# js43o/HifiDiff

Measured on AMD Instinct MI355X. Metric: faces/sec (whole node), 16→128 1000-step reverse diffusion, batch 64, higher is better.
Workload: dtype bf16

## Files before the change

hifidiff_amd/csrc/hd_dispatch.hpp:

```cpp
#pragma once
#include <type_traits>
#include "hd_gemm.hpp"
#include "hd_wide.hpp"

namespace hd {

enum LdKind { LK_F32, LK_LN, LK_BF16, LK_BF16S, LK_CONV_F32, LK_CONV_F32G, LK_CONV_BF16 };
enum EpKind { EK_BIASF32, EK_RESID, EK_GATE, EK_PIXSHUF, EK_BIASBF16, EK_DWGATE, EK_SCA };

template <class LD, class EP, bool PAIR>
hipError_t launch_tile(const GemmP& p, int mode, hipStream_t s) {
    constexpr bool kWideLN = std::is_same<LD, LdF32LN_T<false>>::value && std::is_same<EP, EpGateBF16>::value && PAIR;
    constexpr bool kWidePlain = std::is_same<LD, LdBF16Plain>::value && std::is_same<EP, EpResidF32>::value && !PAIR;
    if constexpr (kWideLN || kWidePlain) {
        const int form = (mode & 32) ? wide_shape_ok<PAIR>(p) : 0;
        if ((form == 1 || (form == 3 && kWideLN)) && (!kWideLN || wide_stats_ok<PAIR>(p))) return launch_gemm_wide<kWideLN, EP, PAIR>(p, s);
    }
    if constexpr (ld_is_deep<LD>::value && ep_is_deep<EP>::value) {
        if ((mode & 16) && deep_shape_ok<PAIR>(p)) return launch_gemm_deep<LD, EP, PAIR>(p, s);
    }
    mode &= 15;
    if constexpr (PAIR) {
        switch (mode) {
            case 0: return launch_gemm<T128P, LD, EP>(p, s);
            case 1: return launch_gemm<T64P, LD, EP>(p, s);
            case 2: return launch_skinny_auto<1, 2, true, LD, EP>(p, s);
            case 4: return launch_gemm<T32WP, LD, EP>(p, s);
            case 5: return launch_skinny_auto<4, 1, true, LD, EP>(p, s);
            case 6: return launch_skinny_auto<8, 1, true, LD, EP>(p, s);
            default: return launch_skinny_auto<1, 1, true, LD, EP>(p, s);
        }
    } else {
        switch (mode) {
            case 0: return launch_gemm<T128, LD, EP>(p, s);
            case 1: return launch_gemm<T64, LD, EP>(p, s);
            case 2: return launch_skinny_auto<1, 2, false, LD, EP>(p, s);
            case 4: return launch_gemm<T32W, LD, EP>(p, s);
            case 5: return launch_skinny_auto<4, 1, false, LD, EP>(p, s);
            case 6: return launch_skinny_auto<8, 1, false, LD, EP>(p, s);
            default: return launch_skinny_auto<1, 1, false, LD, EP>(p, s);
        }
    }
}

template <class LN>
hipError_t dispatch_dwgate(const GemmP& p, hipStream_t s) {
    if constexpr (std::is_same<LN, LdF32LN_T<false>>::value) {
        static const bool no_wide = hd_env("HD_NO_WIDE") != nullptr;
        const int form = wide_shape_ok<true>(p);
        if (!no_wide && form && wide_stats_ok<true>(p) && p.hw >= 4 && wide_form_rows(form) % p.hw == 0 && p.side * p.side == p.hw)
            return launch_gemm_wide<true, EpDwGate, true>(p, s);
    }
    if constexpr (ld_is_deep<LN>::value) {
        static const bool no_deep_dw = hd_env("HD_NO_DEEP_DW") != nullptr;
        if (!no_deep_dw && deep_shape_ok<true>(p) && p.M % 128 == 0 && p.hw >= 4 && p.hw <= 128 && 128 % p.hw == 0 && p.side * p.side == p.hw)
            return launch_gemm_deep<LN, EpDwGate, true>(p, s);
    }
    if (p.hw <= 32 && 64 % p.hw == 0 && p.M % 64 == 0 && (p.M / 32) * (p.N / 64) >= (p.Kp >= 2048 ? 512 : 1024)) return launch_skinny_auto<1, 2, true, LN, EpDwGate>(p, s);
    if (p.hw <= 32) return launch_skinny_auto<1, 1, true, LN, EpDwGate>(p, s);
    static const bool big64 = hd_env("HD_NO_DW64_WM8") == nullptr;
    if (p.hw == 64 && big64 && p.M % 256 == 0 && (p.M / 64) * (p.N / 64) >= 1024) return launch_skinny_auto<8, 1, true, LN, EpDwGate>(p, s);
    if (p.hw == 64) return launch_skinny_auto<2, 1, true, LN, EpDwGate>(p, s);
    if (p.hw == 256) return launch_skinny_auto<8, 1, true, LN, EpDwGate>(p, s);
    return hipErrorInvalidValue;
}

template <class LN>
hipError_t dispatch_ln(const GemmP& p, EpKind ek, int mode, hipStream_t s) {
    if (ek == EK_DWGATE) {
        static const bool no_dw1 = hd_env("HD_NO_DW1") != nullptr;
        if (p.hw == 1 && !no_dw1) return launch_skinny_auto<1, 1, true, LN, EpDwGate1>(p, s);
        return dispatch_dwgate<LN>(p, s);
    }
    if (ek == EK_BIASF32) return launch_tile<LN, EpBiasF32, false>(p, mode, s);
    if (ek == EK_GATE) return launch_tile<LN, EpGateBF16, true>(p, mode, s);
    return hipErrorInvalidValue;
}

hipError_t dispatch_gemm_ln_shared(const GemmP& p, EpKind ek, int mode, hipStream_t s);
hipError_t dispatch_gemm_ln_face(const GemmP& p, EpKind ek, int mode, hipStream_t s);
hipError_t dispatch_gemm_bf16(const GemmP& p, LdKind lk, EpKind ek, int mode, hipStream_t s);
hipError_t dispatch_gemm_misc(const GemmP& p, LdKind lk, EpKind ek, int mode, hipStream_t s);

}
```

hifidiff_amd/csrc/hd_gemm.hpp:

```cpp
#pragma once
#include <hip/hip_runtime.h>
#include <stdint.h>

#include <stdlib.h>

#include <atomic>

#pragma clang fp contract(off)

namespace hd {

inline hipError_t grant_dynamic_lds(const void* fn, int bytes, std::atomic<unsigned long long>& mask) {
    int dev = 0;
    hipError_t e = hipGetDevice(&dev);
    if (e != hipSuccess) return e;
    const unsigned long long bit = 1ull << (dev & 63);
    if (mask.load(std::memory_order_acquire) & bit) return hipSuccess;
    e = hipFuncSetAttribute(fn, hipFuncAttributeMaxDynamicSharedMemorySize, bytes);
    if (e != hipSuccess) return e;
    mask.fetch_or(bit, std::memory_order_release);
    return hipSuccess;
}


inline const char* hd_env(const char* name) {
    return getenv("HD_EXPERIMENTS") != nullptr ? getenv(name) : nullptr;
}

typedef __attribute__((ext_vector_type(8))) __bf16 bf16x8_t;
typedef __attribute__((ext_vector_type(16))) float f32x16_t;

constexpr int BK = 64;
constexpr int LDS_ROW = BK * 2 + 16;

struct GemmP {
    int M, N, K, Kp;
    int nt_total;
    const uint4* W;
    const float2* stats_in;
    int stats_np, stats_cnt;
    float2* stats_out;
    const void* A;
    int lda;
    float a_scale;
    int hw;
    int face0;
    const float* film;
    int film_face_stride, film_step_stride, film_gain_off, film_bias_off;
    const int* step_ptr;
    float ln_eps;
    const float* rowscale;
    int Hin, Win, Cin, KH, KW, stride, pad, Hout, Wout, ntaps;
    const float* gate_c;
    const float* gate_s;
    const float* add_src;
    void* out;
    int ldo;
    unsigned short* out16;
    unsigned short* outg16;
    const float* bias;
    const float* rscale;
    const void* resid;
    int ldr;
    int act;
    int shuffle_r;
    int xcd_tile_affine;
    const float* dw_w;
    const float* dw_b;
    float* pooled;
    unsigned short* pooled16;
    int side;
    unsigned short* scale_G;
    int scale_hw;
    int w_nt;
    const uint4* pf_base;
    unsigned pf_tile_u4;
    int pf_ntiles;
#ifdef HD_STAMPS
    unsigned long long* stamps;
#endif
};

#ifdef HD_STAMPS
#define HD_STAMP(i)                                                                                     \
    do {                                                                                                \
        if (p.stamps && threadIdx.x == 0)                                                               \
            p.stamps[((size_t)blockIdx.y * gridDim.x + blockIdx.x) * 8 + (i)] = __builtin_amdgcn_s_memrealtime(); \
    } while (0)
#else
#define HD_STAMP(i) do { } while (0)
#endif

typedef float f32x2_t __attribute__((ext_vector_type(2)));
typedef __bf16 bf16x2_t __attribute__((ext_vector_type(2)));
__device__ __forceinline__ unsigned pack2(f32x2_t v) { return __builtin_bit_cast(unsigned, __builtin_convertvector(v, bf16x2_t)); }
__device__ __forceinline__ unsigned pack2(float lo, float hi) { return pack2((f32x2_t){lo, hi}); }
__device__ __forceinline__ uint4 pack8(const float* v) {
    return make_uint4(pack2(v[0], v[1]), pack2(v[2], v[3]), pack2(v[4], v[5]), pack2(v[6], v[7]));
}
__device__ __forceinline__ void unpack8(uint4 u, float* v) {
    v[0] = __uint_as_float(u.x << 16); v[1] = __uint_as_float(u.x & 0xffff0000u);
    v[2] = __uint_as_float(u.y << 16); v[3] = __uint_as_float(u.y & 0xffff0000u);
    v[4] = __uint_as_float(u.z << 16); v[5] = __uint_as_float(u.z & 0xffff0000u);
    v[6] = __uint_as_float(u.w << 16); v[7] = __uint_as_float(u.w & 0xffff0000u);
}
__device__ __forceinline__ float bf16_bits_to_f32(unsigned short v) { return __uint_as_float((unsigned)v << 16); }
__device__ __forceinline__ unsigned short f32_to_bf16_bits(float f) {
    return __builtin_bit_cast(unsigned short, (__bf16)f);
}
template <int CTRL>
__device__ __forceinline__ float dpp_mov(float v) {
    return __builtin_bit_cast(float, __builtin_amdgcn_update_dpp(0, __builtin_bit_cast(int, v), CTRL, 0xF, 0xF, true));
}
__device__ __forceinline__ float row16_sum(float v) {
    v += dpp_mov<0xB1>(v);
    v += dpp_mov<0x4E>(v);
    v += dpp_mov<0x141>(v);
    v += dpp_mov<0x140>(v);
    return v;
}
__device__ __forceinline__ float lane_value(float v, int lane) {
    return __builtin_bit_cast(float, __builtin_amdgcn_readlane(__builtin_bit_cast(int, v), lane));
}
__device__ __forceinline__ float halfwave_sum_hi(float v) {
    v = row16_sum(v);
    const int t = __builtin_amdgcn_update_dpp(0, __builtin_bit_cast(int, v), 0x142, 0xA, 0xF, false);
    return v + __builtin_bit_cast(float, t);
}
__device__ __forceinline__ float wave_sum(float v) {
    v = halfwave_sum_hi(v);
    return lane_value(v, 31) + lane_value(v, 63);
}

struct F8 { float4 a, b; };
__device__ __forceinline__ F8 ldg44(const float* p) {
    F8 r; r.a = *reinterpret_cast<const float4*>(p); r.b = *reinterpret_cast<const float4*>(p + 32); return r;
}
__device__ __forceinline__ F8 zero8() { F8 r; r.a = make_float4(0, 0, 0, 0); r.b = r.a; return r; }
__device__ __forceinline__ void f8_to_arr(const F8& x, float* v) {
    v[0] = x.a.x; v[1] = x.a.y; v[2] = x.a.z; v[3] = x.a.w; v[4] = x.b.x; v[5] = x.b.y; v[6] = x.b.z; v[7] = x.b.w;
}
template <bool SPLIT>
__device__ __forceinline__ void lds_write_unit(char* row_base, int kq, uint4 v) {
    if (SPLIT) {
        *reinterpret_cast<uint2*>(row_base + 8 * kq) = make_uint2(v.x, v.y);
        *reinterpret_cast<uint2*>(row_base + 64 + 8 * kq) = make_uint2(v.z, v.w);
    } else {
        *reinterpret_cast<uint4*>(row_base + 16 * kq) = v;
    }
}

struct LdF32Plain {
    static constexpr int kRawRegs = 8;
    static constexpr bool kGainBiasLds = false, kSplit = true, kStaticK = false;
    struct St { const float* rowp; bool valid; };
    struct Raw { F8 x; };
    struct Pre {};
    template <int BM, int THREADS> static __device__ __forceinline__ void block_issue(const GemmP&, int, float*, int, Pre&) {}
    template <int BM, int THREADS> static __device__ __forceinline__ void block_finish(const GemmP&, int, char*, float*, int, const Pre&) {}
    template <int BM, int THREADS> static __device__ void block_init(const GemmP&, int, char*, float*, int) {}
    template <class S> static __device__ __forceinline__ void unit_stats(S&, int, const char*) {}
    static __device__ __forceinline__ void unit_init(const GemmP& p, St& st, int row, int, const char*, const float*) {
        st.valid = row < p.M;
        st.rowp = reinterpret_cast<const float*>(p.A) + (size_t)(st.valid ? row : 0) * p.lda;
    }
    static __device__ __forceinline__ void fetch(const GemmP& p, const St& st, int kc, int kq, Raw& r) {
        if (st.valid && kc + 32 + 4 * kq < p.K) r.x = ldg44(st.rowp + kc + 4 * kq);
        else { r.x = zero8(); if (st.valid && kc + 4 * kq < p.K) r.x.a = *reinterpret_cast<const float4*>(st.rowp + kc + 4 * kq); }
    }
    static __device__ __forceinline__ uint4 finish(const GemmP& p, const St&, int, int, const Raw& r) {
        float v[8]; f8_to_arr(r.x, v);
#pragma unroll
        for (int i = 0; i < 8; ++i) v[i] *= p.a_scale;
        return pack8(v);
    }
};

template <bool PER_FACE>
struct LdF32LN_T {
    static constexpr int kRawRegs = 4;
    static constexpr bool kGainBiasLds = !PER_FACE, kSplit = false, kStaticK = true;
    static constexpr bool kDeep = !PER_FACE;
    struct St { const unsigned short* rowp; const float* gain; const float* bias; const float* gbl; float mu, rstd; bool valid; };
    struct Raw { uint4 x; };
    static constexpr int kPP = 4;
    struct Pre { float2 s[kPP]; float4 g[2], b[2]; };
    template <int BM, int THREADS> static constexpr int tpr() { return THREADS / BM >= 16 ? 16 : (THREADS / BM >= 1 ? THREADS / BM : 1); }
    template <int BM, int THREADS> static __device__ __forceinline__ bool fast(const GemmP& p) {
        return p.stats_np <= kPP * tpr<BM, THREADS>() && BM * tpr<BM, THREADS>() <= THREADS;
    }
    static __device__ __forceinline__ const float* film_row(const GemmP& p) {
        const int step = p.step_ptr ? *p.step_ptr : 0;
        return p.film + (size_t)step * p.film_step_stride;
    }
    template <int BM, int THREADS> static __device__ __forceinline__ void block_issue(const GemmP& p, int row0, float* gb, int tid, Pre& pre) {
        constexpr int TPR = tpr<BM, THREADS>();
        if (fast<BM, THREADS>(p)) {
            const int rl = tid / TPR, part = tid % TPR, row = row0 + rl;
            const bool rv = rl < BM && row < p.M;
            const float2* sp = p.stats_in + (size_t)(rv ? row : 0) * p.stats_np;
#pragma unroll
            for (int i = 0; i < kPP; ++i) {
                const int j = part + i * TPR;
                pre.s[i] = (rv && j < p.stats_np) ? sp[j] : make_float2(0.f, -1.f);
            }
        }
        if (gb && p.film_face_stride == 0) {
            const float* f = film_row(p);
#pragma unroll
            for (int i = 0; i < 2; ++i) {
                const int k = (tid + i * THREADS) * 4;
                if (k < p.K) {
                    pre.g[i] = *reinterpret_cast<const float4*>(f + p.film_gain_off + k);
                    pre.b[i] = *reinterpret_cast<const float4*>(f + p.film_bias_off + k);
                }
            }
        }
    }
    template <int BM, int THREADS> static __device__ __forceinline__ void block_finish(const GemmP& p, int row0, char* stats, float* gb, int tid, const Pre& pre) {
        constexpr int TPR = tpr<BM, THREADS>();
        float2* st = reinterpret_cast<float2*>(stats);
        if (gb && p.film_face_stride == 0) {
#pragma unroll
            for (int i = 0; i < 2; ++i) {
                const int k = (tid + i * THREADS) * 4;
                if (k < p.K) {
                    *reinterpret_cast<float4*>(gb + k) = pre.g[i];
                    *reinterpret_cast<float4*>(gb + p.Kp + k) = pre.b[i];
                }
            }
// ... 297 lines not shown
        for (int h = 0; h < 2; ++h) {
            float4 x = r.inb[h] ? r.x[h] : make_float4(0, 0, 0, 0);
            if (GATED && r.inb[h]) {
                const float4 a = r.add[h], g = r.gc[h];
                const float s = 1.0f + r.gs[h];
                x.x = (x.x + a.x) * (s + g.x); x.y = (x.y + a.y) * (s + g.y);
                x.z = (x.z + a.z) * (s + g.z); x.w = (x.w + a.w) * (s + g.w);
            }
            v[4 * h] = x.x; v[4 * h + 1] = x.y; v[4 * h + 2] = x.z; v[4 * h + 3] = x.w;
        }
        return pack8(v);
    }
};

__device__ __forceinline__ float activate(float v, int act) {
    if (act == 1) return fmaxf(v, 0.f);
    if (act == 2) return 1.0f / (1.0f + expf(-v));
    return v;
}
struct ColC { float bias, bias2, rscale, rscale2; };

struct EpBiasF32 {
    static constexpr bool kStats = true, kTile = false;
    static __device__ __forceinline__ size_t stat_index(const GemmP& p, int row, int tile_idx) { return (size_t)row * (p.N >> 5) + tile_idx; }
    static __device__ __forceinline__ ColC col_init(const GemmP& p, int col) { ColC c; c.bias = p.bias ? p.bias[col] : 0.f; c.bias2 = 0.f; c.rscale = 1.f; return c; }
    static __device__ __forceinline__ float pre(const GemmP&, int, int) { return 0.f; }
    static __device__ __forceinline__ float store(const GemmP& p, int row, int col, float v, float, const ColC& c) {
        v = activate(v + c.bias, p.act);
        reinterpret_cast<float*>(p.out)[(size_t)row * p.ldo + col] = v;
        if (p.out16) p.out16[(size_t)row * p.ldo + col] = f32_to_bf16_bits(v);
        return v;
    }
};
struct EpScaBF16 {
    static constexpr bool kStats = false, kTile = false, kScaTile = true;
    static __device__ __forceinline__ ColC col_init(const GemmP& p, int col) { ColC c; c.bias = p.bias[col]; c.bias2 = 0.f; c.rscale = 1.f; return c; }
    static __device__ __forceinline__ float pre(const GemmP&, int, int) { return 0.f; }
    static __device__ __forceinline__ float store(const GemmP& p, int row, int col, float v, float, const ColC& c) {
        v += c.bias;
        reinterpret_cast<float*>(p.out)[(size_t)row * p.ldo + col] = v;
        return v;
    }
};
struct EpResidF32 {
    static constexpr bool kStats = true, kTile = false;
    static constexpr bool kDeep = true;
    static __device__ __forceinline__ size_t stat_index(const GemmP& p, int row, int tile_idx) { return (size_t)row * (p.N >> 5) + tile_idx; }
    static __device__ __forceinline__ ColC col_init(const GemmP& p, int col) { ColC c; c.bias = p.bias[col]; c.bias2 = 0.f; c.rscale = p.rscale[col]; return c; }
    static __device__ __forceinline__ float pre(const GemmP& p, int row, int col) {
        return reinterpret_cast<const float*>(p.resid)[(size_t)row * p.ldr + col];
    }
    static __device__ __forceinline__ float store(const GemmP& p, int row, int col, float v, float r, const ColC& c) {
        v = fmaf(v + c.bias, c.rscale, r);
        reinterpret_cast<float*>(p.out)[(size_t)row * p.ldo + col] = v;
        if (p.out16) p.out16[(size_t)row * p.ldo + col] = f32_to_bf16_bits(v);
        if (p.outg16) {
            const float a = p.add_src ? p.add_src[(size_t)row * p.ldo + col] : 0.f;
            const float g = 1.0f + p.gate_c[(size_t)(row / p.hw) * p.N + col] + p.gate_s[row];
            p.outg16[(size_t)row * p.ldo + col] = f32_to_bf16_bits((v + a) * g);
        }
        return v;
    }
};
struct EpGateBF16 {
    static constexpr bool kStats = false, kTile = false;
    static constexpr bool kDeep = true;
    static __device__ __forceinline__ ColC col_init(const GemmP& p, int col) { ColC c; c.bias = p.bias[col]; c.bias2 = p.bias[col + (p.N >> 1)]; c.rscale = 1.f; return c; }
    static __device__ __forceinline__ float pre(const GemmP&, int, int) { return 0.f; }
    static __device__ __forceinline__ void store2(const GemmP& p, int row, int col, float v1, float v2, const ColC& c) {
        reinterpret_cast<unsigned short*>(p.out)[(size_t)row * p.ldo + col] = f32_to_bf16_bits((v1 + c.bias) * (v2 + c.bias2));
    }
};
struct EpDwGate1 {
    static constexpr bool kStats = false, kTile = false;
    static __device__ __forceinline__ ColC col_init(const GemmP& p, int col) {
        const int C2 = p.N >> 1;
        const float wa = p.dw_w[(size_t)4 * p.N + col], wb = p.dw_w[(size_t)4 * p.N + col + C2];
        ColC c; c.bias = p.dw_b[col] + wa * p.bias[col]; c.bias2 = p.dw_b[col + C2] + wb * p.bias[col + C2];
        c.rscale = wa; c.rscale2 = wb;
        return c;
    }
    static __device__ __forceinline__ float pre(const GemmP&, int, int) { return 0.f; }
    static __device__ __forceinline__ void store2(const GemmP& p, int row, int col, float v1, float v2, const ColC& c) {
        const float g = fmaf(c.rscale, v1, c.bias) * fmaf(c.rscale2, v2, c.bias2);
        const size_t o = (size_t)row * p.ldo + col;
        reinterpret_cast<unsigned short*>(p.out)[o] = f32_to_bf16_bits(g);
        p.pooled[o] = g;
        if (p.pooled16) p.pooled16[o] = f32_to_bf16_bits(g);
    }
};
struct EpSca1BF16 {
    static constexpr bool kStats = false, kTile = false;
    static __device__ __forceinline__ ColC col_init(const GemmP& p, int col) { ColC c; c.bias = p.bias[col]; c.bias2 = 0.f; c.rscale = 1.f; c.rscale2 = 0.f; return c; }
    static __device__ __forceinline__ float pre(const GemmP& p, int row, int col) { return bf16_bits_to_f32(p.scale_G[(size_t)row * p.ldo + col]); }
    static __device__ __forceinline__ float store(const GemmP& p, int row, int col, float v, float g, const ColC& c) {
        v += c.bias;
        reinterpret_cast<float*>(p.out)[(size_t)row * p.ldo + col] = v;
        p.scale_G[(size_t)row * p.ldo + col] = f32_to_bf16_bits(g * v);
        return v;
    }
};
struct EpPixShufF32 {
    static constexpr bool kStats = true, kTile = false;
    static __device__ __forceinline__ ColC col_init(const GemmP&, int) { ColC c; c.bias = 0.f; c.bias2 = 0.f; c.rscale = 1.f; return c; }
    static __device__ __forceinline__ size_t out_row(const GemmP& p, int row, int sub) {
        const int lw = 31 - __builtin_clz(p.Win);
        const int b = row >> (2 * lw), rem = row & ((1 << (2 * lw)) - 1);
        const int h = rem >> lw, w = rem & (p.Win - 1);
        return (((size_t)b << (lw + 1)) + (2 * h + (sub >> 1))) * (2 * p.Win) + (2 * w + (sub & 1));
    }
    static __device__ __forceinline__ size_t index(const GemmP& p, int row, int col) {
        if (p.shuffle_r == 2) {
            const int lc = 31 - __builtin_clz(p.ldo);
            return out_row(p, row, col >> lc) * p.ldo + (col & (p.ldo - 1));
        }
        return (size_t)row * p.ldo + col;
    }
    static __device__ __forceinline__ size_t stat_index(const GemmP& p, int row, int tile_idx) {
        if (p.shuffle_r == 2) {
            const int lt = 31 - __builtin_clz(p.ldo >> 5);
            return out_row(p, row, tile_idx >> lt) * (p.ldo >> 5) + (tile_idx & ((p.ldo >> 5) - 1));
        }
        return (size_t)row * (p.N >> 5) + tile_idx;
    }
    static __device__ __forceinline__ float pre(const GemmP& p, int row, int col) {
        return p.resid ? reinterpret_cast<const float*>(p.resid)[index(p, row, col)] : 0.f;
    }
    static __device__ __forceinline__ float store(const GemmP& p, int row, int col, float v, float r, const ColC&) {
        v += r;
        const size_t o = index(p, row, col);
        reinterpret_cast<float*>(p.out)[o] = v;
        if (p.out16) p.out16[o] = f32_to_bf16_bits(v);
        return v;
    }
};
struct EpBiasBF16 {
    static constexpr bool kStats = false, kTile = false;
    static __device__ __forceinline__ ColC col_init(const GemmP& p, int col) { ColC c; c.bias = p.bias[col]; c.bias2 = 0.f; c.rscale = 1.f; return c; }
    static __device__ __forceinline__ float pre(const GemmP& p, int row, int col) {
        return p.resid ? bf16_bits_to_f32(reinterpret_cast<const unsigned short*>(p.resid)[(size_t)row * p.ldr + col]) : 0.f;
    }
    static __device__ __forceinline__ float store(const GemmP& p, int row, int col, float v, float r, const ColC& c) {
        v = activate(v + c.bias + r, p.act);
        reinterpret_cast<unsigned short*>(p.out)[(size_t)row * p.ldo + col] = f32_to_bf16_bits(v);
        return v;
    }
};
struct EpDwGate {
    static constexpr bool kStats = false, kTile = true;
    static __device__ __forceinline__ ColC col_init(const GemmP&, int) { ColC c; c.bias = 0.f; c.bias2 = 0.f; c.rscale = 1.f; return c; }
    static __device__ __forceinline__ float pre(const GemmP&, int, int) { return 0.f; }
    static __device__ __forceinline__ void store2(const GemmP&, int, int, float, float, const ColC&) {}
};

constexpr int kStatLane = 16;
__device__ __forceinline__ float2 halfwave_mean_m2(float v) {
    const float s1 = halfwave_sum_hi(v), s2 = halfwave_sum_hi(v * v);
    const float mean = s1 * (1.0f / 32.0f);
    return make_float2(mean, fmaxf(fmaf(-s1, mean, s2), 0.f));
}

template <bool FULL, bool PAIR, class EP>
__device__ __forceinline__ void tile_epilogue_mfma(const GemmP& p, const f32x16_t& a1, const f32x16_t& a2, int rbase, int col,
                                                   int ncols, int tile_idx, int lane) {
    const bool cv = FULL || col < ncols;
    const ColC cc = EP::col_init(p, cv ? col : 0);
    float pre[16], v[16];
#pragma unroll
    for (int i = 0; i < 16; ++i) {
        const int row = rbase + (i & 3) + 8 * (i >> 2);
        pre[i] = (FULL || (cv && row < p.M)) ? EP::pre(p, row, col) : 0.f;
    }
#pragma unroll
    for (int i = 0; i < 16; ++i) {
        const int row = rbase + (i & 3) + 8 * (i >> 2);
        v[i] = 0.f;
        if (FULL || (cv && row < p.M)) {
            if constexpr (PAIR) EP::store2(p, row, col, a1[i], a2[i], cc);
            else v[i] = EP::store(p, row, col, a1[i], pre[i], cc);
        }
    }
    if constexpr (EP::kStats) {
        if (p.stats_out) {
            float2 ms[16];
#pragma unroll
            for (int i = 0; i < 16; ++i) ms[i] = halfwave_mean_m2(v[i]);
            if ((lane & 31) == kStatLane) {
#pragma unroll
                for (int i = 0; i < 16; ++i) {
                    const int row = rbase + (i & 3) + 8 * (i >> 2);
                    if (FULL || row < p.M) p.stats_out[EP::stat_index(p, row, tile_idx)] = ms[i];
                }
            }
        }
    }
}

template <int WM_, int WN_, int MT_, int TN_, bool PAIR_>
struct Cfg {
    static constexpr int WM = WM_, WN = WN_, MT = MT_, TN = TN_;
    static constexpr bool PAIR = PAIR_;
    static constexpr int WAVES = WM * WN;
    static constexpr int THREADS = 64 * WAVES;
    static constexpr int BM = WM * MT * 32;
    static constexpr int TNT = PAIR ? 2 * TN : TN;
    static constexpr int NCOLS = WN * TN * 32;
    static constexpr int UNITS = BM * 8 / THREADS;
    static constexpr int A_BUF = BM * LDS_ROW;
    static constexpr int STATS_OFF = 2 * A_BUF;
    static constexpr int GB_OFF = STATS_OFF + BM * 8;
    static constexpr int SMEM = GB_OFF;
    static_assert(UNITS >= 1 && UNITS * THREADS == BM * 8, "tile/threads mismatch");
};

template <class C, class LD, class EP>
__global__ __launch_bounds__(C::THREADS) void gemm_kernel(const GemmP p) {
    extern __shared__ __attribute__((aligned(16))) char smem[];
    const int tid = threadIdx.x, lane = tid & 63, wave = tid >> 6;
    const int w_m = wave / C::WN, w_n = wave - w_m * C::WN;
    const int row0 = blockIdx.x * C::BM;
    const int ksteps_total = p.Kp >> 4;
    const int c_end = p.Kp >> 6;

    int tile[C::TNT];
#pragma unroll
    for (int tn = 0; tn < C::TN; ++tn) {
        const int t = (blockIdx.y * C::WN + w_n) * C::TN + tn;
        tile[tn] = t;
        if (C::PAIR) tile[C::TN + tn] = t + (p.N >> 6);
    }
    const int tiles_half = C::PAIR ? (p.N >> 6) : p.nt_total;

    HD_STAMP(0);
    float* gb = LD::kGainBiasLds ? reinterpret_cast<float*>(smem + C::GB_OFF) : nullptr;
    typename LD::St st[C::UNITS];
    int u_ldsoff[C::UNITS];
    const int kq = tid & 7;
#pragma unroll
    for (int u = 0; u < C::UNITS; ++u) {
        const int rl = (tid >> 3) + u * (C::THREADS / 8);
        u_ldsoff[u] = rl * LDS_ROW;
        LD::unit_init(p, st[u], row0 + rl, rl, smem + C::STATS_OFF, gb);
    }

    f32x16_t acc[C::MT][C::TNT];
#pragma unroll
    for (int mt = 0; mt < C::MT; ++mt)
#pragma unroll
        for (int tn = 0; tn < C::TNT; ++tn)
#pragma unroll
            for (int i = 0; i < 16; ++i) acc[mt][tn][i] = 0.f;

    typename LD::Raw raw[C::UNITS];
    uint4 bcur[C::TNT][4], bnxt[C::TNT][4];
    const uint4* Wl = p.W + lane;

#define HD_LOAD_B(dst, chunk)                                                                         \
    _Pragma("unroll") for (int tn = 0; tn < C::TNT; ++tn) {                                           \
        const bool tv = (tn < C::TN ? tile[tn] : tile[tn] - (p.N >> 6)) < tiles_half &&               \
                        tile[tn] < p.nt_total;                                                        \
        _Pragma("unroll") for (int s = 0; s < 4; ++s)                                                 \
            dst[tn][s] = tv ? Wl[((size_t)tile[tn] * ksteps_total + (chunk) * 4 + s) * 64]            \
                            : make_uint4(0, 0, 0, 0);                                                 \
    }
#define HD_FETCH_A(chunk)                                                                             \
    _Pragma("unroll") for (int u = 0; u < C::UNITS; ++u) LD::fetch(p, st[u], (chunk) * BK, kq, raw[u]);
#define HD_WRITE_A(chunk, buf)                                                                        \
    _Pragma("unroll") for (int u = 0; u < C::UNITS; ++u)                                              \
        lds_write_unit<LD::kSplit>(smem + (buf) * C::A_BUF + u_ldsoff[u], kq, LD::finish(p, st[u], (chunk) * BK, kq, raw[u]));

    HD_FETCH_A(0);
    HD_LOAD_B(bcur, 0);
    LD::template block_init<C::BM, C::THREADS>(p, row0, smem + C::STATS_OFF, gb, tid);
#pragma unroll
    for (int u = 0; u < C::UNITS; ++u) LD::unit_stats(st[u], (tid >> 3) + u * (C::THREADS / 8), smem + C::STATS_OFF);
    HD_STAMP(1);
    HD_WRITE_A(0, 0);
    __syncthreads();
    HD_STAMP(2);

    const int a_lane_off = (lane & 31) * LDS_ROW + (lane >> 5) * 16;
    for (int c = 0; c < c_end; ++c) {
        const int buf = c & 1;
        const bool has_next = (c + 1) < c_end;
        if (has_next) {
            HD_FETCH_A(c + 1);
            HD_LOAD_B(bnxt, c + 1);
        }
        const char* sA = smem + buf * C::A_BUF + a_lane_off;
#pragma unroll
        for (int s = 0; s < 4; ++s) {
            bf16x8_t a[C::MT];
#pragma unroll
            for (int mt = 0; mt < C::MT; ++mt)
                a[mt] = *reinterpret_cast<const bf16x8_t*>(sA + ((w_m * C::MT + mt) * 32) * LDS_ROW + s * 32);
#pragma unroll
            for (int tn = 0; tn < C::TNT; ++tn)
#pragma unroll
                for (int mt = 0; mt < C::MT; ++mt)
                    acc[mt][tn] = __builtin_amdgcn_mfma_f32_32x32x16_bf16(
                        a[mt], __builtin_bit_cast(bf16x8_t, bcur[tn][s]), acc[mt][tn], 0, 0, 0);
        }
        if (has_next) {
            HD_WRITE_A(c + 1, buf ^ 1);
        }
        __syncthreads();
// ... 289 lines not shown
            const bool up = y > 0, dn = y < S - 1;
            const int row = row0 + p0;
            unsigned short* gout = reinterpret_cast<unsigned short*>(p.out) + (size_t)row * p.ldo + col;
            const int left = p.M - row;
            float rsum;
            switch (S) {
                case 16: rsum = dw_gate_row<16>(t1a, t1b, p0, up, dn, wa, wb, ba, bb, gout, p.ldo, true, left); break;
                case 8: rsum = dw_gate_row<8>(t1a, t1b, p0, up, dn, wa, wb, ba, bb, gout, p.ldo, true, left); break;
                case 4: rsum = dw_gate_row<4>(t1a, t1b, p0, up, dn, wa, wb, ba, bb, gout, p.ldo, true, left); break;
                default: rsum = dw_gate_row<2>(t1a, t1b, p0, up, dn, wa, wb, ba, bb, gout, p.ldo, true, left); break;
            }
            rs[rr * 32 + j] = rsum;
        }
        asm volatile("s_waitcnt lgkmcnt(0)\n\ts_barrier" ::: "memory");
        const int faces = 128 / HW;
        for (int idx = tid; idx < faces * 32; idx += THREADS) {
            const int f = idx >> 5;
            float sacc = 0.f;
            for (int r = 0; r < S; ++r) sacc += rs[(f * S + r) * 32 + j];
            const int face = row0 / HW + f;
            if (face * HW < p.M) {
                const float pm = sacc / (float)HW;
                p.pooled[(size_t)face * C2 + col] = pm;
                if (p.pooled16) p.pooled16[(size_t)face * C2 + col] = f32_to_bf16_bits(pm);
            }
        }
        (void)ncols;
        return;
    }
    float* xch = reinterpret_cast<float*>(smem);
    if (half) {
#pragma unroll
        for (int i = 0; i < 16; ++i) xch[(w_m * 16 + i) * 64 + lane] = acc[i];
    }
    asm volatile("s_waitcnt lgkmcnt(0)\n\ts_barrier" ::: "memory");
    if (!half) {
        f32x16_t acc2;
#pragma unroll
        for (int i = 0; i < 16; ++i) acc2[i] = xch[(w_m * 16 + i) * 64 + lane];
        const int ncols = p.N >> 1;
        const int rtile = row0 + w_m * 32;
        const int rbase = rtile + 4 * (lane >> 5);
        const int col = tile0 * 32 + (lane & 31);
        if (rtile + 32 <= p.M) tile_epilogue_mfma<true, true, EP>(p, acc, acc2, rbase, col, ncols, tile0, lane);
        else tile_epilogue_mfma<false, true, EP>(p, acc, acc2, rbase, col, ncols, tile0, lane);
    }
    HD_STAMP(5);
}

template <class EP, class = void> struct ep_is_sca_tile { static constexpr bool value = false; };
template <class EP> struct ep_is_sca_tile<EP, decltype((void)EP::kScaTile)> { static constexpr bool value = EP::kScaTile; };

typedef unsigned u32x4_t __attribute__((ext_vector_type(4)));
__device__ __forceinline__ void prefetch_issue(const GemmP& p, int lin, int nwg, int tid, int nthreads, u32x4_t& sink) {
    if (!p.pf_base) return;
    const int x = lin & 7, r = lin >> 3, per_x = nwg >> 3;
    const int tiles_x = (p.pf_ntiles - x + 7) >> 3;
    if (tiles_x <= 0 || r >= per_x) return;
    const unsigned total = (unsigned)tiles_x * p.pf_tile_u4;
    const unsigned share = (total + per_x - 1) / per_x;
    const unsigned lo = share * r, hi = (lo + share < total) ? lo + share : total;
    for (unsigned i = lo + tid; i < hi; i += nthreads) {
        const unsigned t = i / p.pf_tile_u4, o = i - t * p.pf_tile_u4;
        const uint4* q = p.pf_base + ((size_t)(x + 8 * t) * p.pf_tile_u4 + o);
        asm volatile("global_load_dwordx4 %0, %1, off" : "+v"(sink) : "v"(q) : "memory");
    }
}
__device__ __forceinline__ void prefetch_drain(u32x4_t& sink) {
    asm volatile("s_waitcnt vmcnt(0)" : "+v"(sink) : : "memory");
}

typedef unsigned nt_u32x4 __attribute__((ext_vector_type(4)));
__device__ __forceinline__ uint4 nt_load_u4(const uint4* q) {
    const nt_u32x4 v = __builtin_nontemporal_load(reinterpret_cast<const nt_u32x4*>(q));
    return make_uint4(v.x, v.y, v.z, v.w);
}
template <int WM_, int WK_, int MT_, bool PAIR_, int D_, bool HALF_ = false>
struct SkinnyCfg {
    static constexpr int WM = WM_, WK = WK_, MT = MT_, D = D_;
    static constexpr bool HALF = HALF_;
    static_assert(!HALF_ || (WM_ == 1 && MT_ == 1), "HALF tiles are single-row-tile workgroups");
    static constexpr int WROWS = HALF_ ? 16 : MT_ * 32;
    static constexpr int WAVES = WM * WK, THREADS = 64 * WAVES, BM = WM * WROWS, TNT = PAIR_ ? 2 : 1;
    static constexpr int UN = WROWS / 8;
    static constexpr int A_WAVE = MT * 32 * LDS_ROW;
    static constexpr int RED = WK * BM * 32 * TNT * 4;
    static constexpr int STAGE = (WAVES * A_WAVE > RED) ? WAVES * A_WAVE : RED;
    static constexpr int GT_OFF = STAGE;
    static constexpr int STATS_OFF = GT_OFF + BM * 32 * 4;
    static constexpr int GB_OFF = STATS_OFF + BM * 8;
};

template <int S>
__device__ __forceinline__ float dw_gate_row(const float* t1a, const float* t1b, int p0, bool up, bool dn, const float* wa,
                                             const float* wb, float ba, float bb, unsigned short* gout, int ldo, bool store_ok,
                                             int rows_left) {
    float va[3][S + 2], vb[3][S + 2];
#pragma unroll
    for (int r = 0; r < 3; ++r) { va[r][0] = 0.f; va[r][S + 1] = 0.f; vb[r][0] = 0.f; vb[r][S + 1] = 0.f; }
#pragma unroll
    for (int x = 0; x < S; ++x) {
        va[0][x + 1] = up ? t1a[(p0 + x - S) * 32] : 0.f; vb[0][x + 1] = up ? t1b[(p0 + x - S) * 32] : 0.f;
        va[1][x + 1] = t1a[(p0 + x) * 32];                vb[1][x + 1] = t1b[(p0 + x) * 32];
        va[2][x + 1] = dn ? t1a[(p0 + x + S) * 32] : 0.f; vb[2][x + 1] = dn ? t1b[(p0 + x + S) * 32] : 0.f;
    }
    float rsum = 0.f;
#pragma unroll
    for (int x = 0; x < S; ++x) {
        float u1 = ba, u2 = bb;
#pragma unroll
        for (int r = 0; r < 3; ++r) {
            u1 = fmaf(wa[r * 3], va[r][x], u1); u1 = fmaf(wa[r * 3 + 1], va[r][x + 1], u1); u1 = fmaf(wa[r * 3 + 2], va[r][x + 2], u1);
            u2 = fmaf(wb[r * 3], vb[r][x], u2); u2 = fmaf(wb[r * 3 + 1], vb[r][x + 1], u2); u2 = fmaf(wb[r * 3 + 2], vb[r][x + 2], u2);
        }
        const float g = u1 * u2;
        rsum += g;
        if (store_ok && x < rows_left) gout[(size_t)x * ldo] = f32_to_bf16_bits(g);
    }
    return rsum;
}

template <class C> struct SkinnyPre { static constexpr int NIT = (C::BM * 32 + C::THREADS - 1) / C::THREADS; ColC cc; float pre[NIT]; };
template <bool FULL, class C, class EP>
__device__ __forceinline__ void skinny_rows_pre(const GemmP& p, int row0, int col, int ncols, int tid, SkinnyPre<C>& sp) {
    constexpr int NIT = SkinnyPre<C>::NIT;
    constexpr bool EVEN = (C::BM * 32) % C::THREADS == 0;
    const bool cv = FULL || col < ncols;
    sp.cc = EP::col_init(p, cv ? col : 0);
#pragma unroll
    for (int it = 0; it < NIT; ++it) {
        const int e = it * C::THREADS + tid;
        const int row = row0 + (e >> 5);
        const bool ok = (EVEN || e < C::BM * 32) && (FULL || (row < p.M && cv));
        sp.pre[it] = ok ? EP::pre(p, row, col) : 0.f;
    }
}
template <bool FULL, class C, class EP>
__device__ __forceinline__ void skinny_rows_epilogue(const GemmP& p, const float* red, int row0, int col, int ncols, int tile_idx, int tid,
                                                     const SkinnyPre<C>& sp) {
    constexpr int NIT = (C::BM * 32 + C::THREADS - 1) / C::THREADS, TNT = C::TNT, WK = C::WK;
    constexpr int TILE_F = C::BM * 32 * TNT;
    constexpr bool EVEN = (C::BM * 32) % C::THREADS == 0;
    const bool cv = FULL || col < ncols;
    const ColC cc = sp.cc;
    const float (&pre)[NIT] = sp.pre;
    float v[NIT];
#pragma unroll
    for (int it = 0; it < NIT; ++it) {
        const int e = it * C::THREADS + tid;
        const int row = row0 + (e >> 5);
        const bool ev = EVEN || e < C::BM * 32;
        float v1 = 0.f, v2 = 0.f;
        if (ev) {
#pragma unroll
            for (int w = 0; w < WK; ++w) {
                v1 += red[w * TILE_F + e];
                if (TNT == 2) v2 += red[w * TILE_F + C::BM * 32 + e];
            }
        }
        v[it] = 0.f;
        if (ev && (FULL || (row < p.M && cv))) {
            if constexpr (TNT == 2) EP::store2(p, row, col, v1, v2, cc);
            else v[it] = EP::store(p, row, col, v1, pre[it], cc);
        }
    }
    if constexpr (EP::kStats) {
        if (p.stats_out) {
            float2 ms[NIT];
#pragma unroll
            for (int it = 0; it < NIT; ++it) ms[it] = halfwave_mean_m2(v[it]);
            if ((tid & 31) == kStatLane) {
#pragma unroll
                for (int it = 0; it < NIT; ++it) {
                    const int e = it * C::THREADS + tid;
                    const int row = row0 + (e >> 5);
                    if ((EVEN || e < C::BM * 32) && (FULL || row < p.M)) p.stats_out[EP::stat_index(p, row, tile_idx)] = ms[it];
                }
            }
        }
    }
}

template <class C, class LD, class EP, bool W_NT = false, int CPW = 0>
__global__ __launch_bounds__(C::THREADS) void gemm_skinny_kernel(const GemmP p) {
    extern __shared__ __attribute__((aligned(16))) char smem[];
    constexpr int MT = C::MT, TNT = C::TNT, WK = C::WK, D = C::D, UN = C::UN;
    const int tid = threadIdx.x, lane = tid & 63, wave = tid >> 6;
    const int wm = wave / WK, wk = wave - wm * WK;
    int bx = blockIdx.x, by = blockIdx.y;
    if (p.xcd_tile_affine && (gridDim.y & 7) == 0 && gridDim.x > 1) {
        const int lin = blockIdx.y * gridDim.x + blockIdx.x;
        const int j = lin >> 3;
        bx = j % (int)gridDim.x;
        by = (j / (int)gridDim.x) * 8 + (lin & 7);
    }
    const int row0 = bx * C::BM;
    const int ksteps_total = p.Kp >> 4;
    const int cpw = CPW > 0 ? CPW : (p.Kp >> 6) / WK;
    const int c0 = wk * cpw, c_end = c0 + cpw;
    int tile[TNT];
    tile[0] = by;
    if (TNT == 2) tile[1] = by + (p.N >> 6);
    const uint4* Wl = p.W + lane;
    constexpr bool w_nt = W_NT;
    HD_STAMP(0);

    f32x16_t acc[MT][TNT];
#pragma unroll
    for (int mt = 0; mt < MT; ++mt)
#pragma unroll
        for (int tn = 0; tn < TNT; ++tn)
#pragma unroll
            for (int i = 0; i < 16; ++i) acc[mt][tn][i] = 0.f;
    uint4 bq[D][4][TNT];
    typename LD::Raw aq[D][UN];
#define HD_SK_LOAD_B(slot, chunk)                                                                      \
    _Pragma("unroll") for (int ss = 0; ss < 4; ++ss) _Pragma("unroll") for (int tn = 0; tn < TNT; ++tn) \
        bq[slot][ss][tn] = ((chunk) < c_end) ? (w_nt ? nt_load_u4(&Wl[((size_t)tile[tn] * ksteps_total + (chunk) * 4 + ss) * 64]) : Wl[((size_t)tile[tn] * ksteps_total + (chunk) * 4 + ss) * 64]) : make_uint4(0, 0, 0, 0);
    float* gb = LD::kGainBiasLds ? reinterpret_cast<float*>(smem + C::GB_OFF) : nullptr;
    typename LD::Pre pre;
    LD::template block_issue<C::BM, C::THREADS>(p, row0, gb, tid, pre);
#define HD_SK_LOAD_B_NC(slot, chunk)                                                                   \
    _Pragma("unroll") for (int ss = 0; ss < 4; ++ss) _Pragma("unroll") for (int tn = 0; tn < TNT; ++tn) \
        bq[slot][ss][tn] = w_nt ? nt_load_u4(&Wl[((size_t)tile[tn] * ksteps_total + (chunk) * 4 + ss) * 64]) : Wl[((size_t)tile[tn] * ksteps_total + (chunk) * 4 + ss) * 64];
    if constexpr (CPW == 0) {
#pragma unroll
        for (int d = 0; d < D; ++d) { HD_SK_LOAD_B(d, c0 + d); }
    }

    typename LD::St st[UN];
    int u_off[UN];
    const int kq = lane & 7;
#pragma unroll
    for (int u = 0; u < UN; ++u) {
        const int rw = (lane >> 3) + 8 * u;
        const int rl = wm * C::WROWS + rw;
        u_off[u] = rw * LDS_ROW;
        LD::unit_init(p, st[u], row0 + rl, rl, smem + C::STATS_OFF, gb);
    }
#define HD_SK_FETCH_A(slot, chunk)                                                                     \
    _Pragma("unroll") for (int u = 0; u < UN; ++u)                                                     \
        LD::fetch(p, st[u], ((chunk) < c_end) ? (chunk) * BK : p.Kp, kq, aq[slot][u]);
#define HD_SK_FETCH_A_NC(slot, chunk) \
    _Pragma("unroll") for (int u = 0; u < UN; ++u) LD::fetch_nc(p, st[u], (chunk) * BK, kq, aq[slot][u]);
    if constexpr (CPW > 0) {
#pragma unroll
        for (int d = 0; d < (D < CPW ? D : CPW); ++d) { HD_SK_LOAD_B_NC(d, c0 + d); HD_SK_FETCH_A_NC(d, c0 + d); }
    } else {
#pragma unroll
        for (int d = 0; d < D; ++d) { HD_SK_FETCH_A(d, c0 + d); }
    }
    constexpr bool kEarlyDw = EP::kTile && C::THREADS >= 512;
    float dw_wa[9], dw_wb[9], dw_ba = 0.f, dw_bb = 0.f, dw_b1a = 0.f, dw_b1b = 0.f;
    auto load_dw = [&]() {
        const int ncols_e = p.N >> 1, col_e = tile[0] * 32 + (tid & 31);
        const bool cok = col_e < ncols_e;
#pragma unroll
        for (int t = 0; t < 9; ++t) { dw_wa[t] = cok ? p.dw_w[(size_t)t * p.N + col_e] : 0.f; dw_wb[t] = cok ? p.dw_w[(size_t)t * p.N + col_e + ncols_e] : 0.f; }
        if (cok) { dw_ba = p.dw_b[col_e]; dw_bb = p.dw_b[col_e + ncols_e]; dw_b1a = p.bias[col_e]; dw_b1b = p.bias[col_e + ncols_e]; }
    };
    if constexpr (kEarlyDw) load_dw();
    uint4 sca_g[2] = {make_uint4(0, 0, 0, 0), make_uint4(0, 0, 0, 0)};
    if constexpr (ep_is_sca_tile<EP>::value) {
        const int hw = p.scale_hw, units = C::BM * hw * 4;
        if (hw > 0 && tile[0] * 32 + 32 <= p.N) {
#pragma unroll
            for (int j = 0; j < 2; ++j) {
                const int u = tid + j * C::THREADS;
                const int f = u / (hw * 4), rem = u - f * hw * 4, r = rem >> 2, q = rem & 3;
                if (u < units && row0 + f < p.M)
                    sca_g[j] = *reinterpret_cast<const uint4*>(p.scale_G + ((size_t)(row0 + f) * hw + r) * p.ldo + tile[0] * 32 + q * 8);
            }
        }
    }
    constexpr bool kEarlyPre = !EP::kTile && !ep_is_sca_tile<EP>::value && C::THREADS >= 512;
    SkinnyPre<C> spre;
    if constexpr (kEarlyPre) {
        const int ncols_e = (TNT == 2) ? (p.N >> 1) : p.N, col_e = tile[0] * 32 + (tid & 31);
        const bool full_e = (row0 + C::BM <= p.M) && (tile[0] * 32 + 32 <= ncols_e);
        if (full_e) skinny_rows_pre<true, C, EP>(p, row0, col_e, ncols_e, tid, spre);
        else skinny_rows_pre<false, C, EP>(p, row0, col_e, ncols_e, tid, spre);
    }
    u32x4_t pf_sink = {0u, 0u, 0u, 0u};
    prefetch_issue(p, (int)(blockIdx.y * gridDim.x + blockIdx.x), (int)(gridDim.x * gridDim.y), tid, C::THREADS, pf_sink);
    HD_STAMP(6);
    LD::template block_finish<C::BM, C::THREADS>(p, row0, smem + C::STATS_OFF, gb, tid, pre);
#pragma unroll
    for (int u = 0; u < UN; ++u) LD::unit_stats(st[u], wm * C::WROWS + (lane >> 3) + 8 * u, smem + C::STATS_OFF);
    HD_STAMP(1);

    char* sA = smem + wave * C::A_WAVE;
    const int a_lane_off = (lane & 31) * LDS_ROW + (lane >> 5) * 16;
    if constexpr (C::HALF) {
        for (int i = lane; i < 16 * LDS_ROW / 16; i += 64) reinterpret_cast<uint4*>(sA + 16 * LDS_ROW)[i] = make_uint4(0, 0, 0, 0);
        __builtin_amdgcn_wave_barrier();
    }
    auto chunk_mma = [&](int d, int cc) {
        if constexpr (CPW > 0) {
            typename LD::ChunkC chunk_c;
            LD::chunk_consts(p, st[0], cc * BK, kq, chunk_c);
#pragma unroll
            for (int u = 0; u < UN; ++u) lds_write_unit<LD::kSplit>(sA + u_off[u], kq, LD::finish_nc(p, st[u], cc * BK, kq, aq[d][u], chunk_c));
        } else {
#pragma unroll
            for (int u = 0; u < UN; ++u) lds_write_unit<LD::kSplit>(sA + u_off[u], kq, LD::finish(p, st[u], cc * BK, kq, aq[d][u]));
        }
        __builtin_amdgcn_wave_barrier();
#pragma unroll
        for (int ss = 0; ss < 4; ++ss) {
            bf16x8_t a[MT];
#pragma unroll
            for (int mt = 0; mt < MT; ++mt)
                a[mt] = *reinterpret_cast<const bf16x8_t*>(sA + a_lane_off + (mt * 32) * LDS_ROW + ss * 32);
#pragma unroll
            for (int tn = 0; tn < TNT; ++tn)
#pragma unroll
                for (int mt = 0; mt < MT; ++mt)
                    acc[mt][tn] = __builtin_amdgcn_mfma_f32_32x32x16_bf16(
                        a[mt], __builtin_bit_cast(bf16x8_t, bq[d][ss][tn]), acc[mt][tn], 0, 0, 0);
        }
        __builtin_amdgcn_wave_barrier();
    };
    if constexpr (CPW > 0) {
#pragma unroll
        for (int i = 0; i < CPW; ++i) {
            const int d = i % D, cc = c0 + i;
            chunk_mma(d, cc);
            if (i + D < CPW) { HD_SK_LOAD_B_NC(d, cc + D); HD_SK_FETCH_A_NC(d, cc + D); }
            if (i == 0) HD_STAMP(2);
        }
    } else {
        for (int cb = c0; cb < c_end; cb += D) {
#pragma unroll
            for (int d = 0; d < D; ++d) {
                const int cc = cb + d;
                if (cc < c_end) {
                    chunk_mma(d, cc);
                    HD_SK_LOAD_B(d, cc + D);
                    HD_SK_FETCH_A(d, cc + D);
                    if (cc == c0) HD_STAMP(2);
                }
            }
        }
    }
#undef HD_SK_LOAD_B
#undef HD_SK_FETCH_A
#undef HD_SK_LOAD_B_NC
#undef HD_SK_FETCH_A_NC
    HD_STAMP(3);

    __syncthreads();
    HD_STAMP(4);
    float* red = reinterpret_cast<float*>(smem);
    constexpr int TILE_F = C::BM * 32 * TNT;
#pragma unroll
    for (int mt = 0; mt < MT; ++mt)
#pragma unroll
        for (int tn = 0; tn < TNT; ++tn)
#pragma unroll
            for (int i = 0; i < (C::HALF ? 8 : 16); ++i) {
                const int r = (wm * MT + mt) * 32 + (i & 3) + 8 * (i >> 2) + 4 * (lane >> 5);
                red[wk * TILE_F + (tn * C::BM + r) * 32 + (lane & 31)] = acc[mt][tn][i];
            }
    __syncthreads();
    const int ncols = (TNT == 2) ? (p.N >> 1) : p.N;
    const int col = tile[0] * 32 + (tid & 31);

    if constexpr (EP::kTile) {
        static_assert(TNT == 2, "EpDwGate needs a PAIR tile");
        const int C2 = p.N >> 1;
        if constexpr (!kEarlyDw) load_dw();
        {
            const float bias_a = dw_b1a, bias_b = dw_b1b;
            for (int e = tid; e < C::BM * 32; e += C::THREADS) {
                float va = bias_a, vb = bias_b;
#pragma unroll
                for (int w = 0; w < WK; ++w) { va += red[w * TILE_F + e]; vb += red[w * TILE_F + C::BM * 32 + e]; }
                red[e] = va; red[C::BM * 32 + e] = vb;
            }
        }
        __syncthreads();
        float* rs = reinterpret_cast<float*>(smem + C::GT_OFF);
        const int j = tid & 31;
        const int S = p.side, ls = 31 - __builtin_clz(S), HW = p.hw;
        const float (&wa)[9] = dw_wa; const float (&wb)[9] = dw_wb;
        const float ba = dw_ba, bb = dw_bb;
        const float* t1a = red + j;
        const float* t1b = red + C::BM * 32 + j;
        const int nrows_img = C::BM >> ls;
        for (int rr = tid >> 5; rr < nrows_img; rr += C::THREADS / 32) {
            const int p0 = rr << ls;
            const int y = (p0 & (HW - 1)) >> ls;
            const bool up = y > 0, dn = y < S - 1;
            const int row = row0 + p0;
            unsigned short* gout = reinterpret_cast<unsigned short*>(p.out) + (size_t)row * p.ldo + col;
            const bool ok = col < ncols;
            const int left = p.M - row;
            float rsum;
            switch (S) {
                case 16: rsum = dw_gate_row<16>(t1a, t1b, p0, up, dn, wa, wb, ba, bb, gout, p.ldo, ok, left); break;
                case 8: rsum = dw_gate_row<8>(t1a, t1b, p0, up, dn, wa, wb, ba, bb, gout, p.ldo, ok, left); break;
                case 4: rsum = dw_gate_row<4>(t1a, t1b, p0, up, dn, wa, wb, ba, bb, gout, p.ldo, ok, left); break;
                case 2: rsum = dw_gate_row<2>(t1a, t1b, p0, up, dn, wa, wb, ba, bb, gout, p.ldo, ok, left); break;
                default: rsum = dw_gate_row<1>(t1a, t1b, p0, up, dn, wa, wb, ba, bb, gout, p.ldo, ok, left); break;
            }
            rs[rr * 32 + j] = rsum;
        }
        __syncthreads();
        const int faces = C::BM / HW;
        for (int idx = tid; idx < faces * 32; idx += C::THREADS) {
            const int f = idx >> 5;
            float sacc = 0.f;
            for (int r = 0; r < S; ++r) sacc += rs[(f * S + r) * 32 + j];
            const int face = row0 / HW + f;
            if (face * HW < p.M && col < ncols) {
                const float pm = sacc / (float)HW;
                p.pooled[(size_t)face * C2 + col] = pm;
                if (p.pooled16) p.pooled16[(size_t)face * C2 + col] = f32_to_bf16_bits(pm);
            }
        }
    } else if constexpr (ep_is_sca_tile<EP>::value) {
        {
            const float bias = col < ncols ? p.bias[col] : 0.f;
            for (int e = tid; e < C::BM * 32; e += C::THREADS) {
                float v = bias;
#pragma unroll
                for (int w = 0; w < WK; ++w) v += red[w * TILE_F + e];
                const int face = row0 + (e >> 5);
                if (face < p.M && col < ncols) reinterpret_cast<float*>(p.out)[(size_t)face * p.ldo + col] = v;
                red[e] = v;
            }
        }
        __syncthreads();
        const int hw = p.scale_hw;
        if (hw > 0 && tile[0] * 32 + 32 <= ncols) {
            const int units = C::BM * hw * 4;
            for (int u0 = tid; u0 < units; u0 += C::THREADS * 2) {
                uint4 g[2]; unsigned short* gp[2]; const float* sp[2]; bool ok[2];
#pragma unroll
                for (int j = 0; j < 2; ++j) {
                    const int u = u0 + j * C::THREADS;
                    const int f = u / (hw * 4), rem = u - f * hw * 4, r = rem >> 2, q = rem & 3;
                    const int face = row0 + f;
                    ok[j] = u < units && face < p.M;
                    gp[j] = p.scale_G + ((size_t)(ok[j] ? face : 0) * hw + r) * p.ldo + tile[0] * 32 + q * 8;
                    sp[j] = red + f * 32 + q * 8;
                    g[j] = (u0 == tid) ? sca_g[j]
                                       : (ok[j] ? *reinterpret_cast<const uint4*>(gp[j]) : make_uint4(0, 0, 0, 0));
                }
#pragma unroll
                for (int j = 0; j < 2; ++j) {
                    if (ok[j]) {
                        float v[8];
                        unpack8(g[j], v);
#pragma unroll
                        for (int i = 0; i < 8; ++i) v[i] *= sp[j][i];
                        *reinterpret_cast<uint4*>(gp[j]) = pack8(v);
                    }
                }
            }
        }
    } else {
        const bool full = (row0 + C::BM <= p.M) && (tile[0] * 32 + 32 <= ncols);
        if constexpr (!kEarlyPre) {
            if (full) skinny_rows_pre<true, C, EP>(p, row0, col, ncols, tid, spre);
            else skinny_rows_pre<false, C, EP>(p, row0, col, ncols, tid, spre);
        }
        if (full) skinny_rows_epilogue<true, C, EP>(p, red, row0, col, ncols, tile[0], tid, spre);
        else skinny_rows_epilogue<false, C, EP>(p, red, row0, col, ncols, tile[0], tid, spre);
    }
    if (p.pf_base) prefetch_drain(pf_sink);
    HD_STAMP(5);
}

typedef Cfg<4, 1, 1, 2, false> T128;
typedef Cfg<4, 1, 1, 1, true> T128P;
typedef Cfg<2, 2, 1, 1, false> T64;
typedef Cfg<2, 2, 1, 1, true> T64P;
typedef Cfg<1, 4, 1, 2, false> T32W;
typedef Cfg<1, 4, 1, 1, true> T32WP;

template <class C, class LD, class EP>
inline hipError_t launch_gemm(const GemmP& p, hipStream_t s) {
    const int ncols = C::PAIR ? p.N / 2 : p.N;
    const int smem = C::SMEM + (LD::kGainBiasLds ? 2 * p.Kp * 4 : 0);
    if (smem > 65536) {
        static std::atomic<unsigned long long> granted{0};
        { const hipError_t e = grant_dynamic_lds(reinterpret_cast<const void*>(&gemm_kernel<C, LD, EP>), 160 * 1024, granted); if (e != hipSuccess) return e; }
    }
    dim3 grid((p.M + C::BM - 1) / C::BM, (ncols + C::NCOLS - 1) / C::NCOLS, 1);
    hipLaunchKernelGGL((gemm_kernel<C, LD, EP>), grid, dim3(C::THREADS), smem, s, p);
    return hipGetLastError();
}

template <bool PAIR>
inline bool deep_shape_ok(const GemmP& p) {
    const int ncols = PAIR ? p.N / 2 : p.N;
    return p.K == p.Kp && (p.Kp == 512 || p.Kp == 1024) && p.M >= (PAIR ? 1024 : 2048) && ncols % 32 == 0 && p.film_face_stride == 0 &&
           ((p.M + 127) / 128) * (ncols / 32) >= 256;
}
#ifndef HD_DEEP_P
#define HD_DEEP_P 4
#endif
template <class LD, class EP, bool PAIR>
inline hipError_t launch_gemm_deep(const GemmP& p, hipStream_t s) {
    typedef Cfg<4, 1, 1, 1, PAIR> C;
    constexpr int P = HD_DEEP_P;
    const int ncols = PAIR ? p.N / 2 : p.N;
    const int smem = C::SMEM + (LD::kGainBiasLds ? 2 * p.Kp * 4 : 0) + 2 * (PAIR ? 8 : 4) * 1024;
    dim3 grid((p.M + C::BM - 1) / C::BM, ncols / 32, 1);
    if constexpr (PAIR) {
        if (p.Kp == 1024) hipLaunchKernelGGL((gemm_deep_pair8_kernel<LD, EP, 16, P>), grid, dim3(512), smem, s, p);
        else hipLaunchKernelGGL((gemm_deep_pair8_kernel<LD, EP, 8, P>), grid, dim3(512), smem, s, p);
        return hipGetLastError();
    }
    if (p.Kp == 1024) hipLaunchKernelGGL((gemm_deep_kernel<C, LD, EP, 16, P>), grid, dim3(C::THREADS), smem, s, p);
    else hipLaunchKernelGGL((gemm_deep_kernel<C, LD, EP, 8, P>), grid, dim3(C::THREADS), smem, s, p);
    return hipGetLastError();
}

template <class C, class LD, class EP, bool NT, int CPW>
inline hipError_t launch_skinny_inst(const GemmP& p, hipStream_t s, int smem) {
    if (smem > 65536) {
        static std::atomic<unsigned long long> granted{0};
        { const hipError_t e = grant_dynamic_lds(reinterpret_cast<const void*>(&gemm_skinny_kernel<C, LD, EP, NT, CPW>), 160 * 1024, granted); if (e != hipSuccess) return e; }
    }
    const int ncols = (C::TNT == 2) ? p.N / 2 : p.N;
    dim3 grid((p.M + C::BM - 1) / C::BM, (ncols + 31) / 32, 1);
    hipLaunchKernelGGL((gemm_skinny_kernel<C, LD, EP, NT, CPW>), grid, dim3(C::THREADS), smem, s, p);
    return hipGetLastError();
}

template <class C, class LD, class EP>
inline hipError_t launch_skinny(const GemmP& p, hipStream_t s) {
    const int smem = C::GB_OFF + (LD::kGainBiasLds ? 2 * p.Kp * 4 : 0);
    if (smem > 160 * 1024 || (p.Kp / 64) % C::WK != 0) return hipErrorInvalidValue;
    const bool nt = p.w_nt != 0;
    if constexpr (LD::kStaticK) {
        static const bool no_static = hd_env("HD_NO_STATIC_K") != nullptr;
        const int cpw = (p.Kp / 64) / C::WK;
        const int ncols = (C::TNT == 2) ? p.N / 2 : p.N;
        const bool ok = !no_static && p.K == p.Kp && ncols % 32 == 0 && LD::static_ok(p);
        if (ok && (cpw == 2 || cpw == 4)) {
            if (cpw == 4) return nt ? launch_skinny_inst<C, LD, EP, true, 4>(p, s, smem) : launch_skinny_inst<C, LD, EP, false, 4>(p, s, smem);
            return nt ? launch_skinny_inst<C, LD, EP, true, 2>(p, s, smem) : launch_skinny_inst<C, LD, EP, false, 2>(p, s, smem);
        }
        if constexpr (LD::kStatic8 && C::WK == 8 && C::MT == 1) {
            if (ok && cpw == 8) return nt ? launch_skinny_inst<C, LD, EP, true, 8>(p, s, smem) : launch_skinny_inst<C, LD, EP, false, 8>(p, s, smem);
        }
    }
    return nt ? launch_skinny_inst<C, LD, EP, true, 0>(p, s, smem) : launch_skinny_inst<C, LD, EP, false, 0>(p, s, smem);
}

template <int MT, bool PAIR, class LD>
struct ChunkDepth {
    static constexpr int TNT = PAIR ? 2 : 1;
    static constexpr int fixed = MT * TNT * 16 + 48 + MT * 4 * 6;
    static constexpr int per_d = TNT * 16 + MT * 4 * LD::kRawRegs;
    static constexpr int D = (fixed + 3 * per_d <= 236) ? 3 : ((fixed + 2 * per_d <= 236) ? 2 : 1);
};

template <int WM, int MT, bool PAIR, class LD, class EP>
inline hipError_t launch_skinny_auto(const GemmP& p, hipStream_t s) {
    constexpr int D = ChunkDepth<MT, PAIR, LD>::D;
    const int chunks = p.Kp / 64;
    if constexpr (WM == 1 && MT == 1) {
        static const bool no_half = hd_env("HD_NO_HALF") != nullptr;
        const int tiles = (PAIR ? p.N / 2 : p.N) / 32;
        static const int half_m = hd_env("HD_HALF_M") ? atoi(hd_env("HD_HALF_M")) : 64;
        static const int half_wg = hd_env("HD_HALF_WG") ? atoi(hd_env("HD_HALF_WG")) : 256;
        if (!no_half && p.M <= half_m && p.M % 16 == 0 && ((p.M + 31) / 32) * tiles < half_wg) {
            if (chunks >= 16 && chunks % 8 == 0) return launch_skinny<SkinnyCfg<1, 8, 1, PAIR, D, true>, LD, EP>(p, s);
            if (chunks >= 8 && chunks % 4 == 0) return launch_skinny<SkinnyCfg<1, 4, 1, PAIR, D, true>, LD, EP>(p, s);
        }
    }
    if constexpr (WM <= 1) if (chunks >= 16 && chunks % 8 == 0) return launch_skinny<SkinnyCfg<WM, 8, MT, PAIR, D>, LD, EP>(p, s);
    if constexpr (WM <= 2) if (chunks >= 8 && chunks % 4 == 0) return launch_skinny<SkinnyCfg<WM, 4, MT, PAIR, D>, LD, EP>(p, s);
    if constexpr (WM <= 4) if (chunks >= 4 && chunks % 2 == 0) return launch_skinny<SkinnyCfg<WM, 2, MT, PAIR, D>, LD, EP>(p, s);
    return launch_skinny<SkinnyCfg<WM, 1, MT, PAIR, D>, LD, EP>(p, s);
}

}

#pragma clang fp contract(fast)
```

hifidiff_amd/csrc/hd_internal.hpp:

```cpp
#pragma once
#include <hip/hip_runtime.h>

#include <cmath>
#include <cstdio>
#include <cstring>
#include <functional>
#include <map>
#include <memory>
#include <string>
#include <unordered_map>
#include <vector>

#include "../../include/hifidiff_hip.h"
#include "hd_chain.hpp"
#include "hd_conv.hpp"
#include "hd_cr.hpp"
#include "hd_dispatch.hpp"
#include "hd_gemm.hpp"
#include "hd_kernels.hpp"
#include "hd_end.hpp"
#include "hd_faceset.hpp"
#include "hd_vae.hpp"
#include "hd_stage_api.hpp"

using namespace hd;

namespace hdi {

constexpr int WIDTH = 128;
constexpr int FILM_IN = 256;
constexpr size_t HOST_MIRROR_MAX = 1 << 16;

struct RawTensor {
    std::vector<int64_t> shape;
    size_t numel = 0;
    float* dev = nullptr;
    std::vector<float> host;
};

struct PackedW {
    uint4* w = nullptr;
    int N = 0, K = 0, Kp = 0, nt_total = 0;
    const float* bias = nullptr;
};

struct BlockW {
    std::string name;
    int C = 0, film_off = -1;
    PackedW conv1, conv3, sca, conv4, conv5;
    const float *dw_w = nullptr, *dw_b = nullptr, *beta = nullptr, *gamma = nullptr;
    const float* dw_wT = nullptr;
};

struct HcaW {
    int C = 0;
    PackedW mlp0, mlp2, sp0, fused;
    const float* sp3_w = nullptr;
    float sp3_b = 0.f;
    bool centre_only = false;
};

struct ResConv { PackedW w; int cin, cout, k, stride, pad; };
struct ResBlock { ResConv c1, c2, c3, ds; bool has_ds = false; };


struct Op {
    std::string name;
    std::function<hipError_t(hipStream_t)> run;
    std::shared_ptr<GemmP> gemm;
    bool skinny_affine = false;
    const void* out = nullptr;
    size_t out_elems = 0;
    int out_bf16 = 0;
    int lk = -1, ek = -1, mode = -1;
};

struct Level { int C, H, M; float *X, *Y, *T1, *pooled, *S; unsigned short *G, *Xb, *Yb, *Xg, *pooled16; float2 *sx, *sy; };

struct SampleCall {
    const char* fn = "";
    int n = 0, ncoef = 7;
    const float *timesteps = nullptr, *coef = nullptr;
    const float* noise = nullptr;
    uint64_t seed = 0;
    const int32_t* start_rows = nullptr;
    int n_iters = 0;
    const int32_t *begin_rows = nullptr, *end_rows = nullptr;
    const uint64_t* face_seeds = nullptr;
    const int32_t* first = nullptr;
    int resume = 0;
};
constexpr size_t kFaceArgBytes = sizeof(uint64_t) + 4 * sizeof(int32_t);
struct FaceArgs { unsigned long long* seeds; int *rows, *first, *begins, *ends; };
inline FaceArgs face_args(void* base, int B) {
    unsigned long long* seeds = static_cast<unsigned long long*>(base);
    int* rows = reinterpret_cast<int*>(seeds + B);
    return FaceArgs{seeds, rows, rows + B, rows + 2 * B, rows + 3 * B};
}
struct StageCursor {
    size_t at = 0;
    size_t take(size_t bytes) { const size_t o = at; at += (bytes + 7) / 8 * 8; return o; }
};

}
using namespace hdi;

struct Chain {
    int B = 0, face0 = 0, index = 0;
    Level lv[5];
    float *lat = nullptr, *eps = nullptr, *x0_hist = nullptr, *prior[5] = {}, *gate_c[5] = {}, *gate_s[5] = {}, *idc_term = nullptr;
    float *id_emb = nullptr, *pool_tmp = nullptr, *mlp_tmp = nullptr, *sp_tmp = nullptr;
    unsigned short* res_buf[4] = {};
    uint4* face8 = nullptr;
    std::vector<Op> program;
    std::vector<Op> prep_program;
    StepState* step_state = nullptr;
    float* film_cur = nullptr;
    hipStream_t stream = nullptr;
    hipEvent_t done = nullptr;
    hipGraphExec_t graph_exec = nullptr;
    hipGraphExec_t graph_multi = nullptr;
    hipGraphExec_t graph_rows_exec = nullptr, graph_rows_multi = nullptr;
    unsigned rows_gen = 0;
    const float* rows_film = nullptr;
    bool fold_intro = false, fold_down0 = false, fold_up = false, fuse_end = false;
};

constexpr int kGraphSteps = 10;

struct VaeWs { float *X = nullptr, *T = nullptr, *S = nullptr, *mom = nullptr, *Q = nullptr, *K = nullptr, *V = nullptr, *resz = nullptr, *out3 = nullptr;
               unsigned short *H = nullptr, *H2 = nullptr, *Xb = nullptr, *U = nullptr; uint4* in8 = nullptr; double* part = nullptr; int B = 0, R = 0; };

struct Workspace {
    Workspace() = default;
    Workspace(const Workspace&) = delete;
    Workspace& operator=(const Workspace&) = delete;
    int key = 0;
    int B = 0;
    uint64_t stamp = 0;
    std::vector<Chain> chains;
    float *lat = nullptr, *eps = nullptr;
    float* x0_hist = nullptr;
    Chain slot_stage;
    bool slot_stage_ok = false;
    int* slots_dev = nullptr;
    std::vector<void*> allocs;
    std::map<std::string, std::pair<void*, std::pair<size_t, int>>> dbg;
    unsigned graph_gen = 0;
    const float* graph_film = nullptr;
    int graph_B = 0;
    std::vector<Op> cr_program;
    const float* cr_in = nullptr; float* cr_out = nullptr;
    float* cr_skip[5] = {};
    float *cr_loc1 = nullptr, *cr_loc2 = nullptr, *cr_theta = nullptr;
    VaeWs vws;
    std::vector<Op> vae_enc_prog, vae_dec_prog;
    const void *vae_enc_key[4] = {}, *vae_dec_key[2] = {};
    int vae_enc_flags = -1;
    uint64_t vae_seed = 0;
};

enum class EvalMode { EpsShared, EpsFaces, LoopShared, LoopRows };
constexpr bool mode_is_loop(EvalMode m) { return m == EvalMode::LoopShared || m == EvalMode::LoopRows; }
constexpr bool mode_is_rows(EvalMode m) { return m == EvalMode::LoopRows; }
constexpr bool mode_shared_row(EvalMode m) { return m == EvalMode::EpsShared || m == EvalMode::LoopShared; }
constexpr bool mode_allows_stages(EvalMode m) { return m != EvalMode::EpsFaces; }
static_assert(!mode_is_loop(EvalMode::EpsShared) && !mode_is_loop(EvalMode::EpsFaces) && mode_is_loop(EvalMode::LoopShared) && mode_is_loop(EvalMode::LoopRows), "EvalMode table");
static_assert(!mode_is_rows(EvalMode::EpsShared) && !mode_is_rows(EvalMode::EpsFaces) && !mode_is_rows(EvalMode::LoopShared) && mode_is_rows(EvalMode::LoopRows), "EvalMode table");
static_assert(mode_shared_row(EvalMode::EpsShared) && !mode_shared_row(EvalMode::EpsFaces) && mode_shared_row(EvalMode::LoopShared) && !mode_shared_row(EvalMode::LoopRows), "EvalMode table");
static_assert(mode_allows_stages(EvalMode::EpsShared) && !mode_allows_stages(EvalMode::EpsFaces) && mode_allows_stages(EvalMode::LoopShared) && mode_allows_stages(EvalMode::LoopRows), "EvalMode table");

struct hd_ctx;
struct MaskState {
    float *dmask = nullptr, *dknown = nullptr, *dnoise = nullptr;
    int *on = nullptr, *slots = nullptr;
    int cap = 0;
    FaceSet faces;
    bool active(const hd_ctx* c) const;
    void fill(const hd_ctx* c, StepState& st, size_t f0) const;
    int clear_all(hd_ctx* c, hipStream_t s);
    int clear_slots(hd_ctx* c, int n, const int32_t* slots, const int* slots_dev, hipStream_t s);
};
struct GuideState {
    bool on = false;
    float *lp = nullptr, *w = nullptr;
    int *n = nullptr, *rows = nullptr, *args = nullptr;
    int cap = 0;
    FaceSet faces;
    bool active(const hd_ctx* c) const;
    void fill(const hd_ctx* c, StepState& st, size_t f0) const;
    int clear_all(hd_ctx* c, hipStream_t s);
    int clear_slots(hd_ctx* c, int n, const int32_t* slots, const int* slots_dev, hipStream_t s);
};
struct PreviewState {
    bool on = false;
    int every = 1, snaps = 0, B = 0, planes = 0;
    float *x0 = nullptr, *snap = nullptr;
    int *row = nullptr, *slots = nullptr;
    bool active(const hd_ctx* c) const;
    void fill(const hd_ctx* c, StepState& st, size_t f0) const;
    int clear_all(hd_ctx* c, hipStream_t s);
    int clear_slots(hd_ctx* c, int n, const int32_t* slots, const int* slots_dev, hipStream_t s);
    void free_planes(hd_ctx* c);
};
struct HistState {
    bool valid = false;
    FaceSet faces;
    bool active(const hd_ctx*) const { return false; }
    void fill(const hd_ctx*, StepState&, size_t) const {}
    int clear_all(hd_ctx* c, hipStream_t s);
    int clear_slots(hd_ctx* c, int n, const int32_t* slots, const int* slots_dev, hipStream_t s);
};

struct hd_ctx {
    int L = 16, device = 0, S = 1;
    bool conditional = true;
    bool cr = false;
    struct CrStage { std::string name; int C, H, nblk, samp, level; };
    std::vector<CrStage> cr_stages;
    std::vector<BlockW> cr_blocks;
    PackedW cr_samp[9];
    float* cr_ln_pack = nullptr;
    std::string err;
    std::unordered_map<std::string, RawTensor> raw;
    std::vector<void*> allocs;
    std::unique_ptr<Workspace> ws = std::make_unique<Workspace>();
    std::map<int, std::unique_ptr<Workspace>> ws_cache;
    uint64_t ws_clock = 0;
    bool finalized = false;

    std::vector<BlockW> den_blocks, fpg_blocks;
    std::map<std::string, int> den_block_index;
    PackedW den_down[4], den_up[4], fpg_down[4], fpg_convs[5], idc_conv;
    float *intro_wT = nullptr, *fpg_intro_wT = nullptr, *ending_wT = nullptr;
    HcaW hca[5];
    ResConv res_conv1;
    std::vector<ResBlock> res_blocks;
    int film_total = 0;
    float *film_W = nullptr, *film_b = nullptr, *ln_pack = nullptr, *fpg_ln_pack = nullptr;
    FilmBlock* film_blocks_dev = nullptr;
    float* freq_dev = nullptr;
    int64_t weight_bytes_per_step = 0;
    double flops_per_face_step = 0.0;

    Chain* ch = nullptr;
    bool prepared = false;

    float *t_dev = nullptr, *temb_a = nullptr, *temb_b = nullptr, *temb_c = nullptr, *film_table = nullptr;
    int film_rows_cap = 0;
    EvalMode mode = EvalMode::EpsShared;
    float* coef_dev = nullptr;
    int coef_cap = 0;
    float* c7_dev = nullptr;
    int c7_cap = 0;
    float* film_pf = nullptr;
    size_t film_pf_cap = 0;
    unsigned long long* faces_dev = nullptr;
    int faces_cap = 0;
    unsigned rows_gen = 1, graphs_gen = 1;
    MaskState mask;
    GuideState guide;
    PreviewState preview;
    HistState hist;
    int graph_captures = 0;
    int stage_count = 0, face_stage_count = 0;
    int sample_stages = -1, sample_face_stages = -1, rows_stages = -1;
    hipEvent_t fork_ev = nullptr;
    struct Stage { float* host = nullptr; size_t cap = 0; hipEvent_t ev = nullptr; bool pending = false; } stage[2];
    int stage_idx = 0;
    std::vector<float> film_sched;
    bool film_valid = false;
    hipEvent_t film_ev = nullptr;

    bool vae = false;
    struct VaeRes { std::string name; int cin = 0, cout = 0; PackedW c1, c2, sc; bool has_sc = false; const float *n1w = nullptr, *n1b = nullptr, *n2w = nullptr, *n2b = nullptr; };
    struct VaeAttn { std::string name; const float *gw = nullptr, *gb = nullptr; PackedW q, k, v, o; };
    struct VaeW {
        PackedW enc_in, enc_out, dec_in, dec_out, enc_down[3], dec_up[3];
        VaeRes enc_res[4][2], enc_mid[2], dec_mid[2], dec_res[4][3];
        VaeAttn enc_attn, dec_attn;
        const float *enc_nw = nullptr, *enc_nb = nullptr, *dec_nw = nullptr, *dec_nb = nullptr;
        const float *quant_w = nullptr, *quant_b = nullptr, *pq_w = nullptr, *pq_b = nullptr, *ones = nullptr;
    } vw;

    struct XStage {
        XBlockW* blocks_dev = nullptr; unsigned* sync = nullptr; int nblocks = 0;
        XBlockW* blocks2_dev = nullptr; unsigned* sync2 = nullptr;
        uint4 *hX = nullptr, *hG = nullptr, *hY = nullptr; float2 *hsx = nullptr, *hsy = nullptr;
    };
    std::map<int, XStage> xstages;
    bool xcd_ok = false;
    bool xcd_on = true;
    int xcd2_mask = 0;
    bool xcd2_on = true;
    int xcd_phase_limit = 0, xcd_force_global = 0;
    struct FStage { unsigned* sync = nullptr; float* pool_part = nullptr; };
    std::map<int, FStage> fstages;
    bool face_ok = false;
    bool face_on = true;
    int face_block_limit = 0;
    bool end_fold = true;
    bool end_fused = true;
    bool up_fold = true;
    bool down_fold = true;
    bool intro_fold = true;
    int face_l1_rows = 16;
    int stage_limit_first = -1;
    unsigned* xcd_tmo_host = nullptr;
    unsigned* xcd_tmo_dev = nullptr;
    unsigned* abort_dev = nullptr;
    int stage_test_abort = 0;

    int op_limit = -1, prep_limit = -1;

    bool profiling = false;
    hipEvent_t ev0 = nullptr, ev1 = nullptr;
    double last_loop_ms = 0.0;
    int last_steps = 0;
    std::map<std::string, std::pair<void*, std::pair<size_t, int>>> dbg;

    int pool_cap = 0;
    float* pool_dev = nullptr;
    float* pool_buf[kSlotBufs] = {};
    int pool_sz[kSlotBufs] = {};
    std::vector<char> pool_ok;
};

struct FilmRows { const float* base; int face_stride; };
inline FilmRows film_rows(const hd_ctx* c, const Chain* chp) {
    return {mode_is_rows(c->mode) ? c->film_pf : mode_is_loop(c->mode) ? chp->film_cur : c->film_table, mode_shared_row(c->mode) ? 0 : c->film_total};
}
template <class P> inline void set_film(P& p, const hd_ctx* c, const Chain* chp) { const FilmRows f = film_rows(c, chp); p.film = f.base; p.film_face_stride = f.face_stride; }

#define HD_FAIL(ctx, code, ...)                                   \
    do {                                                          \
        char _b[512];                                             \
        snprintf(_b, sizeof(_b), __VA_ARGS__);                    \
        (ctx)->err = _b;                                          \
        return (code);                                            \
    } while (0)
#define HIPCHECK(ctx, expr)                                                                         \
    do {                                                                                            \
        hipError_t _e = (expr);                                                                     \
        if (_e != hipSuccess) HD_FAIL(ctx, HD_ERR_HIP, "%s failed: %s (%s:%d)", #expr, hipGetErrorString(_e), __FILE__, __LINE__); \
    } while (0)

namespace {

template <class T>
int alloc_into(hd_ctx* c, std::vector<void*>& owner, T** out, size_t count) {
    void* p = nullptr;
    HIPCHECK(c, hipMalloc(&p, count * sizeof(T) + 256));
    owner.push_back(p);
    *out = reinterpret_cast<T*>(p);
    return HD_OK;
}
template <class T> int dev_alloc(hd_ctx* c, T** out, size_t count) { return alloc_into(c, c->allocs, out, count); }
template <class T> int ws_alloc(hd_ctx* c, T** out, size_t count) { return alloc_into(c, c->ws->allocs, out, count); }
void dev_free(hd_ctx* c, void* p) {
    if (!p) return;
    for (auto& a : c->allocs)
        if (a == p) { a = nullptr; break; }
    (void)hipFree(p);
}

struct BufSpec { char** p; size_t bytes; bool zero; };
template <class T> BufSpec buf_spec(T** p, size_t count, bool zero) { return {reinterpret_cast<char**>(p), count * sizeof(T), zero}; }
int realloc_buffers(hd_ctx* c, std::initializer_list<BufSpec> bufs, hipStream_t s) {
    auto drop = [&] { for (const BufSpec& b : bufs) { dev_free(c, *b.p); *b.p = nullptr; } };
    auto make = [&]() -> int {
        for (const BufSpec& b : bufs) { const int rc = dev_alloc(c, b.p, b.bytes); if (rc) return rc; }
        for (const BufSpec& b : bufs) if (b.zero) HIPCHECK(c, hipMemsetAsync(*b.p, 0, b.bytes, s));
        return HD_OK;
    };
    drop();
    const int rc = make();
    if (rc) drop();
    return rc;
}
template <class F>
int each_extra(hd_ctx* c, F f) {
    int rc = f(c->mask);
    if (!rc) rc = f(c->guide);
    if (!rc) rc = f(c->preview);
    if (!rc) rc = f(c->hist);
    return rc;
}

struct ChainCursor {
    hd_ctx* c; Chain* prev;
    ChainCursor(hd_ctx* c_, Chain* ch) : c(c_), prev(c_->ch) { c->ch = ch; }
    ~ChainCursor() { c->ch = prev; }
    ChainCursor(const ChainCursor&) = delete;
    ChainCursor& operator=(const ChainCursor&) = delete;
};

int alloc_level(hd_ctx* c, Level& v, int B, size_t xg, bool names, int l) {
    const size_t mc = (size_t)v.M * v.C;
    int rc = 0;
    rc |= ws_alloc(c, &v.X, mc); rc |= ws_alloc(c, &v.Y, mc); rc |= ws_alloc(c, &v.T1, 2 * mc + (size_t)B * ((v.H + 7) / 8) * v.C);
    rc |= ws_alloc(c, &v.G, mc); rc |= ws_alloc(c, &v.pooled, (size_t)B * v.C); rc |= ws_alloc(c, &v.S, (size_t)B * v.C);
    rc |= ws_alloc(c, &v.sx, (size_t)v.M * (v.C / 32)); rc |= ws_alloc(c, &v.sy, (size_t)v.M * (v.C / 32));
    rc |= ws_alloc(c, &v.Xb, mc); rc |= ws_alloc(c, &v.Yb, mc); rc |= ws_alloc(c, &v.Xg, xg);
    rc |= ws_alloc(c, &v.pooled16, (size_t)B * v.C);
    if (rc || !names) return rc;
    auto& dbg = c->ws->dbg;
    const std::string s = std::to_string(l);
    dbg["X" + s] = {v.X, {mc, 0}}; dbg["Y" + s] = {v.Y, {mc, 0}}; dbg["T1_" + s] = {v.T1, {2 * mc, 0}};
    dbg["G" + s] = {v.G, {mc, 1}}; dbg["pooled" + s] = {v.pooled, {(size_t)B * v.C, 0}}; dbg["S" + s] = {v.S, {(size_t)B * v.C, 0}};
    dbg["Xb" + s] = {v.Xb, {mc, 1}}; dbg["Yb" + s] = {v.Yb, {mc, 1}};
    dbg["pooled16_" + s] = {v.pooled16, {(size_t)B * v.C, 1}};
    dbg["sx" + s] = {v.sx, {(size_t)v.M * (v.C / 32) * 2, 0}}; dbg["sy" + s] = {v.sy, {(size_t)v.M * (v.C / 32) * 2, 0}};
    return HD_OK;
}

constexpr size_t kWsCached = 3;
void destroy_chain_queue(Chain& ch) {
    if (ch.stream) (void)hipStreamDestroy(ch.stream);
    if (ch.done) (void)hipEventDestroy(ch.done);
    ch.stream = nullptr; ch.done = nullptr;
}
void destroy(Workspace& w) {
    if (w.slot_stage_ok) destroy_chain_queue(w.slot_stage);
    for (auto& ch : w.chains) {
        for (hipGraphExec_t g : {ch.graph_exec, ch.graph_multi, ch.graph_rows_exec, ch.graph_rows_multi}) if (g) (void)hipGraphExecDestroy(g);
        destroy_chain_queue(ch);
    }
    for (void* p : w.allocs) if (p) (void)hipFree(p);
    w.chains.clear(); w.allocs.clear();
}
template <class Make>
int switch_workspace(hd_ctx* c, int key, Make make) {
    if (key == c->ws->key) return HD_OK;
    c->prepared = false; c->ch = nullptr;
    if (c->ws->B != 0) {
        c->ws->stamp = ++c->ws_clock;
        const int old_key = c->ws->key;
        c->ws_cache[old_key] = std::move(c->ws);
        while (c->ws_cache.size() > kWsCached) {
            auto old = c->ws_cache.begin();
            for (auto it = c->ws_cache.begin(); it != c->ws_cache.end(); ++it) if (it->second->stamp < old->second->stamp) old = it;
            (void)hipDeviceSynchronize();
            destroy(*old->second);
            c->ws_cache.erase(old);
        }
    }
    auto it = c->ws_cache.find(key);
    if (it != c->ws_cache.end()) {
        c->ws = std::move(it->second);
        c->ws_cache.erase(it);
    } else {
        c->ws = std::make_unique<Workspace>();
        c->ws->key = key;
        if (const int rc = make(*c->ws)) { destroy(*c->ws); c->ws = std::make_unique<Workspace>(); return rc; }
    }
    c->ch = c->ws->chains.empty() ? nullptr : &c->ws->chains[0];
    return HD_OK;
}
void invalidate_step_graphs(hd_ctx* c) { ++c->graphs_gen; ++c->rows_gen; }

const RawTensor* find_raw(hd_ctx* c, const std::string& n) {
    auto it = c->raw.find(n);
    return it == c->raw.end() ? nullptr : &it->second;
}

using Shape = std::vector<int64_t>;
void m_conv(std::vector<std::pair<std::string, Shape>>& m, const std::string& n, int co, int ci, int kh, int kw, bool bias = true) {
    m.push_back({n + ".weight", {co, ci, kh, kw}});
    if (bias) m.push_back({n + ".bias", {co}});
}
void m_lin(std::vector<std::pair<std::string, Shape>>& m, const std::string& n, int co, int ci) {
    m.push_back({n + ".weight", {co, ci}});
    m.push_back({n + ".bias", {co}});
}
void m_bn(std::vector<std::pair<std::string, Shape>>& m, const std::string& n, int c) {
    m.push_back({n + ".weight", {c}}); m.push_back({n + ".bias", {c}});
    m.push_back({n + ".running_mean", {c}}); m.push_back({n + ".running_var", {c}});
    m.push_back({n + ".num_batches_tracked", {}});
}
void m_naf(std::vector<std::pair<std::string, Shape>>& m, const std::string& p, int c, bool film) {
    m.push_back({p + ".beta", {1, c, 1, 1}}); m.push_back({p + ".gamma", {1, c, 1, 1}});
    if (film) m_lin(m, p + ".mlp.1", 4 * c, FILM_IN);
    m_conv(m, p + ".conv1", 2 * c, c, 1, 1);
    m_conv(m, p + ".conv2", 2 * c, 1, 3, 3);
    m_conv(m, p + ".conv3", c, c, 1, 1);
    m_conv(m, p + ".sca.1", c, c, 1, 1);
    m_conv(m, p + ".conv4", 2 * c, c, 1, 1);
    m_conv(m, p + ".conv5", c, c, 1, 1);
    for (const char* n : {".norm1", ".norm2"}) { m.push_back({p + n + ".weight", {c}}); m.push_back({p + n + ".bias", {c}}); }
}
std::vector<std::pair<std::string, Shape>> build_manifest(int L, bool conditional = true) {
    std::vector<std::pair<std::string, Shape>> m;
    const int enc[4] = {2, 2, 4, 8}, res_layers[4] = {3, 4, 6, 3}, planes[4] = {64, 128, 256, 512};
    if (conditional) { m_conv(m, "idc.conv1", 64, 3, 7, 7, false); m_bn(m, "idc.batch_norm1", 64); }
    int cin = 64;
    for (int li = 0; li < 4 && conditional; ++li)
        for (int b = 0; b < res_layers[li]; ++b) {
            std::string q = "idc.layer" + std::to_string(li + 1) + "." + std::to_string(b);
            m_conv(m, q + ".conv1", planes[li], cin, 1, 1); m_bn(m, q + ".batch_norm1", planes[li]);
            m_conv(m, q + ".conv2", planes[li], planes[li], 3, 3); m_bn(m, q + ".batch_norm2", planes[li]);
            m_conv(m, q + ".conv3", planes[li] * 4, planes[li], 1, 1); m_bn(m, q + ".batch_norm3", planes[li] * 4);
            if (b == 0) { m_conv(m, q + ".i_downsample.0", planes[li] * 4, cin, 1, 1); m_bn(m, q + ".i_downsample.1", planes[li] * 4); }
            cin = planes[li] * 4;
        }
    const std::string d = "denoiser";
    m_lin(m, d + ".time_mlp.1", 1024, 128); m_lin(m, d + ".time_mlp.3", 512, 512);
    m_conv(m, d + ".intro", 128, 4, 3, 3); m_conv(m, d + ".ending", 4, 128, 3, 3);
    int c = WIDTH;
    for (int i = 0; i < 4; ++i) { for (int j = 0; j < enc[i]; ++j) m_naf(m, d + ".encoders." + std::to_string(i) + "." + std::to_string(j), c, true); c *= 2; }
    c = WIDTH * 16;
    for (int i = 0; i < 4; ++i) { c /= 2; for (int j = 0; j < 2; ++j) m_naf(m, d + ".decoders." + std::to_string(i) + "." + std::to_string(j), c, true); }
    c = WIDTH * 16;
    for (int j = 0; j < 8; ++j) m_naf(m, d + ".middle_blks." + std::to_string(j), c, true);
    for (int i = 0; i < 4; ++i) { m_conv(m, d + ".ups." + std::to_string(i) + ".0", c * 2, c, 1, 1, false); c /= 2; }
    c = WIDTH;
    for (int i = 0; i < 4; ++i) { m_conv(m, d + ".downs." + std::to_string(i), 2 * c, c, 2, 2); c *= 2; }
    if (!conditional) return m;
    c = WIDTH * 16;
    for (int i = 0; i < 5; ++i) {
        std::string p = d + ".hcas." + std::to_string(i);
        m_lin(m, p + ".channel_mlp.0", c, c); m_lin(m, p + ".channel_mlp.2", c, c);
        m_conv(m, p + ".spatial_mlp.0", c / 2, c, 1, 1); m_bn(m, p + ".spatial_mlp.1", c / 2);
        m_conv(m, p + ".spatial_mlp.3", 1, c / 2, 1, 1); m_bn(m, p + ".spatial_mlp.4", 1);
        m_conv(m, p + ".fused_mlp.0", c, c, 3, 3); m_bn(m, p + ".fused_mlp.1", c);
        c /= 2;
    }
    const int s = L / 16;
    m_conv(m, d + ".idc_conv", 2048 * s * s, 2048, 1, 1);
    const std::string f = "fpg";
    m_conv(m, f + ".intro", 128, 4, 3, 3);
    c = WIDTH;
    for (int i = 0; i < 4; ++i) { for (int j = 0; j < enc[i]; ++j) m_naf(m, f + ".encoders." + std::to_string(i) + "." + std::to_string(j), c, false); c *= 2; }
    c = WIDTH;
    for (int i = 0; i < 4; ++i) { m_conv(m, f + ".downs." + std::to_string(i), 2 * c, c, 2, 2); c *= 2; }
    m_conv(m, f + ".convs.0.0", c, c, 1, 1, false);
    for (int i = 1; i < 5; ++i) { m_conv(m, f + ".convs." + std::to_string(i) + ".0", c * 2, c, 1, 1, false); c /= 2; }
    return m;
}

static void cr_stage_list(std::vector<hd_ctx::CrStage>& st) {
    st.clear();
    const int enc[4] = {2, 2, 4, 8};
    int C = 32, H = 128;
    for (int i = 0; i < 4; ++i) { st.push_back({"encoders." + std::to_string(i), C, H, enc[i], 1, i}); C *= 2; H /= 2; }
    st.push_back({"middle_blocks", C, H, 8, 0, 4});
    for (int i = 0; i < 4; ++i) { st.push_back({"decoders." + std::to_string(i), C, H, 2, 2, 4 - i}); C /= 2; H *= 2; }
}
static void stn_shape(int res, int* k0, int* k1, int* fc) {
    if (res <= 8) { *k0 = 3; *k1 = 1; } else if (res <= 16) { *k0 = 5; *k1 = 3; } else if (res <= 32) { *k0 = 7; *k1 = 5; } else { *k0 = 9; *k1 = 7; }
    const int fr = (res - *k0 - 2 * *k1 + 3) / 4;
    *fc = 10 * fr * fr;
}
std::vector<std::pair<std::string, Shape>> build_cr_manifest() {
    std::vector<std::pair<std::string, Shape>> m;
    m_conv(m, "intro", 32, 3, 3, 3); m_conv(m, "outro", 3, 32, 3, 3);
    std::vector<hd_ctx::CrStage> st;
    cr_stage_list(st);
    for (const auto& g : st) {
        for (int j = 0; j < g.nblk; ++j) m_naf(m, g.name + ".nfbs." + std::to_string(j), g.C, false);
        int k0, k1, fc;
        stn_shape(g.H, &k0, &k1, &fc);
        const int n1 = (int)std::sqrt((double)fc);
        m_conv(m, g.name + ".stn.localization.0", 8, g.C, k0, k0); m_conv(m, g.name + ".stn.localization.3", 10, 8, k1, k1);
        m_lin(m, g.name + ".stn.fc_loc.0", n1, fc); m_lin(m, g.name + ".stn.fc_loc.2", 6, n1);
        if (g.samp == 1) m_conv(m, g.name + ".sampling", 2 * g.C, g.C, 2, 2);
        else if (g.samp == 2) m_conv(m, g.name + ".sampling.0", 2 * g.C, g.C, 1, 1, false);
    }
    return m;
}

int upload_vec(hd_ctx* c, const std::vector<float>& v, const float** out) {
    float* d = nullptr;
    int rc = dev_alloc(c, &d, v.size());
    if (rc) return rc;
    HIPCHECK(c, hipMemcpy(d, v.data(), v.size() * sizeof(float), hipMemcpyHostToDevice));
    *out = d;
    return HD_OK;
}

int bn_affine(hd_ctx* c, const std::string& bn, std::vector<float>& s, std::vector<float>& o) {
    const RawTensor *w = find_raw(c, bn + ".weight"), *b = find_raw(c, bn + ".bias"), *m = find_raw(c, bn + ".running_mean"),
                    *v = find_raw(c, bn + ".running_var");
    if (!w || !b || !m || !v) HD_FAIL(c, HD_ERR_WEIGHTS, "missing BatchNorm tensors for %s", bn.c_str());
    const size_t n = w->numel;
    s.resize(n); o.resize(n);
    for (size_t i = 0; i < n; ++i) {
        s[i] = w->host[i] / std::sqrt(v->host[i] + 1e-5f);
        o[i] = b->host[i] - m->host[i] * s[i];
    }
    return HD_OK;
}

struct PackOpts { int cin_pad = 0; bool centre_only = false; int S2 = 1; std::string bn; };

int pack_weight(hd_ctx* c, const std::string& name, PackedW* out, const PackOpts& o = PackOpts()) {
    const RawTensor* w = find_raw(c, name + ".weight");
    if (!w) HD_FAIL(c, HD_ERR_WEIGHTS, "missing %s.weight", name.c_str());
    const int N = (int)w->shape[0], Cin = (int)w->shape[1];
    const int KH = w->shape.size() == 4 ? (int)w->shape[2] : 1, KW = w->shape.size() == 4 ? (int)w->shape[3] : 1;
    const int cin_pad = o.cin_pad ? o.cin_pad : Cin;
    const int ntaps = o.centre_only ? 1 : KH * KW;
    PackP p{};
    p.src = w->dev; p.N = N; p.Cin = Cin; p.Cin_pad = cin_pad; p.KH = KH; p.KW = KW; p.ntaps = ntaps;
    p.centre_only = o.centre_only ? 1 : 0; p.S2 = o.S2;
    const int K = ntaps * cin_pad;
    p.Kp = (K + 63) / 64 * 64;
    p.nt_total = (N + 31) / 32;
    std::vector<float> s, off;
    const float* nscale = nullptr;
    if (!o.bn.empty()) {
        int rc = bn_affine(c, o.bn, s, off);
        if (rc) return rc;
        rc = upload_vec(c, s, &nscale);
        if (rc) return rc;
    }
    p.nscale = nscale;
    const size_t n16 = (size_t)p.nt_total * (p.Kp / 16) * 64;
    int rc = dev_alloc(c, &p.dst, n16);
    if (rc) return rc;
    const int blocks = (int)std::min<size_t>((n16 + 255) / 256, 65535);
    hipLaunchKernelGGL(pack_weight_kernel, dim3(blocks), dim3(256), 0, 0, p);
    HIPCHECK(c, hipGetLastError());
    out->w = p.dst; out->N = N; out->K = K; out->Kp = p.Kp; out->nt_total = p.nt_total;
    const RawTensor* b = find_raw(c, name + ".bias");
    out->bias = b ? b->dev : nullptr;
    if (!o.bn.empty() || (o.S2 > 1 && b)) {
        std::vector<float> bf(N, 0.f);
        for (int n = 0; n < N; ++n) {
            float v = b ? b->host[n] : 0.f;
            if (!o.bn.empty()) v = v * s[n] + off[n];
            bf[n] = v;
        }
        if (o.S2 > 1) {
            std::vector<float> bp(N);
            const int cg = N / o.S2;
            for (int np = 0; np < N; ++np) bp[np] = bf[(np % cg) * o.S2 + np / cg];
            bf.swap(bp);
        }
        rc = upload_vec(c, bf, &out->bias);
        if (rc) return rc;
    }
    return HD_OK;
}

bool dwgate_ok(int hw) { return hw == 1 || hw == 4 || hw == 16 || hw == 64 || hw == 256; }

hipError_t dispatch_gemm(const GemmP& p, LdKind lk, EpKind ek, int mode, hipStream_t s) {
    if (lk == LK_LN) return p.film_face_stride != 0 ? dispatch_gemm_ln_face(p, ek, mode, s) : dispatch_gemm_ln_shared(p, ek, mode, s);
    if (lk == LK_BF16 || lk == LK_BF16S) return dispatch_gemm_bf16(p, lk, ek, mode, s);
    return dispatch_gemm_misc(p, lk, ek, mode, s);
}

int choose_mode(const GemmP& p, bool pair) {
    const int ncols = pair ? p.N / 2 : p.N;
    const int nb64 = (ncols + 63) / 64, nb32 = (ncols + 31) / 32;
    static const int force = hd_env("HD_GEMM_MODE") ? atoi(hd_env("HD_GEMM_MODE")) : -1;
    if (force >= 0) return force;
    const int nb256 = (ncols + (pair ? 127 : 255)) / (pair ? 128 : 256);
    if (p.Kp <= 256 && nb256 <= 2 && ((p.M + 31) / 32) * nb256 >= 512) return 4;
    const bool wm_ok = p.Kp >= 1024 || (p.Kp >= 512 && ((p.M + 63) / 64) * nb32 >= 1024);
    if (wm_ok && p.M >= 2048) {
        if (((p.M + 255) / 256) * nb32 >= 256) return 6;
        if (((p.M + 127) / 128) * nb32 >= 192) return 5;
    }
    static const int tall_maxk = hd_env("HD_TALL_MAXK") ? atoi(hd_env("HD_TALL_MAXK")) : 128;
    if (p.Kp <= tall_maxk) {
        if (((p.M + 127) / 128) * nb64 >= 256) return 0;
        if (((p.M + 63) / 64) * nb64 >= 256) return 1;
    }
    const int wg64 = ((p.M + 63) / 64) * nb32;
    static const int short_k_wg = hd_env("HD_SHORTK_WG") ? atoi(hd_env("HD_SHORTK_WG")) : 2048;
    if (wg64 >= 192 && (p.Kp > 512 || wg64 >= short_k_wg)) return 2;
    return 3;
}

GemmP base_gemm(const PackedW& w, int M) {
    GemmP p{};
    p.M = M; p.N = w.N; p.K = w.K; p.Kp = w.Kp; p.nt_total = w.nt_total; p.W = w.w; p.bias = w.bias;
    p.a_scale = 1.f; p.hw = 1; p.ln_eps = 1e-6f; p.shuffle_r = 1; p.stats_np = 1; p.stats_cnt = 1;
    return p;
}

void add_gemm(hd_ctx* c, std::vector<Op>& prog, const std::string& name, GemmP p, LdKind lk, EpKind ek, int mode_hint = -1) {
    int t128 = choose_mode(p, ek == EK_GATE || ek == EK_DWGATE);
    if (mode_hint >= 0 && hd_env("HD_GEMM_MODE") == nullptr) t128 = mode_hint;
    {
        static const bool no_deep = hd_env("HD_NO_DEEP") != nullptr;
        const bool kinds = (lk == LK_LN && ek == EK_GATE) || (lk == LK_BF16 && ek == EK_RESID);
        if (kinds && !no_deep && mode_hint < 0 && (ek == EK_GATE ? deep_shape_ok<true>(p) : deep_shape_ok<false>(p))) t128 |= 16;
    }
    {
        static const bool no_wide = hd_env("HD_NO_WIDE") != nullptr;
        const bool pair = (lk == LK_LN && ek == EK_GATE), plain = (lk == LK_BF16 && ek == EK_RESID);
        if (!no_wide && ((pair && (wide_shape_ok<true>(p) == 1 || wide_shape_ok<true>(p) == 3)) || (plain && wide_shape_ok<false>(p) == 1))) t128 |= 32;
    }
    {
        static const std::string over = hd_env("HD_OP_MODE") ? hd_env("HD_OP_MODE") : "";
        for (size_t at = 0; at < over.size();) {
            const size_t end = over.find(',', at) == std::string::npos ? over.size() : over.find(',', at);
            const size_t eq = over.find('=', at);
            if (eq != std::string::npos && eq < end && name.find(over.substr(at, eq - at)) != std::string::npos) { t128 = atoi(over.c_str() + eq + 1); break; }
            at = end + 1;
        }
    }
    {
        const size_t a_bytes = (size_t)p.M * p.Kp * ((lk == LK_BF16 || lk == LK_BF16S || lk == LK_CONV_BF16 || lk == LK_LN) ? 2 : 4);
        p.xcd_tile_affine = ((size_t)p.N * p.Kp * 2 > a_bytes) ? 1 : 0;
        static const bool no_nt = hd_env("HD_NO_NT") != nullptr;
        static const int nt_maxm = hd_env("HD_NT_MAXM") ? atoi(hd_env("HD_NT_MAXM")) : 256;
        p.w_nt = (!no_nt && p.xcd_tile_affine && p.M <= nt_maxm) ? 1 : 0;
    }
    const bool film = (lk == LK_LN);
    size_t out_rows = (size_t)p.M * (ek == EK_PIXSHUF ? p.shuffle_r * p.shuffle_r : 1);
    Op op;
    op.name = name; op.out = p.out; op.out_elems = out_rows * p.ldo; op.out_bf16 = (ek == EK_GATE || ek == EK_BIASBF16 || ek == EK_DWGATE) ? 1 : 0;
    Chain* chp = c->ch;
    auto gp = std::make_shared<GemmP>(p);
    op.gemm = gp;
    op.lk = (int)lk; op.ek = (int)ek; op.mode = t128;
    op.skinny_affine = p.xcd_tile_affine && (t128 & 48) == 0 && t128 != 0 && t128 != 1 && t128 != 4;
    op.run = [c, chp, gp, lk, ek, t128, film](hipStream_t s) mutable -> hipError_t {
                        if (film && gp->film == nullptr) {
                            GemmP q = *gp;
                            set_film(q, c, chp);
                            return dispatch_gemm(q, lk, ek, t128, s);
                        }
                        return dispatch_gemm(*gp, lk, ek, t128, s);
                    };
    prog.push_back(op);
}

struct GateOut { const float* gate_c = nullptr; const float* gate_s = nullptr; const float* add = nullptr; };
void add_naf_block(hd_ctx* c, std::vector<Op>& prog, const BlockW& bw, const Level& lv, const float* static_film, int* x_np,
                   int* x_cnt, const GateOut* gate = nullptr) {
    const int C = bw.C, M = lv.M, HW = lv.H * lv.H;
    auto film_fields = [&](GemmP& p, int half) {
        p.hw = HW; p.face0 = c->ch->face0;
        p.film = static_film;
        p.film_bias_off = bw.film_off + (2 * half) * C;
        p.film_gain_off = bw.film_off + (2 * half + 1) * C;
    };
    bool strip_pool = false;
    static const bool no_fuse = hd_env("HD_NO_DWFUSE") != nullptr, no_chain = hd_env("HD_NO_CHAIN") != nullptr;
    static const bool no_strip = hd_env("HD_NO_STRIP") != nullptr || no_fuse || no_chain;
    const bool by_strips = ((C == 128 && lv.H == 32) || (C == 256 && lv.H == 16)) && (*x_np) * (*x_cnt) == C && *x_np <= 16 && !no_strip;
    if (dwgate_ok(HW) && !no_fuse && !by_strips) {
        GemmP p = base_gemm(bw.conv1, M);
        p.A = lv.Xb; p.lda = C; film_fields(p, 0);
        p.stats_in = lv.sx; p.stats_np = *x_np; p.stats_cnt = *x_cnt;
        p.out = lv.G; p.ldo = C; p.dw_w = bw.dw_wT; p.dw_b = bw.dw_b; p.pooled = lv.pooled; p.pooled16 = lv.pooled16; p.side = lv.H;
        add_gemm(c, prog, bw.name + ".conv2_gate_pool", p, LK_LN, EK_DWGATE);
    } else if (by_strips) {
        StripP q{};
        q.faces = M / HW; q.side = lv.H; q.C = C;
        q.Xb = lv.Xb; q.stats_in = lv.sx; q.stats_np = *x_np; q.stats_cnt = *x_cnt;
        q.W1 = bw.conv1.w; q.b1 = bw.conv1.bias; q.dw_wT = bw.dw_wT; q.dw_b = bw.dw_b;
        q.film = static_film; q.film_gain_off = bw.film_off + C; q.film_bias_off = bw.film_off; q.film_face_stride = 0; q.face0 = c->ch->face0; q.ln_eps = 1e-6f;
        q.G = lv.G; q.pool_part = lv.T1;
        Chain* chp = c->ch;
        Op op;
        op.name = bw.name + ".conv2_gate_pool"; op.out = lv.G; op.out_elems = (size_t)M * C; op.out_bf16 = 1;
        op.run = [c, chp, q](hipStream_t s) mutable -> hipError_t {
            StripP r = q;
            if (r.film == nullptr) set_film(r, c, chp);
            return run_strip_dwgate(r, s);
        };
        prog.push_back(op);
        strip_pool = true;
    } else {
        {
            GemmP p = base_gemm(bw.conv1, M);
            p.A = lv.Xb; p.lda = C; film_fields(p, 0);
            p.stats_in = lv.sx; p.stats_np = *x_np; p.stats_cnt = *x_cnt;
            p.out = lv.T1; p.ldo = 2 * C;
            add_gemm(c, prog, bw.name + ".conv1", p, LK_LN, EK_BIASF32);
        }
        {
            const float *T1 = lv.T1, *w = bw.dw_w, *b = bw.dw_b;
            unsigned short* G = lv.G; float* pooled = lv.pooled;
            const int H = lv.H, faces = M / HW;
            float* part = lv.T1 + (size_t)2 * M * C;
            const int nbands = (H + 7) / 8;
            prog.push_back({bw.name + ".conv2_gate_pool", [=](hipStream_t s) -> hipError_t {
                                hipLaunchKernelGGL(dwconv_gate_pool_kernel, dim3(C / 32, faces, nbands), dim3(256), 0, s, T1, w, b, G, part, H, H, C);
                                return hipGetLastError();
                            }});
            prog.back().out = G; prog.back().out_elems = (size_t)M * C; prog.back().out_bf16 = 1;
            prog.push_back({bw.name + ".pool_finish", [=](hipStream_t s) -> hipError_t {
                                hipLaunchKernelGGL(dwconv_pool_finish_kernel, dim3((faces * C + 255) / 256), dim3(256), 0, s, part, pooled, faces, nbands, C,
                                                   1.0f / (float)(H * H));
                                return hipGetLastError();
                            }});
            prog.back().out = pooled; prog.back().out_elems = (size_t)faces * C;
        }
    }
    if ((C == 128 || C == 256) && HW % 32 == 0 && !no_fuse && !no_chain) {
        ChainP q{};
        q.M = M; q.hw = HW; q.face0 = c->ch->face0;
        q.G = lv.G; q.pooled = lv.pooled; q.X = lv.X;
        if (strip_pool) { q.pool_part = lv.T1; q.pool_nparts = lv.H / 4 ; q.pool_scale = 1.0f / (float)HW; q.pooled_out = lv.pooled; }
        q.Wsca = bw.sca.w; q.W3 = bw.conv3.w; q.W4 = bw.conv4.w; q.W5 = bw.conv5.w;
        q.bsca = bw.sca.bias; q.b3 = bw.conv3.bias; q.b4 = bw.conv4.bias; q.b5 = bw.conv5.bias; q.beta = bw.beta; q.gamma = bw.gamma;
        q.film = static_film; q.film_bias_off = bw.film_off + 2 * C; q.film_gain_off = bw.film_off + 3 * C; q.ln_eps = 1e-6f;
        q.Xout = lv.X; q.Xout16 = lv.Xb; q.stats_out = lv.sx;
        if (gate) { q.outg16 = lv.Xg; q.gate_c = gate->gate_c; q.gate_s = gate->gate_s; q.add_src = gate->add; q.stats_out = nullptr; q.Xout16 = nullptr; }
        Chain* chp = c->ch;
        const bool big = (C == 256);
        static const int mt128 = hd_env("HD_CHAIN_MT") ? atoi(hd_env("HD_CHAIN_MT")) : 1;
        const bool two = !big && mt128 == 2 && HW % 64 == 0 && M % 64 == 0;
        Op op;
        op.name = bw.name + ".conv5"; op.out = lv.X; op.out_elems = (size_t)M * C; op.out_bf16 = 0;
        op.run = [c, chp, q, big, two](hipStream_t s) mutable -> hipError_t {
            ChainP r = q;
            if (r.film == nullptr) set_film(r, c, chp);
            return big ? launch_chain<256, 1>(r, s) : two ? launch_chain<128, 2>(r, s) : launch_chain<128, 1>(r, s);
        };
        prog.push_back(op);
        *x_np = C / 32; *x_cnt = 32;
        return;
    }
    const int hint35 = (M == 1024 && C == 1024) ? 3 : -1, hint3 = (M == 4096 && C == 512) ? 1 : hint35, hint4 = (M == 4096 && C == 512) ? 1 : -1;
    const bool prescale = dwgate_ok(HW) && !no_fuse && HW <= 16;
    if (prescale) {
        {
            GemmP p = base_gemm(bw.sca, M / HW);
            p.A = lv.pooled16; p.lda = C; p.out = lv.S; p.ldo = C; p.scale_G = lv.G; p.scale_hw = HW;
            add_gemm(c, prog, bw.name + ".sca", p, LK_BF16, EK_SCA);
        }
        {
            GemmP p = base_gemm(bw.conv3, M);
            p.A = lv.G; p.lda = C;
            p.out = lv.Y; p.ldo = C; p.resid = lv.X; p.ldr = C; p.rscale = bw.beta;
            p.stats_out = lv.sy; p.out16 = lv.Yb;
            add_gemm(c, prog, bw.name + ".conv3", p, LK_BF16, EK_RESID, hint3);
        }
    } else {
        {
            GemmP p = base_gemm(bw.sca, M / HW);
            p.out = lv.S; p.ldo = C;
            if (dwgate_ok(HW) && !no_fuse) {
                p.A = lv.pooled16; p.lda = C; p.scale_G = lv.G; p.scale_hw = 0;
                add_gemm(c, prog, bw.name + ".sca", p, LK_BF16, EK_SCA);
            } else {
                p.A = lv.pooled; p.lda = C;
                add_gemm(c, prog, bw.name + ".sca", p, LK_F32, EK_BIASF32);
            }
        }
        {
            GemmP p = base_gemm(bw.conv3, M);
            p.A = lv.G; p.lda = C; p.hw = HW; p.rowscale = lv.S;
            p.out = lv.Y; p.ldo = C; p.resid = lv.X; p.ldr = C; p.rscale = bw.beta;
            p.stats_out = lv.sy; p.out16 = lv.Yb;
            add_gemm(c, prog, bw.name + ".conv3", p, LK_BF16S, EK_RESID, hint3);
        }
    }
    {
        GemmP p = base_gemm(bw.conv4, M);
        p.A = lv.Yb; p.lda = C; film_fields(p, 1);
        p.stats_in = lv.sy; p.stats_np = C / 32; p.stats_cnt = 32;
        p.out = lv.G; p.ldo = C;
        add_gemm(c, prog, bw.name + ".conv4", p, LK_LN, EK_GATE, hint4);
    }
    {
        GemmP p = base_gemm(bw.conv5, M);
        p.A = lv.G; p.lda = C;
        p.out = lv.X; p.ldo = C; p.resid = lv.Y; p.ldr = C; p.rscale = bw.gamma;
        p.stats_out = lv.sx; p.out16 = lv.Xb;
        if (gate) {
            p.outg16 = lv.Xg; p.gate_c = gate->gate_c; p.gate_s = gate->gate_s; p.add_src = gate->add; p.hw = HW;
            p.stats_out = nullptr; p.out16 = nullptr;
        }
        add_gemm(c, prog, bw.name + ".conv5", p, LK_BF16, EK_RESID, hint35);
    }
    *x_np = C / 32; *x_cnt = 32;
}

void add_down(hd_ctx* c, std::vector<Op>& prog, const std::string& name, const PackedW& w, const Level& src, const Level& dst) {
    GemmP p = base_gemm(w, dst.M);
    p.A = src.Xb; p.lda = src.C; p.Hin = src.H; p.Win = src.H; p.Cin = src.C; p.KH = 2; p.KW = 2; p.stride = 2; p.pad = 0;
    p.Hout = dst.H; p.Wout = dst.H; p.ntaps = 4;
    p.out = dst.X; p.ldo = dst.C; p.stats_out = dst.sx; p.out16 = dst.Xb;
    add_gemm(c, prog, name, p, LK_CONV_BF16, EK_BIASF32, dst.M >= 4096 ? 3 : -1);
}

void add_up(hd_ctx* c, std::vector<Op>& prog, const std::string& name, const PackedW& w, const void* in, bool in_bf16, int M_in,
            int H_in, int C_in, float* out, const float* skip, int r, unsigned short* out16 = nullptr, float2* stats = nullptr) {
    GemmP p = base_gemm(w, M_in);
    p.A = in; p.lda = C_in; p.Hin = H_in; p.Win = H_in; p.shuffle_r = r;
    p.out = out; p.ldo = w.N / (r * r); p.resid = skip; p.bias = nullptr;
    p.out16 = out16; p.stats_out = stats;
    const int hint = M_in >= 4096 ? 3 : (M_in >= 1024 && M_in < 2048 && w.Kp >= 1024) ? 1 : -1;
    add_gemm(c, prog, name, p, in_bf16 ? LK_BF16 : LK_F32, EK_PIXSHUF, hint);
}

void add_hca(hd_ctx* c, std::vector<Op>& prog, const std::string& name, const HcaW& hw, const unsigned short* in, float* out,
             unsigned short* out16, int M, int H) {
    static const bool no_lds = hd_env("HD_NO_CONVLDS") != nullptr;
    if (!hw.centre_only && !no_lds) {
        ConvP q{};
        q.M = M; q.X = in; q.W = hw.fused.w; q.bias = hw.fused.bias; q.out = out; q.out16 = out16;
        const int C = hw.C;
        int which = -1;
        if (C == 128 && H == 16) which = 0; else if (C == 256 && H == 8) which = 1; else if (C == 512 && H == 4) which = 2;
        else if (C == 1024 && H == 2) which = 3; else if (C == 256 && H == 16) which = 4; else if (C == 512 && H == 8) which = 5;
        else if (C == 1024 && H == 4) which = 6; else if (C == 2048 && H == 2) which = 7; else if (C == 128 && H == 32) which = 8;
        if (which >= 0) {
            Op op;
            op.name = name; op.out = out; op.out_elems = (size_t)M * C;
            op.run = [q, which](hipStream_t s) -> hipError_t {
                switch (which) {
                    case 0: return launch_hca_conv<ConvL0>(q, s);
                    case 1: return launch_hca_conv<ConvL1>(q, s);
                    case 2: return launch_hca_conv<ConvL2>(q, s);
                    case 3: return launch_hca_conv<ConvL3>(q, s);
                    case 4: return launch_hca_conv<ConvL1x32>(q, s);
                    case 5: return launch_hca_conv<ConvL2x32>(q, s);
                    case 6: return launch_hca_conv<ConvL3x32>(q, s);
                    case 8: return launch_hca_conv<ConvL0x32>(q, s);
                    default: return launch_hca_conv<ConvL4x32>(q, s);
                }
            };
            prog.push_back(op);
            return;
        }
    }
    GemmP p = base_gemm(hw.fused, M);
    p.A = in; p.lda = hw.C; p.Hin = H; p.Win = H; p.Cin = hw.C; p.Hout = H; p.Wout = H; p.stride = 1;
    if (hw.centre_only) { p.KH = 1; p.KW = 1; p.pad = 0; p.ntaps = 1; }
    else { p.KH = 3; p.KW = 3; p.pad = 1; p.ntaps = 9; }
    p.out = out; p.ldo = hw.C; p.act = 1; p.out16 = out16;
    add_gemm(c, prog, name, p, LK_CONV_BF16, EK_BIASF32);
}

void link_prefetch(std::vector<Op>& prog, bool wrap) {
    static const bool off = hd_env("HD_PREFETCH") == nullptr;
    static const std::string only = hd_env("HD_PREFETCH") ? hd_env("HD_PREFETCH") : "";
    static const size_t min_bytes = hd_env("HD_PF_MIN") ? (size_t)atol(hd_env("HD_PF_MIN")) : (size_t)1 << 20;
    const int n = (int)prog.size();
    for (int i = 0; i < n; ++i) {
        if (!prog[i].gemm) continue;
        prog[i].gemm->pf_base = nullptr;
        if (off) continue;
        if (only != "1" && (prog[i].name.size() < only.size() || prog[i].name.compare(prog[i].name.size() - only.size(), only.size(), only) != 0)) continue;
        const int j = (i + 1 < n) ? i + 1 : (wrap ? 0 : -1);
        if (j < 0 || !prog[j].gemm || !prog[j].skinny_affine) continue;
        const GemmP& nx = *prog[j].gemm;
        const size_t tile_bytes = (size_t)nx.Kp * 32 * 2;
        if ((size_t)nx.nt_total * tile_bytes < min_bytes) continue;
        prog[i].gemm->pf_base = nx.W; prog[i].gemm->pf_tile_u4 = (unsigned)(tile_bytes / 16); prog[i].gemm->pf_ntiles = nx.nt_total;
// ... 31 lines not shown
```

hifidiff_amd/csrc/hd_kernels.hpp:

```cpp
#pragma once
#include <hip/hip_runtime.h>
#include <stdint.h>

#include "hd_gemm.hpp"

namespace hd {

struct StepState {
    int step;
    int n_steps;
    const float* noise;
    unsigned long long seed;
    float* x0_hist;
    const float* c7;
    const int* start_rows;
    int hist_first;
    const unsigned long long* face_seeds;
    const int* face_first;
    const float* mask;
    const float* mask_known;
    const float* mask_noise;
    const int* mask_on;
    const int* begin_rows;
    const int* end_rows;
    float* pv_x0;
    int* pv_row;
    float* pv_snap;
    int pv_every, pv_snaps, pv_batch;
    const float* gd_lp;
    const float* gd_w;
    const int* gd_n;
    const int* gd_j0;
    const int* gd_j1;
};

struct PackP {
    const float* src; uint4* dst;
    int N, Cin, Cin_pad, KH, KW, ntaps, centre_only, S2, Kp, nt_total;
    const float* nscale;
};
static __global__ void pack_weight_kernel(const PackP p) {
    const int ksteps = p.Kp >> 4;
    const size_t total = (size_t)p.nt_total * ksteps * 64;
    for (size_t e = (size_t)blockIdx.x * blockDim.x + threadIdx.x; e < total; e += (size_t)gridDim.x * blockDim.x) {
        const int lane = (int)(e & 63);
        const size_t tk = e >> 6;
        const int ks = (int)(tk % ksteps), nt = (int)(tk / ksteps);
        const int np = nt * 32 + (lane & 31);
        float v[8];
#pragma unroll
        for (int j = 0; j < 8; ++j) {
            const int k = ks * 16 + 8 * (lane >> 5) + j;
            const int tap = k / p.Cin_pad, c = k - tap * p.Cin_pad;
            float x = 0.f;
            if (np < p.N && tap < p.ntaps && c < p.Cin) {
                int n = np;
                if (p.S2 > 1) { const int cg = p.N / p.S2; n = (np % cg) * p.S2 + np / cg; }
                int ky, kx;
                if (p.centre_only) { ky = p.KH >> 1; kx = p.KW >> 1; }
                else { ky = tap / p.KW; kx = tap - ky * p.KW; }
                x = p.src[(((size_t)n * p.Cin + c) * p.KH + ky) * p.KW + kx];
                if (p.nscale) x *= p.nscale[n];
            }
            v[j] = x;
        }
        p.dst[e] = pack8(v);
    }
}

static __global__ void pack_weight16_kernel(const float* __restrict__ src, uint4* __restrict__ dst, int N, int K) {
    const int ksteps = K >> 5;
    const size_t total = (size_t)(N >> 4) * ksteps * 64;
    for (size_t e = (size_t)blockIdx.x * blockDim.x + threadIdx.x; e < total; e += (size_t)gridDim.x * blockDim.x) {
        const int lane = (int)(e & 63);
        const size_t tk = e >> 6;
        const int ks = (int)(tk % ksteps), mb = (int)(tk / ksteps);
        const float* q = src + (size_t)(mb * 16 + (lane & 15)) * K + ks * 32 + 8 * (lane >> 4);
        float v[8];
#pragma unroll
        for (int j = 0; j < 8; ++j) v[j] = q[j];
        dst[e] = pack8(v);
    }
}

static __global__ void dw_weight_layout_kernel(const float* __restrict__ w, float* __restrict__ wT, int n2c) {
    const int i = blockIdx.x * blockDim.x + threadIdx.x;
    if (i >= n2c * 9) return;
    const int ch = i / 9, t = i - ch * 9;
    wT[(size_t)t * n2c + ch] = w[i];
}

static __global__ void intro_weight_layout_kernel(const float* __restrict__ w, float* __restrict__ wT) {
    const int i = blockIdx.x * blockDim.x + threadIdx.x;
    if (i >= 128 * 36) return;
    const int co = i / 36;
    wT[(i - co * 36) * 128 + co] = w[i];
}
constexpr int kIntroPx = 8, kEndingPx = 8, kLongRunRows = 32768;
template <int PXS>
__global__ __launch_bounds__(256) void intro_conv_kernel(const float* __restrict__ lat, const float* __restrict__ wT,
                                                          const float* __restrict__ b, float* __restrict__ out,
                                                          unsigned short* __restrict__ out16, float2* __restrict__ stats, int B, int L,
                                                          StepState* st, int advance) {
    __shared__ float patch[4][4][3][PXS + 4];
    if (advance && blockIdx.x == 0 && threadIdx.x == 0) st->step += 1;
    const int lane = threadIdx.x & 63, wave = threadIdx.x >> 6;
    const int nseg = B * L * (L / PXS);
    const int seg = blockIdx.x * 4 + wave;
    if (seg >= nseg) return;
    const int spr = L / PXS;
    const int bb = seg / (L * spr), rem = seg - bb * L * spr, y = rem / spr, x0 = (rem - y * spr) * PXS;
    for (int i = lane; i < 4 * 3 * (PXS + 2); i += 64) {
        const int ci = i / (3 * (PXS + 2)), r = (i - ci * 3 * (PXS + 2)) / (PXS + 2), xx = i - ci * 3 * (PXS + 2) - r * (PXS + 2);
        const int yy = y + r - 1, x = x0 + xx - 1;
        patch[wave][ci][r][xx] = (yy >= 0 && yy < L && x >= 0 && x < L) ? lat[((size_t)(bb * 4 + ci) * L + yy) * L + x] : 0.f;
    }
    float wl[36][2];
#pragma unroll
    for (int r = 0; r < 36; ++r) { wl[r][0] = wT[r * 128 + lane]; wl[r][1] = wT[r * 128 + lane + 64]; }
    const float b0 = b[lane], b1 = b[lane + 64];
    __builtin_amdgcn_wave_barrier();
    const size_t row0 = ((size_t)bb * L + y) * L + x0;
#pragma unroll
    for (int px = 0; px < PXS; ++px) {
        float a0 = b0, a1 = b1;
#pragma unroll
        for (int ci = 0; ci < 4; ++ci)
#pragma unroll
            for (int r = 0; r < 3; ++r)
#pragma unroll
                for (int k = 0; k < 3; ++k) {
                    const float v = patch[wave][ci][r][px + k];
                    a0 += v * wl[ci * 9 + r * 3 + k][0];
                    a1 += v * wl[ci * 9 + r * 3 + k][1];
                }
        const size_t o = (row0 + px) * 128;
        out[o + lane] = a0; out[o + lane + 64] = a1;
        out16[o + lane] = f32_to_bf16_bits(a0); out16[o + lane + 64] = f32_to_bf16_bits(a1);
        const float s1 = wave_sum(a0 + a1), s2 = wave_sum(a0 * a0 + a1 * a1);
        const float mean = s1 * (1.0f / 128.0f);
        if (lane == 0) stats[row0 + px] = make_float2(mean, fmaxf(s2 - s1 * mean, 0.f));
    }
}

struct SchedArgs {
    float* lat;
    const float* coef;
    const StepState* st;
    int elem0, n_total;
    const float* film_table; float* film_cur; int film_total;
};
__device__ __forceinline__ float philox_normal(unsigned long long seed, unsigned step, unsigned idx);
__device__ __forceinline__ int st_row(const StepState* st, int f) { return ((const __attribute__((address_space(1))) int*)st->start_rows)[f]; }
__device__ __forceinline__ int st_begin(const StepState* st, int f) { return st->begin_rows ? ((const __attribute__((address_space(1))) int*)st->begin_rows)[f] : 0; }
__device__ __forceinline__ int st_end(const StepState* st, int f) { return st->end_rows ? ((const __attribute__((address_space(1))) int*)st->end_rows)[f] : st->n_steps; }
__device__ __forceinline__ bool st_first(const StepState* st, int f, int k, int r) {
    return k == r && (st->face_first ? ((const __attribute__((address_space(1))) int*)st->face_first)[f] != 0 : st->hist_first != 0);
}
__device__ __forceinline__ bool st_guided(const StepState* st, int f, int j) {
    if (!st->gd_w) return false;
    if (((const __attribute__((address_space(1))) float*)st->gd_w)[f] == 0.f) return false;
    return j >= ((const __attribute__((address_space(1))) int*)st->gd_j0)[f] && j < ((const __attribute__((address_space(1))) int*)st->gd_j1)[f];
}
__device__ __forceinline__ float sched_x0(float xv, float e, const float* c) {
    float x0 = (xv - c[0] * e) / c[1];
    x0 = fminf(fmaxf(x0, -c[2]), c[2]);
    return x0;
}
template <bool PF = false>
__device__ __forceinline__ float sched_from_x0(float x0, float xv, float e, const float* c, const StepState* st, int step, size_t gi, int n_total,
                                              size_t li, bool first, int f, unsigned ef, int ll) {
    float c3 = c[3];
    if (PF && first && st->x0_hist) c3 += ((const __attribute__((address_space(1))) float*)st->c7)[step];
    float r = c3 * x0 + c[4] * xv + c[5] * e;
    if (c[6] != 0.f) {
        float z;
        if (st->noise) z = ((const __attribute__((address_space(1))) float*)st->noise)[(size_t)step * n_total + gi];
        else if (PF && st->face_seeds) z = philox_normal(((const __attribute__((address_space(1))) unsigned long long*)st->face_seeds)[f], (unsigned)(step - st_begin(st, f)), ef);
        else z = philox_normal(st->seed, (unsigned)(PF ? step - st_begin(st, f) : step), (unsigned)gi);
        r += c[6] * z;
    }
    if (st->x0_hist) {
        __attribute__((address_space(1))) float* h = (__attribute__((address_space(1))) float*)st->x0_hist;
        float c7 = ((const __attribute__((address_space(1))) float*)st->c7)[step];
        if (PF && first) c7 = 0.f;
        if (c7 != 0.f) r += c7 * h[li];
        h[li] = x0;
    }
    if (st->mask && ((const __attribute__((address_space(1))) int*)st->mask_on)[f] != 0) {
        const bool last = step + 1 >= (PF ? st_end(st, f) : st->n_steps);
        const float b0 = last ? 1.f : c[7 + 1], b1 = last ? 0.f : c[7 + 0];
        const float m = ((const __attribute__((address_space(1))) float*)st->mask)[(size_t)f * ll + (ef & (unsigned)(ll - 1))];
        const float kn = b0 * ((const __attribute__((address_space(1))) float*)st->mask_known)[li] +
                         b1 * ((const __attribute__((address_space(1))) float*)st->mask_noise)[li];
        r = m * r + (1.f - m) * kn;
    }
    if (st->pv_x0) {
        float p = x0;
        if (st->mask && ((const __attribute__((address_space(1))) int*)st->mask_on)[f] != 0) {
            const float m = ((const __attribute__((address_space(1))) float*)st->mask)[(size_t)f * ll + (ef & (unsigned)(ll - 1))];
            p = m * x0 + (1.f - m) * ((const __attribute__((address_space(1))) float*)st->mask_known)[li];
        }
        ((__attribute__((address_space(1))) float*)st->pv_x0)[li] = p;
        const int j1 = step - (PF ? st_begin(st, f) : 0) + 1, s = j1 / st->pv_every - 1;
        const bool snap = j1 % st->pv_every == 0 && s < st->pv_snaps;
        if (snap) ((__attribute__((address_space(1))) float*)st->pv_snap)[(size_t)s * st->pv_batch * 4 * ll + li] = p;
        if (ef == 0) {
            __attribute__((address_space(1))) int* rows = (__attribute__((address_space(1))) int*)st->pv_row;
            rows[f] = step;
            if (snap) rows[(size_t)(1 + s) * st->pv_batch + f] = step;
// ... 540 lines not shown
```

hifidiff_amd/csrc/hd_lib.hip:

```cpp
#include "hd_internal.hpp"

static std::string g_create_error;
void set_contextless_error(const std::string& msg) { g_create_error = msg; }

namespace {

int alloc_chain(hd_ctx* c, Chain& ch) {
    const int L = c->L, B = ch.B;
    const bool names = (ch.index == 0);
    auto& dbg = c->ws->dbg;
    int rc = 0;
    for (int l = 0; l < 5; ++l) {
        Level& v = ch.lv[l];
        v.C = WIDTH << l; v.H = L >> l; v.M = B * v.H * v.H;
        const size_t mc = (size_t)v.M * v.C;
        rc |= alloc_level(c, v, B, mc, names, l);
        const int pi = 4 - l;
        rc |= ws_alloc(c, &ch.prior[pi], mc); rc |= ws_alloc(c, &ch.gate_c[pi], (size_t)B * v.C);
        rc |= ws_alloc(c, &ch.gate_s[pi], (size_t)v.M);
        if (rc) return rc;
        if (names) {
            const std::string ps = std::to_string(pi);
            dbg["Xg" + std::to_string(l)] = {v.Xg, {mc, 1}};
            dbg["prior" + ps] = {ch.prior[pi], {mc, 0}}; dbg["wc" + ps] = {ch.gate_c[pi], {(size_t)B * v.C, 0}};
// ... 321 lines not shown

void add_fpg(hd_ctx* c, std::vector<Op>& prog, const float* cr_latent_dev) {
    const int B = c->ch->B, L = c->L;
    const RawTensor *iw = find_raw(c, "fpg.intro.weight"), *ib = find_raw(c, "fpg.intro.bias");
    {
        const float *w = c->fpg_intro_wT, *b = ib->dev; float* out = c->ch->lv[0].X; const int M = c->ch->lv[0].M; float2* sx = c->ch->lv[0].sx;
        unsigned short* xb = c->ch->lv[0].Xb;
        Chain* chp = c->ch;
        prog.push_back({"fpg.intro", [=](hipStream_t s) -> hipError_t {
                            if (M >= kLongRunRows) hipLaunchKernelGGL(intro_conv_kernel<16>, dim3((M / 16 + 3) / 4), dim3(256), 0, s, cr_latent_dev, w, b, out, xb, sx, B, L, chp->step_state, 0);
                            else hipLaunchKernelGGL(intro_conv_kernel<kIntroPx>, dim3((M / kIntroPx + 3) / 4), dim3(256), 0, s, cr_latent_dev, w, b, out, xb, sx, B, L, chp->step_state, 0);
                            return hipGetLastError();
                        }});
        prog.back().out = out; prog.back().out_elems = (size_t)M * 128;
    }
    const int enc[4] = {2, 2, 4, 8};
    int bi = 0;
    int np = 1, cnt = WIDTH;
    for (int l = 0; l < 4; ++l) {
        for (int j = 0; j < enc[l]; ++j) add_naf_block(c, prog, c->fpg_blocks[bi++], c->ch->lv[l], c->fpg_ln_pack, &np, &cnt);
        add_down(c, prog, "fpg.downs." + std::to_string(l), c->fpg_down[l], c->ch->lv[l], c->ch->lv[l + 1]);
        np = c->ch->lv[l + 1].C / 32; cnt = 32;
    }
    add_up(c, prog, "fpg.convs.0", c->fpg_convs[0], c->ch->lv[4].X, false, c->ch->lv[4].M, c->ch->lv[4].H, c->ch->lv[4].C, c->ch->prior[0], nullptr, 1);
    for (int i = 1; i < 5; ++i) {
        const Level &hi = c->ch->lv[5 - i], &lo = c->ch->lv[4 - i];
        GemmP p = base_gemm(c->fpg_convs[i], hi.M);
        p.A = c->ch->prior[i - 1]; p.lda = hi.C; p.Hin = hi.H; p.Win = hi.H; p.shuffle_r = 2;
        p.out = c->ch->prior[i]; p.ldo = lo.C; p.resid = lo.X; p.bias = nullptr;
        add_gemm(c, prog, "fpg.convs." + std::to_string(i), p, LK_F32, EK_PIXSHUF);
    }
}

void add_resconv(hd_ctx* c, std::vector<Op>& prog, const std::string& name, const ResConv& rc, const unsigned short* in, int Hin,
                 unsigned short* out, const unsigned short* resid, bool relu) {
    const int Hout = (Hin + 2 * rc.pad - rc.k) / rc.stride + 1;
    GemmP p = base_gemm(rc.w, c->ch->B * Hout * Hout);
    p.A = in; p.out = out; p.ldo = rc.cout; p.resid = resid; p.ldr = rc.cout; p.act = relu ? 1 : 0;
    if (rc.k == 1 && rc.stride == 1) {
        p.lda = rc.cin;
        add_gemm(c, prog, name, p, LK_BF16, EK_BIASBF16);
    } else {
        const int cin = rc.w.K / (rc.k * rc.k);
        p.lda = cin; p.Hin = Hin; p.Win = Hin; p.Cin = cin; p.KH = rc.k; p.KW = rc.k; p.stride = rc.stride; p.pad = rc.pad;
        p.Hout = Hout; p.Wout = Hout; p.ntaps = rc.k * rc.k;
        add_gemm(c, prog, name, p, LK_CONV_BF16, EK_BIASBF16);
    }
}

void add_resnet(hd_ctx* c, std::vector<Op>& prog, const float* cr_face_dev) {
    const int B = c->ch->B;
    {
        uint4* f8 = c->ch->face8; const size_t npix = (size_t)B * 128 * 128;
        prog.push_back({"idc.input", [=](hipStream_t s) -> hipError_t {
                            hipLaunchKernelGGL(nchw3_to_nhwc8_bf16_kernel, dim3((unsigned)((npix + 255) / 256)), dim3(256), 0, s, cr_face_dev, f8, 128 * 128, npix);
                            return hipGetLastError();
                        }});
        prog.back().out = f8; prog.back().out_elems = npix * 8; prog.back().out_bf16 = 1;
    }
    unsigned short *b0 = c->ch->res_buf[0], *b1 = c->ch->res_buf[1], *b2 = c->ch->res_buf[2], *b3 = c->ch->res_buf[3];
    add_resconv(c, prog, "idc.conv1", c->res_conv1, reinterpret_cast<const unsigned short*>(c->ch->face8), 128, b0, nullptr, true);
    {
        const size_t total = (size_t)B * 32 * 32 * 64;
        prog.push_back({"idc.max_pool", [=](hipStream_t s) -> hipError_t {
                            hipLaunchKernelGGL(maxpool3x3s2_bf16_kernel, dim3((unsigned)((total + 255) / 256)), dim3(256), 0, s, b0, b1, B, 64, 64, 64);
                            return hipGetLastError();
                        }});
        prog.back().out = b1; prog.back().out_elems = total; prog.back().out_bf16 = 1;
    }
    unsigned short *x = b1, *y1 = b0, *y2 = b2, *idn = b3;
    int H = 32, bi = 0;
    const int res_layers[4] = {3, 4, 6, 3};
    for (int li = 0; li < 4; ++li)
        for (int b = 0; b < res_layers[li]; ++b) {
            const ResBlock& rb = c->res_blocks[bi++];
            const std::string q = "idc.layer" + std::to_string(li + 1) + "." + std::to_string(b);
            const int Hout = H / rb.c2.stride;
            add_resconv(c, prog, q + ".conv1", rb.c1, x, H, y1, nullptr, true);
            add_resconv(c, prog, q + ".conv2", rb.c2, y1, H, y2, nullptr, true);
            const unsigned short* identity = x;
            if (rb.has_ds) { add_resconv(c, prog, q + ".i_downsample", rb.ds, x, H, idn, nullptr, false); identity = idn; }
            add_resconv(c, prog, q + ".conv3", rb.c3, y2, Hout, y1, identity, true);
            std::swap(x, y1);
            H = Hout;
        }
    {
        float* emb = c->ch->id_emb; const unsigned short* xin = x; const int HW = H * H;
        prog.push_back({"idc.avgpool", [=](hipStream_t s) -> hipError_t {
                            hipLaunchKernelGGL(avgpool_bf16_kernel, dim3(2048 / 256, B), dim3(256), 0, s, xin, emb, HW, 2048);
                            return hipGetLastError();
                        }});
        prog.back().out = emb; prog.back().out_elems = (size_t)B * 2048;
    }
}

int ensure_film_rows(hd_ctx* c, int rows) {
    if (rows <= c->film_rows_cap) return HD_OK;
    dev_free(c, c->t_dev); dev_free(c, c->temb_a); dev_free(c, c->temb_b); dev_free(c, c->temb_c); dev_free(c, c->film_table);
    int rc = 0;
    rc |= dev_alloc(c, &c->t_dev, rows); rc |= dev_alloc(c, &c->temb_a, (size_t)rows * 128);
    rc |= dev_alloc(c, &c->temb_b, (size_t)rows * 1024); rc |= dev_alloc(c, &c->temb_c, (size_t)rows * 512);
    rc |= dev_alloc(c, &c->film_table, (size_t)rows * c->film_total);
    if (rc) return rc;
    c->film_rows_cap = rows;
    c->film_valid = false;
    c->dbg["film"] = {c->film_table, {(size_t)rows * c->film_total, 0}};
    c->dbg["temb"] = {c->temb_c, {(size_t)rows * 512, 0}};
    return HD_OK;
}

int compute_film(hd_ctx* c, const float* t_dev, int n, hipStream_t s) {
    const RawTensor *w1 = find_raw(c, "denoiser.time_mlp.1.weight"), *b1 = find_raw(c, "denoiser.time_mlp.1.bias");
    const RawTensor *w3 = find_raw(c, "denoiser.time_mlp.3.weight"), *b3 = find_raw(c, "denoiser.time_mlp.3.bias");
    hipLaunchKernelGGL(time_embed_kernel, dim3((n * 64 + 255) / 256), dim3(256), 0, s, t_dev, c->freq_dev, c->temb_a, n);
    hipLaunchKernelGGL((linear_f32_kernel<false>), dim3(1024 / 64, (n + 63) / 64), dim3(256), 0, s, c->temb_a, 128, w1->dev, b1->dev, c->temb_b, 1024, n, 1024, 128);
    hipLaunchKernelGGL((linear_f32_kernel<true>), dim3(512 / 64, (n + 63) / 64), dim3(256), 0, s, c->temb_b, 1024, w3->dev, b3->dev, c->temb_c, 512, n, 512, 512);
    hipLaunchKernelGGL((linear_f32_kernel<true>), dim3((c->film_total + 63) / 64, (n + 63) / 64), dim3(256), 0, s, c->temb_c, 512, c->film_W, c->film_b,
                       c->film_table, c->film_total, n, c->film_total, FILM_IN);
    hipLaunchKernelGGL(film_fold_kernel, dim3(2048 / 256, (unsigned)c->den_blocks.size(), n), dim3(256), 0, s, c->film_table, c->ln_pack, c->film_blocks_dev, c->film_total);
    HIPCHECK(c, hipGetLastError());
    return HD_OK;
}



int setup_xcd(hd_ctx* c) {
    c->xcd_ok = false; c->face_ok = false;
    c->end_fold = getenv("HD_NO_END_FOLD") == nullptr;
    if (c->S != 1 || getenv("HD_NO_XCD")) return HD_OK;
    hipDeviceProp_t prop;
    if (hipGetDeviceProperties(&prop, c->device) != hipSuccess || prop.multiProcessorCount != XS_GROUPS * XS_GROUP_WG) return HD_OK;
    HIPCHECK(c, hipHostMalloc(reinterpret_cast<void**>(&c->xcd_tmo_host), 64, hipHostMallocMapped));
    c->xcd_tmo_host[0] = 0;
    HIPCHECK(c, hipHostGetDevicePointer(reinterpret_cast<void**>(&c->xcd_tmo_dev), c->xcd_tmo_host, 0));
    if (int rc = dev_alloc(c, &c->abort_dev, 64)) return rc;
    HIPCHECK(c, hipMemset(c->abort_dev, 0, 64 * sizeof(unsigned)));
    c->xcd_ok = true;
    c->xcd2_mask = getenv("HD_XCD2") ? (atoi(getenv("HD_XCD2")) & 3) : 1;
    c->face_ok = getenv("HD_NO_FACE") == nullptr;
    c->intro_fold = getenv("HD_NO_INTRO_FOLD") == nullptr;
    c->down_fold = getenv("HD_NO_DOWN_FOLD") == nullptr;
    c->up_fold = getenv("HD_NO_UP_FOLD") == nullptr;
    if (const char* e = getenv("HD_FACE_L1_ROWS")) c->face_l1_rows = atoi(e) == 32 ? 32 : 16;
    return HD_OK;
}
int get_xstage(hd_ctx* c, int first_block, int nblocks, hd_ctx::XStage** out) {
    auto it = c->xstages.find(first_block);
    if (it != c->xstages.end() && it->second.nblocks == nblocks) { *out = &it->second; return HD_OK; }
    hd_ctx::XStage st;
    st.nblocks = nblocks;
    std::vector<XBlockW> host((size_t)nblocks);
    for (int j = 0; j < nblocks; ++j) {
        const BlockW& bw = c->den_blocks[first_block + j];
        XBlockW& x = host[j];
        x.w1 = bw.conv1.w; x.wsca = bw.sca.w; x.w3 = bw.conv3.w; x.w4 = bw.conv4.w; x.w5 = bw.conv5.w;
        x.b1 = bw.conv1.bias; x.bsca = bw.sca.bias; x.b3 = bw.conv3.bias; x.b4 = bw.conv4.bias; x.b5 = bw.conv5.bias;
        x.beta = bw.beta; x.gamma = bw.gamma; x.dw_w = bw.dw_wT; x.dw_b = bw.dw_b; x.film_off = bw.film_off; x.pad_ = 0;
    }
    int rc = dev_alloc(c, &st.blocks_dev, (size_t)nblocks);
    rc |= dev_alloc(c, &st.sync, (size_t)3 * 256);
    if (rc) return rc;
    HIPCHECK(c, hipMemcpy(st.blocks_dev, host.data(), host.size() * sizeof(XBlockW), hipMemcpyHostToDevice));
    HIPCHECK(c, hipMemset(st.sync, 0, (size_t)3 * 256 * sizeof(unsigned)));
    const int C = c->den_blocks[first_block].C, HW = (C == 1024) ? 4 : 16;
    if (c->xcd2_mask & (C == 1024 ? 2 : 1)) {
        for (int j = 0; j < nblocks; ++j) {
            const BlockW& bw = c->den_blocks[first_block + j];
            const char* conv[5] = {".conv1", ".sca.1", ".conv3", ".conv4", ".conv5"};
            const uint4** dst[5] = {&host[j].w1, &host[j].wsca, &host[j].w3, &host[j].w4, &host[j].w5};
            for (int k = 0; k < 5; ++k) {
                const RawTensor* w = find_raw(c, bw.name + conv[k] + ".weight");
                if (!w || (int)w->shape[1] != C) HD_FAIL(c, HD_ERR_WEIGHTS, "missing %s%s.weight", bw.name.c_str(), conv[k]);
                const int N = (int)w->shape[0];
                uint4* d = nullptr;
                if (int r2 = dev_alloc(c, &d, (size_t)N * C / 8)) return r2;
                hipLaunchKernelGGL(pack_weight16_kernel, dim3(1024), dim3(256), 0, 0, w->dev, d, N, C);
                *dst[k] = d;
            }
        }
        int r2 = dev_alloc(c, &st.blocks2_dev, (size_t)nblocks);
        r2 |= dev_alloc(c, &st.sync2, (size_t)2048);
        const size_t hn = (size_t)64 * HW * C / 8;
        r2 |= dev_alloc(c, &st.hX, hn); r2 |= dev_alloc(c, &st.hG, hn); r2 |= dev_alloc(c, &st.hY, hn);
        r2 |= dev_alloc(c, &st.hsx, (size_t)64 * HW * (C / 16)); r2 |= dev_alloc(c, &st.hsy, (size_t)64 * HW * (C / 16));
        if (r2) return r2;
        HIPCHECK(c, hipGetLastError());
        HIPCHECK(c, hipMemcpy(st.blocks2_dev, host.data(), host.size() * sizeof(XBlockW), hipMemcpyHostToDevice));
        HIPCHECK(c, hipMemset(st.sync2, 0, (size_t)2048 * sizeof(unsigned)));
        HIPCHECK(c, hipMemset(st.hX, 0, hn * 16)); HIPCHECK(c, hipMemset(st.hG, 0, hn * 16)); HIPCHECK(c, hipMemset(st.hY, 0, hn * 16));
        HIPCHECK(c, hipMemset(st.hsx, 0, (size_t)64 * HW * (C / 16) * 8)); HIPCHECK(c, hipMemset(st.hsy, 0, (size_t)64 * HW * (C / 16) * 8));
    }
    c->xstages[first_block] = st;
    *out = &c->xstages[first_block];
    return HD_OK;
}
static int check_xcd(hd_ctx* c) {
    if (c->xcd_tmo_host && c->xcd_tmo_host[0]) {
        const unsigned code = c->xcd_tmo_host[0];
        (void)hipDeviceSynchronize();
        c->xcd_tmo_host[0] = 0;
        if (c->abort_dev) (void)hipMemset(c->abort_dev, 0, 64 * sizeof(unsigned));
        c->xcd_on = false;
        invalidate_step_graphs(c);
        for (auto& kv : c->xstages) {
            (void)hipMemset(kv.second.sync, 0, (size_t)3 * 256 * sizeof(unsigned));
            if (kv.second.sync2) (void)hipMemset(kv.second.sync2, 0, (size_t)2048 * sizeof(unsigned));
        }
        for (auto& kv : c->fstages) (void)hipMemset(kv.second.sync, 0, (size_t)2 * 64 * 16 * sizeof(unsigned));
        c->face_on = false;
        HD_FAIL(c, HD_ERR_HIP, "persistent stage: a hand-off wait gave up (code 0x%x%s); the results of that call are invalid (NaN), "
                               "the context now runs one launch per GEMM", code, c->stage_test_abort ? ", injected by stage_test_abort" : "");
    }
    return HD_OK;
}
static int poison_on_abort(hd_ctx* c, float* buf, size_t n, hipStream_t s) {
    if (!c->abort_dev || !c->xcd_ok) return HD_OK;
    hipLaunchKernelGGL(poison_if_abort_kernel, dim3((unsigned)((n + 255) / 256)), dim3(256), 0, s, c->abort_dev, buf, n);
    HIPCHECK(c, hipGetLastError());
    return HD_OK;
}

}

extern "C" {

const char* hd_last_error(const hd_ctx* ctx) { return ctx ? ctx->err.c_str() : g_create_error.c_str(); }

int hd_create_unconditional(hd_ctx** out, int latent_res, int device) {
    int rc = hd_create(out, latent_res, device);
    if (rc == HD_OK) (*out)->conditional = false;
    return rc;
}

int hd_create(hd_ctx** out, int latent_res, int device) {
    if (!out) return HD_ERR_INVALID;
    *out = nullptr;
    if (latent_res != 16 && latent_res != 32 && latent_res != 64) {
        g_create_error = "latent_res must be 16, 32 or 64 (level sides must be powers of two), got " + std::to_string(latent_res);
        return HD_ERR_INVALID;
    }
    int ndev = 0;
    if (hipGetDeviceCount(&ndev) != hipSuccess || ndev <= 0) { g_create_error = "no HIP device available"; return HD_ERR_HIP; }
    if (device < 0 || device >= ndev) { g_create_error = "device index out of range"; return HD_ERR_INVALID; }
    if (hipSetDevice(device) != hipSuccess) { g_create_error = "hipSetDevice failed"; return HD_ERR_HIP; }
    hipDeviceProp_t prop;
    if (hipGetDeviceProperties(&prop, device) != hipSuccess) { g_create_error = "hipGetDeviceProperties failed"; return HD_ERR_HIP; }
    if (std::string(prop.gcnArchName).find("gfx950") == std::string::npos) {
        g_create_error = std::string("this library is built for gfx950 (MI355X) only; device is ") + prop.gcnArchName;
        return HD_ERR_INVALID;
    }
    hd_ctx* c = new hd_ctx();
    c->L = latent_res; c->device = device; c->S = latent_res / 16;
    int rc = dev_alloc(c, &c->freq_dev, 64);
    if (rc) { g_create_error = c->err; hd_destroy(c); return rc; }
    float freq[64];
    const float e = (float)(-(std::log(10000.0) / 63.0));
    for (int k = 0; k < 64; ++k) freq[k] = expf((float)k * e);
    (void)hipMemcpy(c->freq_dev, freq, sizeof(freq), hipMemcpyHostToDevice);
    (void)hipEventCreate(&c->ev0); (void)hipEventCreate(&c->ev1);
    (void)hipEventCreateWithFlags(&c->fork_ev, hipEventDisableTiming);
    *out = c;
    return HD_OK;
}

void hd_destroy(hd_ctx* c) {
    if (!c) return;
    (void)hipSetDevice(c->device);
    (void)hipDeviceSynchronize();
    destroy(*c->ws);
    for (auto& kv : c->ws_cache) destroy(*kv.second);
    if (c->fork_ev) (void)hipEventDestroy(c->fork_ev);
    if (c->film_ev) (void)hipEventDestroy(c->film_ev);
    for (auto& sg : c->stage) { if (sg.ev) (void)hipEventDestroy(sg.ev); if (sg.host) (void)hipHostFree(sg.host); }
    if (c->xcd_tmo_host) (void)hipHostFree(c->xcd_tmo_host);
    if (c->ev0) (void)hipEventDestroy(c->ev0);
    if (c->ev1) (void)hipEventDestroy(c->ev1);
    for (auto& kv : c->raw) if (kv.second.dev) (void)hipFree(kv.second.dev);
    for (void* p : c->allocs) if (p) (void)hipFree(p);
    delete c;
}

int hd_load_weights(hd_ctx* c, const hd_tensor_desc* t, int n) {
    if (!c || (!t && n > 0)) return HD_ERR_INVALID;
    if (c->finalized) HD_FAIL(c, HD_ERR_INVALID, "weights already finalized");
    HIPCHECK(c, hipSetDevice(c->device));
    for (int i = 0; i < n; ++i) {
        if (!t[i].name || t[i].ndim < 0 || t[i].ndim > 4) HD_FAIL(c, HD_ERR_INVALID, "bad tensor descriptor %d", i);
        const std::string name = t[i].name;
        RawTensor r;
        r.numel = 1;
        for (int d = 0; d < t[i].ndim; ++d) { r.shape.push_back(t[i].shape[d]); r.numel *= (size_t)t[i].shape[d]; }
        const bool counter = name.size() > 19 && name.compare(name.size() - 19, 19, "num_batches_tracked") == 0;
        if (!counter) {
            if (!t[i].data) HD_FAIL(c, HD_ERR_INVALID, "tensor %s has no data", name.c_str());
            HIPCHECK(c, hipMalloc(reinterpret_cast<void**>(&r.dev), r.numel * sizeof(float) + 256));
            HIPCHECK(c, hipMemcpy(r.dev, t[i].data, r.numel * sizeof(float), t[i].is_device ? hipMemcpyDeviceToDevice : hipMemcpyHostToDevice));
            if (r.numel <= HOST_MIRROR_MAX) {
                r.host.resize(r.numel);
                HIPCHECK(c, hipMemcpy(r.host.data(), t[i].data, r.numel * sizeof(float), t[i].is_device ? hipMemcpyDeviceToHost : hipMemcpyHostToHost));
            }
        }
        auto it = c->raw.find(name);
        if (it != c->raw.end() && it->second.dev) (void)hipFree(it->second.dev);
        c->raw[name] = std::move(r);
    }
    return HD_OK;
}

int hd_finalize_weights(hd_ctx* c) {
    if (!c) return HD_ERR_INVALID;
    if (c->finalized) return HD_OK;
    HIPCHECK(c, hipSetDevice(c->device));
    if (c->cr) return finalize_cr(c);
    if (c->vae) return finalize_vae(c);
    const auto man = build_manifest(c->L, c->conditional);
    for (const auto& e : man) {
        const RawTensor* r = find_raw(c, e.first);
        if (!r) HD_FAIL(c, HD_ERR_WEIGHTS, "Missing key in state_dict: %s", e.first.c_str());
        if (r->shape != e.second) HD_FAIL(c, HD_ERR_WEIGHTS, "size mismatch for %s", e.first.c_str());
    }
    if (c->raw.size() != man.size()) {
        std::unordered_map<std::string, int> known;
        for (const auto& e : man) known[e.first] = 1;
        for (const auto& kv : c->raw)
            if (!known.count(kv.first)) HD_FAIL(c, HD_ERR_WEIGHTS, "Unexpected key in state_dict: %s", kv.first.c_str());
    }
    int rc = 0;
    auto load_block = [&](const std::string& p, int C, BlockW& bw) -> int {
        bw.name = p; bw.C = C;
        int r = 0;
        r |= pack_weight(c, p + ".conv1", &bw.conv1); r |= pack_weight(c, p + ".conv3", &bw.conv3);
        r |= pack_weight(c, p + ".sca.1", &bw.sca); r |= pack_weight(c, p + ".conv4", &bw.conv4);
        r |= pack_weight(c, p + ".conv5", &bw.conv5);
        if (r) return r;
        bw.dw_w = find_raw(c, p + ".conv2.weight")->dev; bw.dw_b = find_raw(c, p + ".conv2.bias")->dev;
        bw.beta = find_raw(c, p + ".beta")->dev; bw.gamma = find_raw(c, p + ".gamma")->dev;
        return make_dw_layout(c, bw);
    };
    const int enc[4] = {2, 2, 4, 8};
    std::vector<std::pair<std::string, int>> order;
    for (int l = 0; l < 4; ++l) for (int j = 0; j < enc[l]; ++j) order.push_back({"denoiser.encoders." + std::to_string(l) + "." + std::to_string(j), WIDTH << l});
    for (int j = 0; j < 8; ++j) order.push_back({"denoiser.middle_blks." + std::to_string(j), WIDTH << 4});
    for (int i = 0; i < 4; ++i) for (int j = 0; j < 2; ++j) order.push_back({"denoiser.decoders." + std::to_string(i) + "." + std::to_string(j), WIDTH << (3 - i)});
    int off = 0;
    for (auto& e : order) {
        BlockW bw;
        rc = load_block(e.first, e.second, bw);
        if (rc) return rc;
        bw.film_off = off;
        off += 4 * e.second;
        c->den_block_index[e.first] = (int)c->den_blocks.size();
        c->den_blocks.push_back(bw);
    }
    c->film_total = off;
    rc = setup_xcd(c);
    if (rc) return rc;
    off = 0;
    for (int l = 0; l < 4 && c->conditional; ++l)
        for (int j = 0; j < enc[l]; ++j) {
            BlockW bw;
            rc = load_block("fpg.encoders." + std::to_string(l) + "." + std::to_string(j), WIDTH << l, bw);
            if (rc) return rc;
            bw.film_off = off;
            off += 4 * (WIDTH << l);
            c->fpg_blocks.push_back(bw);
        }
    const int fpg_film_total = off;
    rc |= dev_alloc(c, &c->film_W, (size_t)c->film_total * FILM_IN); rc |= dev_alloc(c, &c->film_b, c->film_total);
    rc |= dev_alloc(c, &c->ln_pack, c->film_total); rc |= dev_alloc(c, &c->fpg_ln_pack, fpg_film_total + 4);
    rc |= dev_alloc(c, &c->film_blocks_dev, c->den_blocks.size());
    if (rc) return rc;
    std::vector<FilmBlock> fbs;
    auto copy_ln = [&](const BlockW& bw, float* dst) -> int {
        const char* names[4] = {".norm1.bias", ".norm1.weight", ".norm2.bias", ".norm2.weight"};
        for (int q = 0; q < 4; ++q)
            HIPCHECK(c, hipMemcpy(dst + bw.film_off + q * bw.C, find_raw(c, bw.name + names[q])->dev, bw.C * sizeof(float), hipMemcpyDeviceToDevice));
        return HD_OK;
    };
    for (const BlockW& bw : c->den_blocks) {
        HIPCHECK(c, hipMemcpy(c->film_W + (size_t)bw.film_off * FILM_IN, find_raw(c, bw.name + ".mlp.1.weight")->dev, (size_t)4 * bw.C * FILM_IN * sizeof(float), hipMemcpyDeviceToDevice));
        HIPCHECK(c, hipMemcpy(c->film_b + bw.film_off, find_raw(c, bw.name + ".mlp.1.bias")->dev, (size_t)4 * bw.C * sizeof(float), hipMemcpyDeviceToDevice));
        rc = copy_ln(bw, c->ln_pack);
        if (rc) return rc;
        fbs.push_back({bw.film_off, bw.C});
    }
    for (const BlockW& bw : c->fpg_blocks) { rc = copy_ln(bw, c->fpg_ln_pack); if (rc) return rc; }
    HIPCHECK(c, hipMemcpy(c->film_blocks_dev, fbs.data(), fbs.size() * sizeof(FilmBlock), hipMemcpyHostToDevice));
    {
        const RawTensor *iw = find_raw(c, "denoiser.intro.weight"), *ew = find_raw(c, "denoiser.ending.weight");
        const RawTensor* fw = c->conditional ? find_raw(c, "fpg.intro.weight") : iw;
        if (!iw || !fw || !ew) HD_FAIL(c, HD_ERR_INVALID, "intro/ending weights missing");
        rc |= dev_alloc(c, &c->intro_wT, 36 * 128); rc |= dev_alloc(c, &c->fpg_intro_wT, 36 * 128); rc |= dev_alloc(c, &c->ending_wT, 9 * 4 * 128);
        if (rc) return rc;
        hipLaunchKernelGGL(intro_weight_layout_kernel, dim3(18), dim3(256), 0, 0, iw->dev, c->intro_wT);
        hipLaunchKernelGGL(intro_weight_layout_kernel, dim3(18), dim3(256), 0, 0, fw->dev, c->fpg_intro_wT);
        hipLaunchKernelGGL(ending_weight_layout_kernel, dim3(18), dim3(256), 0, 0, ew->dev, c->ending_wT);
        HIPCHECK(c, hipGetLastError());
    }
    for (int i = 0; i < 4; ++i) {
        rc |= pack_weight(c, "denoiser.downs." + std::to_string(i), &c->den_down[i]);
        { PackOpts o; o.S2 = 4; rc |= pack_weight(c, "denoiser.ups." + std::to_string(i) + ".0", &c->den_up[i], o); }
        if (c->conditional) rc |= pack_weight(c, "fpg.downs." + std::to_string(i), &c->fpg_down[i]);
    }
    for (int i = 0; i < 5 && c->conditional; ++i) { PackOpts o; o.S2 = i ? 4 : 1; rc |= pack_weight(c, "fpg.convs." + std::to_string(i) + ".0", &c->fpg_convs[i], o); }
    if (c->conditional) { PackOpts o; o.S2 = c->S * c->S; rc |= pack_weight(c, "denoiser.idc_conv", &c->idc_conv, o); }
    if (rc) return rc;
    for (int i = 0; i < 5 && c->conditional; ++i) {
        HcaW& h = c->hca[i];
        const std::string p = "denoiser.hcas." + std::to_string(i);
        h.C = (WIDTH << 4) >> i;
        h.centre_only = ((c->L >> (4 - i)) == 1);
        rc |= pack_weight(c, p + ".channel_mlp.0", &h.mlp0); rc |= pack_weight(c, p + ".channel_mlp.2", &h.mlp2);
        { PackOpts o; o.bn = p + ".spatial_mlp.1"; rc |= pack_weight(c, p + ".spatial_mlp.0", &h.sp0, o); }
        { PackOpts o; o.bn = p + ".fused_mlp.1"; o.centre_only = h.centre_only; rc |= pack_weight(c, p + ".fused_mlp.0", &h.fused, o); }
        if (rc) return rc;
        std::vector<float> s, o2;
        rc = bn_affine(c, p + ".spatial_mlp.4", s, o2);
        if (rc) return rc;
        const RawTensor *w3 = find_raw(c, p + ".spatial_mlp.3.weight"), *b3 = find_raw(c, p + ".spatial_mlp.3.bias");
        std::vector<float> wf(w3->numel);
        for (size_t k = 0; k < w3->numel; ++k) wf[k] = w3->host[k] * s[0];
        h.sp3_b = b3->host[0] * s[0] + o2[0];
        rc = upload_vec(c, wf, &h.sp3_w);
        if (rc) return rc;
    }
    auto load_res = [&](const std::string& conv, const std::string& bn, int cin, int cout, int k, int stride, int pad, ResConv& r) -> int {
        PackOpts o; o.bn = bn;
        if (cin == 3) o.cin_pad = 8;
        r.cin = cin; r.cout = cout; r.k = k; r.stride = stride; r.pad = pad;
        return pack_weight(c, conv, &r.w, o);
    };
    if (c->conditional) rc = load_res("idc.conv1", "idc.batch_norm1", 3, 64, 7, 2, 3, c->res_conv1);
    if (rc) return rc;
    if (c->conditional) {
        const int res_layers[4] = {3, 4, 6, 3}, planes[4] = {64, 128, 256, 512};
        int cin = 64;
        for (int li = 0; li < 4; ++li)
            for (int b = 0; b < res_layers[li]; ++b) {
                const std::string q = "idc.layer" + std::to_string(li + 1) + "." + std::to_string(b);
                const int stride = (b == 0 && li > 0) ? 2 : 1;
                ResBlock rb;
                rc |= load_res(q + ".conv1", q + ".batch_norm1", cin, planes[li], 1, 1, 0, rb.c1);
                rc |= load_res(q + ".conv2", q + ".batch_norm2", planes[li], planes[li], 3, stride, 1, rb.c2);
                rc |= load_res(q + ".conv3", q + ".batch_norm3", planes[li], planes[li] * 4, 1, 1, 0, rb.c3);
                if (b == 0) { rb.has_ds = true; rc |= load_res(q + ".i_downsample.0", q + ".i_downsample.1", cin, planes[li] * 4, 1, stride, 0, rb.ds); }
                if (rc) return rc;
                c->res_blocks.push_back(rb);
                cin = planes[li] * 4;
            }
    }
    HIPCHECK(c, hipDeviceSynchronize());
    int64_t params = 0;
    double macs = 0.0;
    auto add_w = [&](const PackedW& w, double rows_per_face) { params += (int64_t)w.N * w.K; macs += rows_per_face * (double)w.N * w.K; };
    {
        int bi = 0;
        auto blocks_at = [&](int l, int n) {
            const double hw = (double)(c->L >> l) * (c->L >> l);
            for (int j = 0; j < n; ++j) {
                const BlockW& b = c->den_blocks[bi++];
                add_w(b.conv1, hw); add_w(b.conv3, hw); add_w(b.conv4, hw); add_w(b.conv5, hw); add_w(b.sca, 1.0);
                params += 2 * b.C * 9 + 2 * b.C; macs += hw * 2 * b.C * 9;
            }
        };
        for (int l = 0; l < 4; ++l) blocks_at(l, enc[l]);
        blocks_at(4, 8);
        for (int i = 0; i < 4; ++i) blocks_at(3 - i, 2);
        for (int l = 0; l < 4; ++l) {
            const double hwd = (double)(c->L >> (l + 1)) * (c->L >> (l + 1));
            add_w(c->den_down[l], hwd);
            add_w(c->den_up[l], (double)(c->L >> (4 - l)) * (c->L >> (4 - l)));
        }
        for (int i = 0; i < 5 && c->conditional; ++i) { const double hw = (double)(c->L >> (4 - i)) * (c->L >> (4 - i)); add_w(c->hca[i].fused, hw); }
        params += 2 * 128 * 36; macs += 2.0 * c->L * c->L * 128 * 36;
    }
    c->weight_bytes_per_step = params * 2;
    c->flops_per_face_step = 2.0 * macs;
    c->finalized = true;
    return HD_OK;
}

static int check_ready(hd_ctx* c, bool need_prepared) {
    if (!c) return HD_ERR_INVALID;
    if (!c->finalized) HD_FAIL(c, HD_ERR_NOT_READY, "weights are not loaded/finalized");
    if (need_prepared && !c->prepared) HD_FAIL(c, HD_ERR_NOT_READY, "hd_prepare has not been called for this batch");
// ... 941 lines not shown
    if (snapshot < -1 || snapshot >= pv.snaps)
        HD_FAIL(c, HD_ERR_INVALID, "hd_preview_read: snapshot = %d outside [-1, %d)", snapshot, pv.snaps);
    HIPCHECK(c, hipSetDevice(c->device));
    hipStream_t s = reinterpret_cast<hipStream_t>(stream);
    if (slots) {
        rc = stage_slots(c, pv.slots, slots, n, s);
        if (rc) return rc;
    }
    const size_t per_face = (size_t)4 * c->L * c->L;
    PreviewReadP p{};
    p.plane = snapshot < 0 ? pv.x0 : pv.snap + (size_t)snapshot * c->ws->B * per_face;
    p.rows = pv.row + (size_t)(1 + snapshot) * c->ws->B;
    p.slots = slots ? pv.slots : nullptr; p.out = x0_out; p.rows_out = rows_out; p.ll4 = (int)per_face;
    hipLaunchKernelGGL(preview_gather_kernel, dim3(4, n), dim3(256), 0, s, p);
    HIPCHECK(c, hipGetLastError());
    return HD_OK;
}

static std::vector<Op>* which_program(hd_ctx* c, int which) {
    static std::vector<Op> empty;
    if (c->cr) return &c->ws->cr_program;
    if (c->vae) return which == 0 ? &c->ws->vae_enc_prog : &c->ws->vae_dec_prog;
    if (c->ws->chains.empty()) return &empty;
    return which == 0 ? &c->ws->chains[0].program : &c->ws->chains[0].prep_program;
}
int hd_num_ops(hd_ctx* c, int which) { return c ? (int)which_program(c, which)->size() : 0; }
int hd_num_chains(hd_ctx* c) { return c ? (int)c->ws->chains.size() : 0; }
int hd_debug_limit_ops(hd_ctx* c, int which, int n) {
    if (!c) return HD_ERR_INVALID;
    (which == 0 ? c->op_limit : c->prep_limit) = n;
    return HD_OK;
}
const char* hd_debug_op_name(hd_ctx* c, int which, int i) {
    if (!c) return "";
    auto* p = which_program(c, which);
    return (i >= 0 && i < (int)p->size()) ? (*p)[i].name.c_str() : "";
}
int hd_debug_op_info(hd_ctx* c, int which, int i) {
    if (!c) return HD_ERR_INVALID;
    auto* p = which_program(c, which);
    if (i < 0 || i >= (int)p->size()) HD_FAIL(c, HD_ERR_INVALID, "no such op %d", i);
    const Op& op = (*p)[i];
    if (!op.gemm || op.lk < 0) return 0;
    return ((op.lk + 1) & 0xff) | (((op.ek + 1) & 0xff) << 8) | (((op.mode + 1) & 0xff) << 16) | ((op.gemm->xcd_tile_affine ? 1 : 0) << 24) |
           ((op.gemm->w_nt ? 1 : 0) << 25);
}
static int64_t read_to_host(hd_ctx* c, const void* dev, size_t n, int is_bf16, float* host_out, int64_t max_elems) {
    if (!host_out) return (int64_t)n;
    if ((int64_t)n > max_elems) HD_FAIL(c, HD_ERR_INVALID, "debug read needs %zu elements", n);
    HIPCHECK(c, hipSetDevice(c->device));
    HIPCHECK(c, hipDeviceSynchronize());
    if (is_bf16) {
        std::vector<unsigned short> tmp(n);
        HIPCHECK(c, hipMemcpy(tmp.data(), dev, n * 2, hipMemcpyDeviceToHost));
        for (size_t i = 0; i < n; ++i) { unsigned u = (unsigned)tmp[i] << 16; memcpy(&host_out[i], &u, 4); }
    } else {
        HIPCHECK(c, hipMemcpy(host_out, dev, n * sizeof(float), hipMemcpyDeviceToHost));
    }
    return (int64_t)n;
}
int64_t hd_debug_read_op(hd_ctx* c, int which, int i, float* host_out, int64_t max_elems) {
    if (!c) return HD_ERR_INVALID;
    auto* p = which_program(c, which);
    if (i < 0 || i >= (int)p->size() || !(*p)[i].out) HD_FAIL(c, HD_ERR_INVALID, "no such op %d", i);
    return read_to_host(c, (*p)[i].out, (*p)[i].out_elems, (*p)[i].out_bf16, host_out, max_elems);
}

static const std::pair<void*, std::pair<size_t, int>>* find_debug(hd_ctx* c, const char* name) {
    for (const auto* m : {&c->ws->dbg, &c->dbg}) {
        const auto it = m->find(name);
        if (it != m->end()) return &it->second;
    }
    return nullptr;
}

int64_t hd_debug_read(hd_ctx* c, const char* name, float* host_out, int64_t max_elems) {
    if (!c || !name) return HD_ERR_INVALID;
    const size_t B = (size_t)c->ws->B, ll = (size_t)c->L * c->L;
    const bool mk = c->mask.dmask && c->ws->B >= 1 && c->ws->B <= c->mask.cap, gd = c->guide.lp && c->ws->B >= 1 && c->ws->B <= c->guide.cap;
    const bool pv = c->preview.active(c);
    const char *no_mask = "no mask has been set for this batch", *no_guide = "no guidance has been set for this batch";
    const char* no_pv = "previews are off or no batch has been prepared since";
    const struct { const char* name; const void* ptr; size_t elems; bool ok; const char* why; } extras[] = {
        {"mask", c->mask.dmask, B * ll, mk, no_mask}, {"mask_known", c->mask.dknown, B * 4 * ll, mk, no_mask},
        {"mask_noise", c->mask.dnoise, B * 4 * ll, mk, no_mask},
        {"guide_lp", c->guide.lp, B * 4 * ll, gd, no_guide}, {"guide_weight", c->guide.w, B, gd, no_guide}, {"guide_scale", c->guide.n, B, gd, no_guide},
        {"x0_preview", c->preview.x0, B * 4 * ll, pv, no_pv}, {"preview_rows", c->preview.row, B, pv, no_pv},
        {"preview_snaps", c->preview.snap, (size_t)c->preview.snaps * B * 4 * ll, pv, no_pv},
    };
    for (const auto& x : extras) {
        if (strcmp(name, x.name) != 0) continue;
        if (!x.ok) HD_FAIL(c, HD_ERR_INVALID, "debug buffer %s: %s", name, x.why);
        return x.elems ? read_to_host(c, x.ptr, x.elems, 0, host_out, max_elems) : 0;
    }
    const auto* e = find_debug(c, name);
    if (!e) HD_FAIL(c, HD_ERR_INVALID, "unknown debug buffer %s", name);
    return read_to_host(c, e->first, e->second.first, e->second.second, host_out, max_elems);
}

int hd_debug_write(hd_ctx* c, const char* name, const float* host_in, int64_t n_elems) {
    if (!c || !name || !host_in) return HD_ERR_INVALID;
    const auto* e = find_debug(c, name);
    if (!e) HD_FAIL(c, HD_ERR_INVALID, "unknown debug buffer %s", name);
    const size_t n = e->second.first;
    if ((int64_t)n != n_elems) HD_FAIL(c, HD_ERR_INVALID, "debug write of %s needs %zu elements", name, n);
    HIPCHECK(c, hipSetDevice(c->device));
    HIPCHECK(c, hipDeviceSynchronize());
    if (e->second.second) {
        std::vector<unsigned short> tmp(n);
        for (size_t i = 0; i < n; ++i) {
            unsigned u; memcpy(&u, &host_in[i], 4);
            if ((u & 0x7fffffffu) > 0x7f800000u) { tmp[i] = (unsigned short)((u >> 16) | 0x40u); continue; }
            tmp[i] = (unsigned short)((u + 0x7fffu + ((u >> 16) & 1u)) >> 16);
        }
        HIPCHECK(c, hipMemcpy(e->first, tmp.data(), n * 2, hipMemcpyHostToDevice));
    } else {
        HIPCHECK(c, hipMemcpy(e->first, host_in, n * sizeof(float), hipMemcpyHostToDevice));
    }
    return HD_OK;
}

int hd_set_option(hd_ctx* c, const char* key, int value) {
    if (!c || !key) return HD_ERR_INVALID;
    const std::string k = key;
    if (k == "xcd") c->xcd_on = value != 0;
    else if (k == "xcd2") c->xcd2_on = value != 0;
    else if (k == "xcd_phase_limit") c->xcd_phase_limit = value;
    else if (k == "xcd_force_global") c->xcd_force_global = value;
    else if (k == "face") c->face_on = value != 0;
    else if (k == "face_block_limit") c->face_block_limit = value;
    else if (k == "stage_limit_first") c->stage_limit_first = value;
    else if (k == "stage_test_abort") c->stage_test_abort = value;
    else HD_FAIL(c, HD_ERR_INVALID, "unknown option %s", key);
    invalidate_step_graphs(c);
    return HD_OK;
}
int hd_get_option(hd_ctx* c, const char* key) {
    if (!c || !key) return HD_ERR_INVALID;
    const std::string k = key;
    if (k == "xcd") return (c->xcd_ok && c->xcd_on) ? 1 : 0;
    if (k == "xcd2") return (c->xcd_ok && c->xcd_on && c->xcd2_on) ? c->xcd2_mask : 0;
    if (k == "xcd_stages") return (int)c->xstages.size();
    if (k == "face_stages") return (int)c->fstages.size();
    if (k == "face_l1_rows") return c->face_l1_rows;
    if (k == "sample_stage_launches") return c->sample_stages;
    if (k == "sample_face_stage_launches") return c->sample_face_stages;
    if (k == "rows_stage_launches") return c->rows_stages;
    if (k == "masked_faces") return c->mask.faces.valid_for(c->ws->B) ? c->mask.faces.count() : 0;
    if (k == "preview") return c->preview.on ? 1 : 0;
    if (k == "guide") return c->guide.on ? 1 : 0;
    if (k == "guided_faces") return c->guide.faces.valid_for(c->ws->B) ? c->guide.faces.count() : 0;
    if (k == "pool_capacity") return c->pool_cap;
    if (k == "pool_valid") { int n = 0; for (char v : c->pool_ok) n += v != 0; return n; }
    if (k == "graph_captures") return c->graph_captures;
    const Chain* ch = c->ws->chains.empty() ? nullptr : &c->ws->chains[0];
    const bool face_runs = c->xcd_ok && c->face_on && c->ws->chains.size() == 1;
    if (k == "intro_fold") return (ch && ch->fold_intro && face_runs) ? 1 : 0;
    if (k == "down_fold") return (ch && ch->fold_down0 && face_runs) ? 1 : 0;
    if (k == "up_fold") return (ch && ch->fold_up && face_runs) ? 1 : 0;
    if (k == "end_fold") return (ch && ch->fuse_end && c->end_fused) ? 1 : 0;
    return HD_ERR_INVALID;
}

int hd_check(hd_ctx* c) {
    if (!c) return HD_ERR_INVALID;
    return check_xcd(c);
}

int hd_set_profiling(hd_ctx* c, int on) { if (!c) return HD_ERR_INVALID; c->profiling = on != 0; return HD_OK; }

int hd_get_profile(hd_ctx* c, double* loop_ms, double* step_ms_avg, int64_t* weight_bytes_per_step, double* flops_per_face_step) {
    if (!c) return HD_ERR_INVALID;
    float ms = 0.f;
    if (c->profiling && c->last_steps > 0) {
        HIPCHECK(c, hipEventSynchronize(c->ev1));
        HIPCHECK(c, hipEventElapsedTime(&ms, c->ev0, c->ev1));
    }
    if (loop_ms) *loop_ms = ms;
    if (step_ms_avg) *step_ms_avg = c->last_steps > 0 ? ms / c->last_steps : 0.0;
    if (weight_bytes_per_step) *weight_bytes_per_step = c->weight_bytes_per_step;
    if (flops_per_face_step) *flops_per_face_step = c->flops_per_face_step;
    return HD_OK;
}

}
```

hifidiff_amd/csrc/hd_wide.hpp:

```cpp
#pragma once
#include "hd_gemm.hpp"

namespace hd {

#ifdef HD_WIDE_NOB
#define HD_WIDE_BSTAGE(s) 0
#else
#define HD_WIDE_BSTAGE(s) (s)
#endif
#ifdef HD_WIDE_NOA
#define HD_WIDE_ASTAGE(s) 0
#else
#define HD_WIDE_ASTAGE(s) (s)
#endif
typedef float f32x4_wi __attribute__((ext_vector_type(4)));
#ifndef HD_WIDE_P
#define HD_WIDE_P 3
#endif
#ifndef HD_WIDE_PB
#define HD_WIDE_PB 2
#endif
template <bool PAIR, int FORM>
struct WideCfg {
    static constexpr int BM = FORM == 1 ? 256 : (FORM == 2 ? 64 : 128), BK = FORM == 1 ? 64 : 128, THREADS = 512, TNT = PAIR ? 2 : 1, P = HD_WIDE_P;
    static constexpr int UPR = BK / 8, RG = 256 / UPR;
    static constexpr int UPT = BM * UPR / 256;
    static constexpr int KSP = FORM == 1 ? 1 : 2, RW = 4 / KSP;
    static constexpr int MTW = FORM == 2 ? 1 : 2;
    static constexpr int TPRW = 256 / BM;
    static constexpr int AROW = BK * 2 + 16;
    static constexpr int A_BUF = BM * AROW;
    static constexpr int A_OFF = 0, STATS_OFF = 2 * A_BUF, GB_OFF = STATS_OFF + BM * 8;
    static constexpr int PB = HD_WIDE_PB;
};

template <bool PAIR>
inline int wide_shape_ok(const GemmP& p) {
    const int ncols = PAIR ? p.N / 2 : p.N;
    if (p.K != p.Kp || ncols % 32 != 0 || p.film_face_stride != 0 || p.lda != p.K) return 0;
    if (p.Kp == 1024 && p.M % 128 == 0 && p.M >= 1024 && p.M <= 2048 && (p.M / 128) * (ncols / 32) >= 256) return 1;
    static const bool no_tall = hd_env("HD_NO_WIDE_TALL") != nullptr, no_64 = hd_env("HD_NO_WIDE_64") != nullptr;
    if (!no_tall && p.Kp == 512 && p.M % 256 == 0 && p.M >= 4096 && (p.M / 256) * (ncols / 32) >= 256 && (p.M / 256) * (ncols / 32) <= 512) return 2;
    if (!no_64 && p.Kp == 2048 && p.M % 64 == 0 && (p.M / 64) * (ncols / 32) >= 256 && (p.M / 64) * (ncols / 32) <= 512) return 3;
    return 0;
}
inline int wide_form_rows(int form) { return form == 1 ? 128 : (form == 2 ? 256 : 64); }

template <bool PAIR>
inline bool wide_stats_ok(const GemmP& p) {
    const int form = wide_shape_ok<PAIR>(p);
    return form != 0 && p.stats_np >= 1 && p.stats_np <= (form == 1 ? 32 : (form == 2 ? 16 : 64)) && p.stats_np * p.stats_cnt == p.K;
}

#ifdef HD_STAMPS
#define HD_WSTAMP(role, s, k) do { if (p.stamps && blockIdx.x == 0 && blockIdx.y == 0 && lane == 0 && pw == 0) p.stamps[4096 + (role) * 64 + 4 * (s) + (k)] = __builtin_amdgcn_s_memrealtime(); } while (0)
#else
#define HD_WSTAMP(role, s, k) do { } while (0)
#endif
template <bool LN, class EP, bool PAIR, int FORM, int NST>
__global__ __launch_bounds__(512) void gemm_wide_kernel(const GemmP p) {
    typedef WideCfg<PAIR, FORM> C;
    extern __shared__ __attribute__((aligned(16))) char smem[];
    typedef unsigned u32x4 __attribute__((ext_vector_type(4)));
    const int tid = threadIdx.x, lane = tid & 63, wave = __builtin_amdgcn_readfirstlane(tid >> 6);
    const bool producer = wave >= 4;
    const int pw = wave & 3, ptid = tid & 255;
    const int rh = pw % C::RW, kh = pw / C::RW;
    const int ksteps_total = p.Kp >> 4;
    int bx = blockIdx.x, by = blockIdx.y;
    if (p.xcd_tile_affine && (gridDim.y & 7) == 0) {
        const int lin = blockIdx.y * gridDim.x + blockIdx.x, j = lin >> 3;
        bx = j % (int)gridDim.x;
        by = (j / (int)gridDim.x) * 8 + (lin & 7);
    }
    const int row0 = bx * C::BM;
    const int tile0 = by, tile1 = by + (p.N >> 6);
    HD_STAMP(0);

    const int q16 = ptid % C::UPR, r8 = ptid / C::UPR;
    const unsigned short* Ap = reinterpret_cast<const unsigned short*>(p.A) + (size_t)(row0 + r8) * p.lda + q16 * 8;
    u32x4 raw[C::P][C::UPT];
#define HD_WIDE_LOAD(s)                                                                                            \
    {                                                                                                               \
        _Pragma("unroll") for (int u = 0; u < C::UPT; ++u)                                                          \
            raw[(s) % C::P][u] = *reinterpret_cast<const u32x4*>(Ap + (size_t)(C::RG * u) * p.lda + (HD_WIDE_ASTAGE(s)) * C::BK);    \
    }
    if (producer) {
#pragma unroll
        for (int d = 0; d < C::P; ++d) HD_WIDE_LOAD(d);
    }
    HD_STAMP(1);

    float mu[C::UPT], rs[C::UPT];
    float* gb = reinterpret_cast<float*>(smem + C::GB_OFF);
    if constexpr (LN) {
      if (!producer) {
        const int rl = tid / C::TPRW, part = tid % C::TPRW, np = p.stats_np;
        const float2* sp = p.stats_in + (size_t)(row0 + rl) * np;
        float2 s[16];
#pragma unroll
        for (int i = 0; i < 16; ++i) { const int j = part + C::TPRW * i; s[i] = j < np ? sp[j] : make_float2(0.f, -1.f); }
        const float* f = LdF32LN_T<false>::film_row(p);
        for (int k = tid * 4; k < p.K; k += 256 * 4) {
            *reinterpret_cast<float4*>(gb + k) = *reinterpret_cast<const float4*>(f + p.film_gain_off + k);
            *reinterpret_cast<float4*>(gb + p.K + k) = *reinterpret_cast<const float4*>(f + p.film_bias_off + k);
        }
        float sm = 0.f;
#pragma unroll
        for (int i = 0; i < 16; ++i) sm += s[i].y >= 0.f ? s[i].x : 0.f;
        if (C::TPRW >= 2) sm += dpp_mov<0xB1>(sm);
        if (C::TPRW == 4) sm += dpp_mov<0x4E>(sm);
        const float inv_np = 1.0f / (float)np, cnt = (float)p.stats_cnt;
        const float mean = sm * inv_np;
        float q = 0.f;
#pragma unroll
        for (int i = 0; i < 16; ++i) { const float d = s[i].x - mean; q += s[i].y >= 0.f ? fmaf(cnt * d, d, s[i].y) : 0.f; }
        if (C::TPRW >= 2) q += dpp_mov<0xB1>(q);
        if (C::TPRW == 4) q += dpp_mov<0x4E>(q);
        const float var = q * (inv_np / cnt);
        if (part == 0) reinterpret_cast<float2*>(smem + C::STATS_OFF)[rl] = make_float2(mean, __frsqrt_rn(var + p.ln_eps));
      }
        __syncthreads();
        if (producer)
#pragma unroll
        for (int u = 0; u < C::UPT; ++u) {
            float2 st = reinterpret_cast<const float2*>(smem + C::STATS_OFF)[r8 + C::RG * u];
            asm volatile("s_waitcnt lgkmcnt(0)" : "+v"(st.x), "+v"(st.y));
            mu[u] = -st.x * st.y; rs[u] = st.y;
        }
    }
    auto write_stage = [&](int s, int ls) __attribute__((always_inline)) {
        char* sA = smem + C::A_OFF + (s & 1) * C::A_BUF + r8 * C::AROW + q16 * 16;
        if constexpr (LN) {
            typedef __attribute__((address_space(3))) const float lds_f1;
            typedef float f4v __attribute__((ext_vector_type(4)));
            typedef __attribute__((address_space(3))) const f4v lds_f4;
            lds_f1* gl = (lds_f1*)gb;
            const int k = s * C::BK + q16 * 8;
            const f4v g0 = *(lds_f4*)(gl + k), g1 = *(lds_f4*)(gl + k + 4), b0 = *(lds_f4*)(gl + p.K + k), b1 = *(lds_f4*)(gl + p.K + k + 4);
            const f32x2_t g[4] = {{g0.x, g0.y}, {g0.z, g0.w}, {g1.x, g1.y}, {g1.z, g1.w}}, b[4] = {{b0.x, b0.y}, {b0.z, b0.w}, {b1.x, b1.y}, {b1.z, b1.w}};
#pragma unroll
            for (int u = 0; u < C::UPT; ++u) {
                const u32x4 w = raw[s % C::P][u];
                const f32x2_t r2 = {rs[u], rs[u]}, m2 = {mu[u], mu[u]};
                u32x4 o;
#pragma unroll
                for (int i = 0; i < 4; ++i) {
                    const f32x2_t x = {__uint_as_float(w[i] << 16), __uint_as_float(w[i] & 0xffff0000u)};
                    o[i] = pack2(__builtin_elementwise_fma(__builtin_elementwise_fma(x, r2, m2), g[i], b[i]));
                }
                *reinterpret_cast<u32x4*>(sA + C::RG * u * C::AROW) = o;
                if (ls >= 0) {
                    raw[ls % C::P][u] = *reinterpret_cast<const u32x4*>(Ap + (size_t)(C::RG * u) * p.lda + (HD_WIDE_ASTAGE(ls)) * C::BK);
                    __builtin_amdgcn_sched_barrier(0);
                }
            }
        } else {
#pragma unroll
            for (int u = 0; u < C::UPT; ++u) {
                *reinterpret_cast<u32x4*>(sA + C::RG * u * C::AROW) = raw[s % C::P][u];
                if (ls >= 0) {
                    raw[ls % C::P][u] = *reinterpret_cast<const u32x4*>(Ap + (size_t)(C::RG * u) * p.lda + (HD_WIDE_ASTAGE(ls)) * C::BK);
                    __builtin_amdgcn_sched_barrier(0);
                }
            }
        }
    };
    if (producer) {
#ifdef HD_WIDE_PRIO
        __builtin_amdgcn_s_setprio(HD_WIDE_PRIO);
#endif
        write_stage(0, -1);
        asm volatile("s_waitcnt lgkmcnt(0)\n\ts_barrier" ::: "memory");
#pragma unroll
        for (int s = 0; s < NST; ++s) {
            HD_WSTAMP(1, s, 0);
            HD_WSTAMP(1, s, 1);
            if (s + 1 < NST) write_stage(s + 1, s + C::P < NST ? s + C::P : -1);
            asm volatile("s_waitcnt lgkmcnt(0)" ::: "memory");
            HD_WSTAMP(1, s, 2);
            asm volatile("s_barrier" ::: "memory");
            HD_WSTAMP(1, s, 3);
        }
        asm volatile("s_barrier" ::: "memory");
        if constexpr (!EP::kTile) return;
    }
#undef HD_WIDE_LOAD
    constexpr int NM = C::KSP == 1 ? 2 : 1;
    const bool finisher = producer ? false : (C::MTW == 2 || kh == 0);
    f32x16_t mine[NM][C::TNT];
    if (!producer) {
    u32x4 breg[C::PB][4][C::TNT];
    const uint4* Wb[C::TNT];
#pragma unroll
    for (int t = 0; t < C::TNT; ++t) Wb[t] = p.W + ((size_t)(t ? tile1 : tile0) * ksteps_total + kh * 4) * 64 + lane;
#define HD_WIDE_BLOAD(s)                                                                                            \
    {                                                                                                               \
        _Pragma("unroll") for (int j = 0; j < 4; ++j)                                                               \
            _Pragma("unroll") for (int t = 0; t < C::TNT; ++t)                                                      \
                breg[(s) % C::PB][j][t] = *reinterpret_cast<const u32x4*>(Wb[t] + (size_t)((HD_WIDE_BSTAGE(s)) * (C::BK / 16) + j) * 64); \
    }
#pragma unroll
    for (int d = 0; d < C::PB; ++d) HD_WIDE_BLOAD(d);
    asm volatile("s_barrier" ::: "memory");
    HD_STAMP(2);
    f32x16_t acc[C::MTW][C::TNT];
#pragma unroll
    for (int mt = 0; mt < C::MTW; ++mt)
#pragma unroll
        for (int t = 0; t < C::TNT; ++t)
#pragma unroll
            for (int i = 0; i < 16; ++i) acc[mt][t][i] = 0.f;
    const int a_lane_off = (rh * 32 * C::MTW + (lane & 31)) * C::AROW + (lane >> 5) * 16 + kh * 4 * 32;
#pragma unroll
    for (int s = 0; s < NST; ++s) {
        HD_WSTAMP(0, s, 0);
        const char* sA = smem + C::A_OFF + (s & 1) * C::A_BUF + a_lane_off;
#pragma unroll
        for (int j = 0; j < 4; ++j) {
            const bf16x8_t a0 = *reinterpret_cast<const bf16x8_t*>(sA + j * 32), a1 = *reinterpret_cast<const bf16x8_t*>(sA + (C::MTW == 2 ? 32 : 0) * C::AROW + j * 32);
#pragma unroll
            for (int t = 0; t < C::TNT; ++t) {
                const bf16x8_t b = __builtin_bit_cast(bf16x8_t, breg[s % C::PB][j][t]);
#ifdef HD_WIDE_NOMMA
                acc[0][t][0] += __builtin_bit_cast(f32x4_wi, a0)[0] + __builtin_bit_cast(f32x4_wi, b)[0]; acc[C::MTW - 1][t][0] += __builtin_bit_cast(f32x4_wi, a1)[1];
#else
                acc[0][t] = __builtin_amdgcn_mfma_f32_32x32x16_bf16(a0, b, acc[0][t], 0, 0, 0);
                if constexpr (C::MTW == 2) acc[1][t] = __builtin_amdgcn_mfma_f32_32x32x16_bf16(a1, b, acc[1][t], 0, 0, 0);
#endif
            }
        }
        if (s + C::PB < NST) {
            HD_WIDE_BLOAD(s + C::PB);
            asm volatile("" ::: "memory");
        }
        asm volatile("s_waitcnt lgkmcnt(0)" ::: "memory");
        HD_WSTAMP(0, s, 2);
        asm volatile("s_barrier" ::: "memory");
        HD_WSTAMP(0, s, 3);
    }
#undef HD_WIDE_BLOAD
    HD_STAMP(3); HD_STAMP(4);

    if constexpr (C::KSP == 2) {
        float* xch = reinterpret_cast<float*>(smem);
#pragma unroll
        for (int t = 0; t < C::TNT; ++t) {
#pragma unroll
            for (int i = 0; i < 16; ++i) {
                if constexpr (C::MTW == 2) {
                    xch[((wave * C::TNT + t) * 16 + i) * 64 + lane] = kh ? acc[0][t][i] : acc[1][t][i];
                    mine[0][t][i] = kh ? acc[1][t][i] : acc[0][t][i];
                } else {
                    if (kh) xch[((wave * C::TNT + t) * 16 + i) * 64 + lane] = acc[0][t][i];
                    mine[0][t][i] = acc[0][t][i];
                }
            }
        }
        asm volatile("s_waitcnt lgkmcnt(0)\n\ts_barrier" ::: "memory");
        const int partner = rh + C::RW * (1 - kh);
        if (C::MTW == 2 || kh == 0) {
#pragma unroll
            for (int t = 0; t < C::TNT; ++t)
#pragma unroll
                for (int i = 0; i < 16; ++i) {
                    const float o = xch[((partner * C::TNT + t) * 16 + i) * 64 + lane];
                    mine[0][t][i] = kh ? o + mine[0][t][i] : mine[0][t][i] + o;
                }
        }
    } else {
#pragma unroll
        for (int m = 0; m < NM; ++m)
#pragma unroll
            for (int t = 0; t < C::TNT; ++t) mine[m][t] = acc[m][t];
        asm volatile("s_barrier" ::: "memory");
    }
    }
    if constexpr (EP::kTile) {
        constexpr int T1_OFF = C::KSP == 2 ? 32768 : 0;
        float* t1 = reinterpret_cast<float*>(smem + T1_OFF);
        float* rs = reinterpret_cast<float*>(smem + T1_OFF + 2 * C::BM * 32 * 4);
        const int S = p.side, ls = 31 - __builtin_clz(S), HW = p.hw;
        float* wx = rs + (C::BM >> ls) * 32;
        if (finisher) {
#pragma unroll
            for (int t = 0; t < C::TNT; ++t) {
                const float b1 = p.bias[(t ? tile1 : tile0) * 32 + (lane & 31)];
#pragma unroll
                for (int m = 0; m < NM; ++m)
#pragma unroll
                    for (int i = 0; i < 16; ++i) {
                        const int r = rh * 32 * C::MTW + (C::MTW == 1 ? 0 : (C::KSP == 2 ? kh : m)) * 32 + (i & 3) + 8 * (i >> 2) + 4 * (lane >> 5);
                        t1[(t * C::BM + r) * 32 + (lane & 31)] = mine[m][t][i] + b1;
                    }
            }
        } else if (producer && pw == 0) {
            const int hb = (tid >> 5) & 1, jj = tid & 31, ce = tile0 * 32 + jj + hb * (p.N >> 1);
#pragma unroll
            for (int t = 0; t < 9; ++t) wx[(hb * 10 + t) * 32 + jj] = p.dw_w[(size_t)t * p.N + ce];
            wx[(hb * 10 + 9) * 32 + jj] = p.dw_b[ce];
        }
        asm volatile("s_waitcnt vmcnt(0) lgkmcnt(0)\n\ts_barrier" ::: "memory");
        const int C2 = p.N >> 1;
        const int j = tid & 31, col = tile0 * 32 + j;
        float wa[9], wb[9];
#pragma unroll
        for (int t = 0; t < 9; ++t) { wa[t] = wx[t * 32 + j]; wb[t] = wx[(10 + t) * 32 + j]; }
        const float ba = wx[9 * 32 + j], bb = wx[19 * 32 + j];
        const float* t1a = t1 + j;
        const float* t1b = t1 + C::BM * 32 + j;
        const int nrows_img = C::BM >> ls;
        for (int rr = tid >> 5; rr < nrows_img; rr += C::THREADS / 32) {
            const int p0 = rr << ls;
            const int y = (p0 & (HW - 1)) >> ls;
            const bool up = y > 0, dn = y < S - 1;
            const int row = row0 + p0;
            unsigned short* gout = reinterpret_cast<unsigned short*>(p.out) + (size_t)row * p.ldo + col;
            const int left = p.M - row;
            float rsum;
            switch (S) {
                case 16: rsum = dw_gate_row<16>(t1a, t1b, p0, up, dn, wa, wb, ba, bb, gout, p.ldo, true, left); break;
                case 8: rsum = dw_gate_row<8>(t1a, t1b, p0, up, dn, wa, wb, ba, bb, gout, p.ldo, true, left); break;
                case 4: rsum = dw_gate_row<4>(t1a, t1b, p0, up, dn, wa, wb, ba, bb, gout, p.ldo, true, left); break;
                default: rsum = dw_gate_row<2>(t1a, t1b, p0, up, dn, wa, wb, ba, bb, gout, p.ldo, true, left); break;
            }
            rs[rr * 32 + j] = rsum;
        }
        asm volatile("s_waitcnt lgkmcnt(0)\n\ts_barrier" ::: "memory");
        const int faces = C::BM / HW;
        for (int idx = tid; idx < faces * 32; idx += C::THREADS) {
            const int f = idx >> 5;
            float sacc = 0.f;
            for (int r = 0; r < S; ++r) sacc += rs[(f * S + r) * 32 + j];
            const int face = row0 / HW + f;
            const float pm = sacc / (float)HW;
            p.pooled[(size_t)face * C2 + col] = pm;
            if (p.pooled16) p.pooled16[(size_t)face * C2 + col] = f32_to_bf16_bits(pm);
        }
        HD_STAMP(5);
    } else {
        const int ncols = PAIR ? (p.N >> 1) : p.N;
        const int col = tile0 * 32 + (lane & 31);
        if (finisher)
#pragma unroll
        for (int m = 0; m < NM; ++m) {
            const int rtile = row0 + rh * 32 * C::MTW + (C::MTW == 1 ? 0 : (C::KSP == 2 ? kh : m)) * 32;
            tile_epilogue_mfma<true, PAIR, EP>(p, mine[m][0], mine[m][PAIR ? 1 : 0], rtile + 4 * (lane >> 5), col, ncols, tile0, lane);
        }
        HD_STAMP(5);
    }
}

template <bool LN, class EP, bool PAIR, int FORM, int NST>
inline hipError_t launch_gemm_wide_inst(const GemmP& p, hipStream_t s) {
    typedef WideCfg<PAIR, FORM> C;
    const int ncols = PAIR ? p.N / 2 : p.N;
    int smem = C::GB_OFF + (LN ? 2 * p.Kp * 4 : 0);
    const int epi = 32768 + 2 * C::BM * 32 * 4 + (C::BM / 2) * 32 * 4 + 2 * 10 * 32 * 4;
    if (EP::kTile && smem < epi) smem = epi;
    static std::atomic<unsigned long long> granted{0};
    { const hipError_t e = grant_dynamic_lds(reinterpret_cast<const void*>(&gemm_wide_kernel<LN, EP, PAIR, FORM, NST>), 160 * 1024, granted); if (e != hipSuccess) return e; }
    hipLaunchKernelGGL((gemm_wide_kernel<LN, EP, PAIR, FORM, NST>), dim3(p.M / C::BM, ncols / 32, 1), dim3(C::THREADS), smem, s, p);
    return hipGetLastError();
}
template <bool LN, class EP, bool PAIR>
inline hipError_t launch_gemm_wide(const GemmP& p, hipStream_t s) {
    const int form = wide_shape_ok<PAIR>(p);
    if (form == 1) return launch_gemm_wide_inst<LN, EP, PAIR, 0, 8>(p, s);
    if (form == 2) return launch_gemm_wide_inst<LN, EP, PAIR, 1, 8>(p, s);
    if (form == 3) return launch_gemm_wide_inst<LN, EP, PAIR, 2, 16>(p, s);
    return hipErrorInvalidValue;
}

}
```

Measured before the change: 65.60.

## Pack middle-block gated weights in paired-16 column order for skinny GEMMs

Middle-block conv1/conv4 weights are repacked so each 32-column N tile holds 16 columns from each half of the gate pair. The skinny and wide GEMM paths then need only one tile per block, or adjacent tiles, instead of two distant ones, and the epilogue regathers the pairs with ds_bpermute or an index remap. The aim is to halve the per-block weight tiles for small-M middle layers and double the grid parallelism. In exchange it disables the stage-kernel, strip and chain fusions for those blocks and adds new dispatch paths.

New measurement: 66.31 (median of 2 runs). Within noise of the previous version (+1.1%).

```diff
diff --git a/hifidiff_amd/csrc/hd_dispatch.hpp b/hifidiff_amd/csrc/hd_dispatch.hpp
--- a/hifidiff_amd/csrc/hd_dispatch.hpp
+++ b/hifidiff_amd/csrc/hd_dispatch.hpp
@@ -21,6 +21,7 @@
     }
     mode &= 15;
     if constexpr (PAIR) {
+        if (p.pair16) return hipErrorInvalidValue;
         switch (mode) {
             case 0: return launch_gemm<T128P, LD, EP>(p, s);
             case 1: return launch_gemm<T64P, LD, EP>(p, s);
@@ -40,6 +41,21 @@
             case 6: return launch_skinny_auto<8, 1, false, LD, EP>(p, s);
             default: return launch_skinny_auto<1, 1, false, LD, EP>(p, s);
         }
+    }
+}
+
+template <class LD>
+hipError_t launch_tile_pair16(const GemmP& p, int mode, hipStream_t s) {
+    typedef EpPair16<EpGateBF16> EP;
+    if constexpr (std::is_same<LD, LdF32LN_T<false>>::value) {
+        if ((mode & 32) && wide_shape_ok<true>(p) == 3 && wide_stats_ok<true>(p)) return launch_gemm_wide_pair16<EpGateBF16>(p, s);
+    }
+    switch (mode & 15) {
+        case 2: return launch_skinny_auto<1, 2, true, LD, EP>(p, s);
+        case 3: return launch_skinny_auto<1, 1, true, LD, EP>(p, s);
+        case 5: return launch_skinny_auto<4, 1, true, LD, EP>(p, s);
+        case 6: return launch_skinny_auto<8, 1, true, LD, EP>(p, s);
+        default: return hipErrorInvalidValue;
     }
 }
 
@@ -69,11 +85,18 @@
 hipError_t dispatch_ln(const GemmP& p, EpKind ek, int mode, hipStream_t s) {
     if (ek == EK_DWGATE) {
         static const bool no_dw1 = hd_env("HD_NO_DW1") != nullptr;
+        if (p.pair16 && (p.hw != 1 || no_dw1)) return hipErrorInvalidValue;
+        if (p.pair16 && p.M <= 64) return launch_skinny_pair16<LN, EpDwGate1>(p, s);
+        if (p.pair16) return launch_skinny_auto<1, 1, true, LN, EpPair16<EpDwGate1>>(p, s);
         if (p.hw == 1 && !no_dw1) return launch_skinny_auto<1, 1, true, LN, EpDwGate1>(p, s);
         return dispatch_dwgate<LN>(p, s);
     }
-    if (ek == EK_BIASF32) return launch_tile<LN, EpBiasF32, false>(p, mode, s);
-    if (ek == EK_GATE) return launch_tile<LN, EpGateBF16, true>(p, mode, s);
+    if (ek == EK_BIASF32) return p.pair16 ? hipErrorInvalidValue : launch_tile<LN, EpBiasF32, false>(p, mode, s);
+    if (ek == EK_GATE) {
+        if (p.pair16 && p.M <= 64) return launch_skinny_pair16<LN, EpGateBF16>(p, s);
+        if (p.pair16) return launch_tile_pair16<LN>(p, mode, s);
+        return launch_tile<LN, EpGateBF16, true>(p, mode, s);
+    }
     return hipErrorInvalidValue;
 }
 
diff --git a/hifidiff_amd/csrc/hd_gemm.hpp b/hifidiff_amd/csrc/hd_gemm.hpp
--- a/hifidiff_amd/csrc/hd_gemm.hpp
+++ b/hifidiff_amd/csrc/hd_gemm.hpp
@@ -25,6 +25,11 @@
 
 inline const char* hd_env(const char* name) {
     return getenv("HD_EXPERIMENTS") != nullptr ? getenv(name) : nullptr;
+}
+
+__host__ __device__ inline int pair16_source_column(int np, int N) {
+    const int t = np >> 5, j = np & 31;
+    return j < 16 ? 16 * t + j : (N >> 1) + 16 * t + (j - 16);
 }
 
 typedef __attribute__((ext_vector_type(8))) __bf16 bf16x8_t;
@@ -76,6 +81,7 @@
     const uint4* pf_base;
     unsigned pf_tile_u4;
     int pf_ntiles;
+    int pair16;
 #ifdef HD_STAMPS
     unsigned long long* stamps;
 #endif
@@ -679,6 +685,25 @@
     static __device__ __forceinline__ float pre(const GemmP&, int, int) { return 0.f; }
     static __device__ __forceinline__ void store2(const GemmP&, int, int, float, float, const ColC&) {}
 };
+template <class EP>
+struct EpPair16 : EP {
+    static constexpr bool kPair16 = true;
+};
+__device__ __forceinline__ void pair16_gather(f32x16_t& a1, f32x16_t& a2, int lane) {
+    const int c = lane & 31;
+    const int src_a = ((lane & 32) | (c & 15)) << 2, src_b = src_a + 64;
+    const bool second = c >= 16;
+#pragma unroll
+    for (int i = 0; i < 16; ++i) {
+        const int x = __float_as_int(a1[i]), y = __float_as_int(a2[i]);
+        const int xa = __builtin_amdgcn_ds_bpermute(src_a, x), xb = __builtin_amdgcn_ds_bpermute(src_b, x);
+        const int ya = __builtin_amdgcn_ds_bpermute(src_a, y), yb = __builtin_amdgcn_ds_bpermute(src_b, y);
+        a1[i] = __int_as_float(second ? ya : xa);
+        a2[i] = __int_as_float(second ? yb : xb);
+    }
+}
+template <class EP, class = void> struct ep_is_pair16 { static constexpr bool value = false; };
+template <class EP> struct ep_is_pair16<EP, decltype((void)EP::kPair16)> { static constexpr bool value = EP::kPair16; };
 
 constexpr int kStatLane = 16;
 __device__ __forceinline__ float2 halfwave_mean_m2(float v) {
@@ -1274,10 +1299,12 @@
         const bool ev = EVEN || e < C::BM * 32;
         float v1 = 0.f, v2 = 0.f;
         if (ev) {
+            int e1 = e, e2 = C::BM * 32 + e;
+            if constexpr (TNT == 2 && ep_is_pair16<EP>::value) { e1 = ((e & 16) ? C::BM * 32 : 0) + (e & ~31) + (e & 15); e2 = e1 + 16; }
 #pragma unroll
             for (int w = 0; w < WK; ++w) {
-                v1 += red[w * TILE_F + e];
-                if (TNT == 2) v2 += red[w * TILE_F + C::BM * 32 + e];
+                v1 += red[w * TILE_F + e1];
+                if (TNT == 2) v2 += red[w * TILE_F + e2];
             }
         }
         v[it] = 0.f;
@@ -1320,9 +1347,15 @@
     const int ksteps_total = p.Kp >> 4;
     const int cpw = CPW > 0 ? CPW : (p.Kp >> 6) / WK;
     const int c0 = wk * cpw, c_end = c0 + cpw;
+    constexpr bool kP16 = ep_is_pair16<EP>::value && TNT == 1, kP16Two = ep_is_pair16<EP>::value && TNT == 2;
+    static_assert(!ep_is_pair16<EP>::value || !EP::kTile, "no tile epilogue reads the paired-16 order");
+    static_assert(!kP16 || C::BM * 16 == C::THREADS, "EpPair16, one tile: one 32-row tile, one (row, gate column) per thread");
     int tile[TNT];
     tile[0] = by;
-    if (TNT == 2) tile[1] = by + (p.N >> 6);
+    if (TNT == 2) {
+        if constexpr (kP16Two) { tile[0] = 2 * by; tile[1] = 2 * by + 1; }
+        else tile[1] = by + (p.N >> 6);
+    }
     const uint4* Wl = p.W + lane;
     constexpr bool w_nt = W_NT;
     HD_STAMP(0);
@@ -1395,11 +1428,13 @@
             }
         }
     }
-    constexpr bool kEarlyPre = !EP::kTile && !ep_is_sca_tile<EP>::value && C::THREADS >= 512;
+    constexpr bool kEarlyPre = !EP::kTile && !ep_is_sca_tile<EP>::value && !kP16 && C::THREADS >= 512;
+    ColC cc16 = {0.f, 0.f, 0.f, 0.f};
+    if constexpr (kP16) cc16 = EP::col_init(p, by * 16 + (tid & 15));
     SkinnyPre<C> spre;
     if constexpr (kEarlyPre) {
-        const int ncols_e = (TNT == 2) ? (p.N >> 1) : p.N, col_e = tile[0] * 32 + (tid & 31);
-        const bool full_e = (row0 + C::BM <= p.M) && (tile[0] * 32 + 32 <= ncols_e);
+        const int ncols_e = (TNT == 2) ? (p.N >> 1) : p.N, col_e = by * 32 + (tid & 31);
+        const bool full_e = (row0 + C::BM <= p.M) && (by * 32 + 32 <= ncols_e);
         if (full_e) skinny_rows_pre<true, C, EP>(p, row0, col_e, ncols_e, tid, spre);
         else skinny_rows_pre<false, C, EP>(p, row0, col_e, ncols_e, tid, spre);
     }
@@ -1486,7 +1521,7 @@
             }
     __syncthreads();
     const int ncols = (TNT == 2) ? (p.N >> 1) : p.N;
-    const int col = tile[0] * 32 + (tid & 31);
+    const int col = by * 32 + (tid & 31);
 
     if constexpr (EP::kTile) {
         static_assert(TNT == 2, "EpDwGate needs a PAIR tile");
@@ -1582,14 +1617,23 @@
                 }
             }
         }
+    } else if constexpr (kP16) {
+        const int r = tid >> 4, j = tid & 15;
+        float v1 = 0.f, v2 = 0.f;
+#pragma unroll
+        for (int w = 0; w < WK; ++w) {
+            v1 += red[w * TILE_F + r * 32 + j];
+            v2 += red[w * TILE_F + r * 32 + 16 + j];
+        }
+        if (row0 + r < p.M) EP::store2(p, row0 + r, by * 16 + j, v1, v2, cc16);
     } else {
-        const bool full = (row0 + C::BM <= p.M) && (tile[0] * 32 + 32 <= ncols);
+        const bool full = (row0 + C::BM <= p.M) && (by * 32 + 32 <= ncols);
         if constexpr (!kEarlyPre) {
             if (full) skinny_rows_pre<true, C, EP>(p, row0, col, ncols, tid, spre);
             else skinny_rows_pre<false, C, EP>(p, row0, col, ncols, tid, spre);
         }
-        if (full) skinny_rows_epilogue<true, C, EP>(p, red, row0, col, ncols, tile[0], tid, spre);
-        else skinny_rows_epilogue<false, C, EP>(p, red, row0, col, ncols, tile[0], tid, spre);
+        if (full) skinny_rows_epilogue<true, C, EP>(p, red, row0, col, ncols, by, tid, spre);
+        else skinny_rows_epilogue<false, C, EP>(p, red, row0, col, ncols, by, tid, spre);
     }
     if (p.pf_base) prefetch_drain(pf_sink);
     HD_STAMP(5);
@@ -1657,6 +1701,7 @@
 inline hipError_t launch_skinny(const GemmP& p, hipStream_t s) {
     const int smem = C::GB_OFF + (LD::kGainBiasLds ? 2 * p.Kp * 4 : 0);
     if (smem > 160 * 1024 || (p.Kp / 64) % C::WK != 0) return hipErrorInvalidValue;
+    if ((p.pair16 != 0) != ep_is_pair16<EP>::value) return hipErrorInvalidValue;
     const bool nt = p.w_nt != 0;
     if constexpr (LD::kStaticK) {
         static const bool no_static = hd_env("HD_NO_STATIC_K") != nullptr;
@@ -1702,6 +1747,13 @@
     return launch_skinny<SkinnyCfg<WM, 1, MT, PAIR, D>, LD, EP>(p, s);
 }
 
+template <class LD, class EP>
+inline hipError_t launch_skinny_pair16(const GemmP& p, hipStream_t s) {
+    constexpr int D = 2;
+    if (!p.pair16 || p.M > 64 || p.N % 64 != 0 || p.Kp < 1024 || p.Kp % 512 != 0) return hipErrorInvalidValue;
+    return launch_skinny<SkinnyCfg<1, 8, 1, false, D>, LD, EpPair16<EP>>(p, s);
+}
+
 }
 
 #pragma clang fp contract(fast)
diff --git a/hifidiff_amd/csrc/hd_internal.hpp b/hifidiff_amd/csrc/hd_internal.hpp
--- a/hifidiff_amd/csrc/hd_internal.hpp
+++ b/hifidiff_amd/csrc/hd_internal.hpp
@@ -42,6 +42,7 @@
     uint4* w = nullptr;
     int N = 0, K = 0, Kp = 0, nt_total = 0;
     const float* bias = nullptr;
+    int pair16 = 0;
 };
 
 struct BlockW {
@@ -303,6 +304,7 @@
     bool end_fused = true;
     bool up_fold = true;
     bool down_fold = true;
+    bool mid_pair32 = false;
     bool intro_fold = true;
     int face_l1_rows = 16;
     int stage_limit_first = -1;
@@ -591,7 +593,7 @@
     return HD_OK;
 }
 
-struct PackOpts { int cin_pad = 0; bool centre_only = false; int S2 = 1; std::string bn; };
+struct PackOpts { int cin_pad = 0; bool centre_only = false; int S2 = 1; std::string bn; bool pair16 = false; };
 
 int pack_weight(hd_ctx* c, const std::string& name, PackedW* out, const PackOpts& o = PackOpts()) {
     const RawTensor* w = find_raw(c, name + ".weight");
@@ -603,6 +605,8 @@
     PackP p{};
     p.src = w->dev; p.N = N; p.Cin = Cin; p.Cin_pad = cin_pad; p.KH = KH; p.KW = KW; p.ntaps = ntaps;
     p.centre_only = o.centre_only ? 1 : 0; p.S2 = o.S2;
+    if (o.pair16 && (N % 64 != 0 || o.S2 > 1)) HD_FAIL(c, HD_ERR_WEIGHTS, "%s: the paired-16 order needs N %% 64 == 0", name.c_str());
+    p.pair16 = o.pair16 ? 1 : 0;
     const int K = ntaps * cin_pad;
     p.Kp = (K + 63) / 64 * 64;
     p.nt_total = (N + 31) / 32;
@@ -621,7 +625,7 @@
     const int blocks = (int)std::min<size_t>((n16 + 255) / 256, 65535);
     hipLaunchKernelGGL(pack_weight_kernel, dim3(blocks), dim3(256), 0, 0, p);
     HIPCHECK(c, hipGetLastError());
-    out->w = p.dst; out->N = N; out->K = K; out->Kp = p.Kp; out->nt_total = p.nt_total;
+    out->w = p.dst; out->N = N; out->K = K; out->Kp = p.Kp; out->nt_total = p.nt_total; out->pair16 = p.pair16;
     const RawTensor* b = find_raw(c, name + ".bias");
     out->bias = b ? b->dev : nullptr;
     if (!o.bn.empty() || (o.S2 > 1 && b)) {
@@ -677,7 +681,7 @@
 GemmP base_gemm(const PackedW& w, int M) {
     GemmP p{};
     p.M = M; p.N = w.N; p.K = w.K; p.Kp = w.Kp; p.nt_total = w.nt_total; p.W = w.w; p.bias = w.bias;
-    p.a_scale = 1.f; p.hw = 1; p.ln_eps = 1e-6f; p.shuffle_r = 1; p.stats_np = 1; p.stats_cnt = 1;
+    p.a_scale = 1.f; p.hw = 1; p.ln_eps = 1e-6f; p.shuffle_r = 1; p.stats_np = 1; p.stats_cnt = 1; p.pair16 = w.pair16;
     return p;
 }
 
@@ -741,9 +745,10 @@
         p.film_gain_off = bw.film_off + (2 * half + 1) * C;
     };
     bool strip_pool = false;
+    const bool p16 = bw.conv1.pair16 || bw.conv4.pair16;
     static const bool no_fuse = hd_env("HD_NO_DWFUSE") != nullptr, no_chain = hd_env("HD_NO_CHAIN") != nullptr;
     static const bool no_strip = hd_env("HD_NO_STRIP") != nullptr || no_fuse || no_chain;
-    const bool by_strips = ((C == 128 && lv.H == 32) || (C == 256 && lv.H == 16)) && (*x_np) * (*x_cnt) == C && *x_np <= 16 && !no_strip;
+    const bool by_strips = !p16 && ((C == 128 && lv.H == 32) || (C == 256 && lv.H == 16)) && (*x_np) * (*x_cnt) == C && *x_np <= 16 && !no_strip;
     if (dwgate_ok(HW) && !no_fuse && !by_strips) {
         GemmP p = base_gemm(bw.conv1, M);
         p.A = lv.Xb; p.lda = C; film_fields(p, 0);
@@ -794,7 +799,7 @@
             prog.back().out = pooled; prog.back().out_elems = (size_t)faces * C;
         }
     }
-    if ((C == 128 || C == 256) && HW % 32 == 0 && !no_fuse && !no_chain) {
+    if (!p16 && (C == 128 || C == 256) && HW % 32 == 0 && !no_fuse && !no_chain) {
         ChainP q{};
         q.M = M; q.hw = HW; q.face0 = c->ch->face0;
         q.G = lv.G; q.pooled = lv.pooled; q.X = lv.X;
diff --git a/hifidiff_amd/csrc/hd_kernels.hpp b/hifidiff_amd/csrc/hd_kernels.hpp
--- a/hifidiff_amd/csrc/hd_kernels.hpp
+++ b/hifidiff_amd/csrc/hd_kernels.hpp
@@ -38,6 +38,7 @@
     const float* src; uint4* dst;
     int N, Cin, Cin_pad, KH, KW, ntaps, centre_only, S2, Kp, nt_total;
     const float* nscale;
+    int pair16;
 };
 static __global__ void pack_weight_kernel(const PackP p) {
     const int ksteps = p.Kp >> 4;
@@ -56,6 +57,7 @@
             if (np < p.N && tap < p.ntaps && c < p.Cin) {
                 int n = np;
                 if (p.S2 > 1) { const int cg = p.N / p.S2; n = (np % cg) * p.S2 + np / cg; }
+                if (p.pair16) n = pair16_source_column(np, p.N);
                 int ky, kx;
                 if (p.centre_only) { ky = p.KH >> 1; kx = p.KW >> 1; }
                 else { ky = tap / p.KW; kx = tap - ky * p.KW; }
diff --git a/hifidiff_amd/csrc/hd_lib.hip b/hifidiff_amd/csrc/hd_lib.hip
--- a/hifidiff_amd/csrc/hd_lib.hip
+++ b/hifidiff_amd/csrc/hd_lib.hip
@@ -497,6 +497,7 @@
     std::vector<XBlockW> host((size_t)nblocks);
     for (int j = 0; j < nblocks; ++j) {
         const BlockW& bw = c->den_blocks[first_block + j];
+        if (bw.conv1.pair16 || bw.conv4.pair16) HD_FAIL(c, HD_ERR_INVALID, "%s: the stage kernels do not read paired-16 weights", bw.name.c_str());
         XBlockW& x = host[j];
         x.w1 = bw.conv1.w; x.wsca = bw.sca.w; x.w3 = bw.conv3.w; x.w4 = bw.conv4.w; x.w5 = bw.conv5.w;
         x.b1 = bw.conv1.bias; x.bsca = bw.sca.bias; x.b3 = bw.conv3.bias; x.b4 = bw.conv4.bias; x.b5 = bw.conv5.bias;
@@ -671,11 +672,15 @@
             if (!known.count(kv.first)) HD_FAIL(c, HD_ERR_WEIGHTS, "Unexpected key in state_dict: %s", kv.first.c_str());
     }
     int rc = 0;
+    c->mid_pair32 = c->S == 1 && getenv("HD_NO_PAIR32") == nullptr && !hd_env("HD_GEMM_MODE") && !hd_env("HD_OP_MODE") &&
+                    !hd_env("HD_NO_DW1") && !hd_env("HD_NO_DWFUSE");
     auto load_block = [&](const std::string& p, int C, BlockW& bw) -> int {
         bw.name = p; bw.C = C;
         int r = 0;
-        r |= pack_weight(c, p + ".conv1", &bw.conv1); r |= pack_weight(c, p + ".conv3", &bw.conv3);
-        r |= pack_weight(c, p + ".sca.1", &bw.sca); r |= pack_weight(c, p + ".conv4", &bw.conv4);
+        PackOpts pair;
+        pair.pair16 = c->mid_pair32 && C == (WIDTH << 4) && p.compare(0, 21, "denoiser.middle_blks.") == 0;
+        r |= pack_weight(c, p + ".conv1", &bw.conv1, pair); r |= pack_weight(c, p + ".conv3", &bw.conv3);
+        r |= pack_weight(c, p + ".sca.1", &bw.sca); r |= pack_weight(c, p + ".conv4", &bw.conv4, pair);
         r |= pack_weight(c, p + ".conv5", &bw.conv5);
         if (r) return r;
         bw.dw_w = find_raw(c, p + ".conv2.weight")->dev; bw.dw_b = find_raw(c, p + ".conv2.bias")->dev;
@@ -1923,6 +1928,7 @@
     if (k == "guided_faces") return c->guide.faces.valid_for(c->ws->B) ? c->guide.faces.count() : 0;
     if (k == "pool_capacity") return c->pool_cap;
     if (k == "pool_valid") { int n = 0; for (char v : c->pool_ok) n += v != 0; return n; }
+    if (k == "mid_pair32") return c->mid_pair32 ? 1 : 0;
     if (k == "graph_captures") return c->graph_captures;
     const Chain* ch = c->ws->chains.empty() ? nullptr : &c->ws->chains[0];
     const bool face_runs = c->xcd_ok && c->face_on && c->ws->chains.size() == 1;
diff --git a/hifidiff_amd/csrc/hd_wide.hpp b/hifidiff_amd/csrc/hd_wide.hpp
--- a/hifidiff_amd/csrc/hd_wide.hpp
+++ b/hifidiff_amd/csrc/hd_wide.hpp
@@ -75,6 +75,9 @@
     }
     const int row0 = bx * C::BM;
     const int tile0 = by, tile1 = by + (p.N >> 6);
+    constexpr bool kP16 = ep_is_pair16<EP>::value;
+    static_assert(!kP16 || (PAIR && FORM == 2 && !EP::kTile), "EpPair16: the 64-row form's element-wise pair epilogue");
+    const int wt0 = kP16 ? 2 * by : tile0, wt1 = kP16 ? 2 * by + 1 : tile1;
     HD_STAMP(0);
 
     const int q16 = ptid % C::UPR, r8 = ptid / C::UPR;
@@ -193,7 +196,7 @@
     u32x4 breg[C::PB][4][C::TNT];
     const uint4* Wb[C::TNT];
 #pragma unroll
-    for (int t = 0; t < C::TNT; ++t) Wb[t] = p.W + ((size_t)(t ? tile1 : tile0) * ksteps_total + kh * 4) * 64 + lane;
+    for (int t = 0; t < C::TNT; ++t) Wb[t] = p.W + ((size_t)(t ? wt1 : wt0) * ksteps_total + kh * 4) * 64 + lane;
 #define HD_WIDE_BLOAD(s)                                                                                            \
     {                                                                                                               \
         _Pragma("unroll") for (int j = 0; j < 4; ++j)                                                               \
@@ -345,6 +348,7 @@
 #pragma unroll
         for (int m = 0; m < NM; ++m) {
             const int rtile = row0 + rh * 32 * C::MTW + (C::MTW == 1 ? 0 : (C::KSP == 2 ? kh : m)) * 32;
+            if constexpr (kP16) pair16_gather(mine[m][0], mine[m][1], lane);
             tile_epilogue_mfma<true, PAIR, EP>(p, mine[m][0], mine[m][PAIR ? 1 : 0], rtile + 4 * (lane >> 5), col, ncols, tile0, lane);
         }
         HD_STAMP(5);
@@ -366,10 +370,16 @@
 template <bool LN, class EP, bool PAIR>
 inline hipError_t launch_gemm_wide(const GemmP& p, hipStream_t s) {
     const int form = wide_shape_ok<PAIR>(p);
+    if (p.pair16) return hipErrorInvalidValue;
     if (form == 1) return launch_gemm_wide_inst<LN, EP, PAIR, 0, 8>(p, s);
     if (form == 2) return launch_gemm_wide_inst<LN, EP, PAIR, 1, 8>(p, s);
     if (form == 3) return launch_gemm_wide_inst<LN, EP, PAIR, 2, 16>(p, s);
     return hipErrorInvalidValue;
 }
-
-}
+template <class EP>
+inline hipError_t launch_gemm_wide_pair16(const GemmP& p, hipStream_t s) {
+    if (!p.pair16 || wide_shape_ok<true>(p) != 3 || !wide_stats_ok<true>(p)) return hipErrorInvalidValue;
+    return launch_gemm_wide_inst<true, EpPair16<EP>, true, 2, 16>(p, s);
+}
+
+}
```
